# marcelm/cutadapt

Hardware: NVIDIA H100
Metric: reads/sec (150bp SE, 1 adapter, e=0.1) (higher is better)
Workload: dtype u8

## Files before the change

### cutadapt_b200/csrc/cg_api.cu

```cuda
#include <cuda_runtime.h>
#include <stdio.h>
#include <stdlib.h>
#include <string.h>

#include <algorithm>
#include <chrono>
#include <map>
#include <string>
#include <vector>

#include "../../include/cutadapt_b200.h"
#include "cg_hostpack.h"
#include <array>

#include "cg_gzip_core.cuh"
#include "cg_kernels.cuh"
#include "cg_jit.h"
#include "cg_setbuild.h"

static_assert(sizeof(cg_match) == 32 && sizeof(cg_match_rec) == 32, "cg_match must be 32 bytes");
static_assert(sizeof(CgAdapter) == 80 && sizeof(CgEntry) == 32 && sizeof(CgGroup) == 32 &&
                  sizeof(CgSetHeader) == 80, "table layout");

static thread_local std::string g_err;

static int fail(int code, const std::string &msg)
{
    g_err = msg;
    return code;
}
static int cuda_fail(cudaError_t e, const char *what)
{
    char buf[256];
    snprintf(buf, sizeof buf, "CUDA error in %s: %s", what, cudaGetErrorString(e));
    g_err = buf;
    return e == cudaErrorMemoryAllocation ? CG_ENOMEM : CG_ECUDA;
}
#define CU(x)                                                  \
    do {                                                       \
        cudaError_t _e = (x);                                  \
        if (_e != cudaSuccess) return cuda_fail(_e, #x);       \
    } while (0)

extern "C" int cg_version(void) { return CG_ABI_VERSION; }
extern "C" const char *cg_last_error(void) { return g_err.c_str(); }

template <class T> struct DevBuf {
    T *p = nullptr;
    size_t cap = 0;
    int ensure(size_t n)
    {
        if (n <= cap) return CG_OK;
        if (p) cudaFree(p);
        p = nullptr; cap = 0;
        size_t want = n + n / 4 + 64;
        cudaError_t e = cudaMalloc((void **)&p, want * sizeof(T));
        if (e != cudaSuccess) return cuda_fail(e, "cudaMalloc");
        cap = want;
        return CG_OK;
    }
    void release() { if (p) cudaFree(p); p = nullptr; cap = 0; }
};
template <class T> struct PinBuf {
    T *p = nullptr;
    size_t cap = 0;
    int ensure(size_t n)
    {
        if (n <= cap) return CG_OK;
        if (p) cudaFreeHost(p);
        p = nullptr; cap = 0;
        size_t want = n + n / 4 + 64;
        cudaError_t e = cudaMallocHost((void **)&p, want * sizeof(T));
        if (e != cudaSuccess) return cuda_fail(e, "cudaMallocHost");
        cap = want;
        return CG_OK;
    }
    void release() { if (p) cudaFreeHost(p); p = nullptr; cap = 0; }
};

#define CG_N_LANES 3
struct Lane {
    cudaStream_t stream = nullptr;
    DevBuf<uint8_t> d_seq, d_qual, d_pack;
    DevBuf<uint64_t> d_exc;
    PinBuf<uint8_t> h_pack;
    PinBuf<uint64_t> h_exc;
    DevBuf<int64_t> d_offs;
    DevBuf<cg_match_rec> d_out;
    DevBuf<int32_t> d_qtrim;
    PinBuf<uint8_t> h_seq, h_qual;
    PinBuf<int64_t> h_offs;
    PinBuf<cg_match_rec> h_out;
    PinBuf<int32_t> h_qtrim;
    bool busy = false;
    cg_match_rec *dst_out = nullptr; size_t n_out = 0; bool out_bounced = false;
    int32_t *dst_qtrim = nullptr; size_t n_qtrim = 0; bool qtrim_bounced = false;
};

#define CG_FQ_SLOTS 4
struct FastqSlot {
    cudaStream_t stream = nullptr;
    bool busy = false;
    int64_t n_bytes = 0;
    DevBuf<uint8_t> d_in, d_out, d_seq, d_qual;
    DevBuf<uint32_t> d_tiles, d_nl;
    DevBuf<CgFastqRecord> d_rec;
    DevBuf<int32_t> d_len, d_interval, d_keep, d_outlen, d_qtrim, d_mask, d_adest, d_dmbytes, d_dest, d_pairkey, d_origin;
    DevBuf<uint8_t> d_destkeep, d_names, d_infoout;
    DevBuf<int32_t> d_nameoff, d_inforow;
    DevBuf<int64_t> d_infooff;
    DevBuf<int64_t> d_dmbase;
    DevBuf<int64_t> d_offs, d_outoff;
    DevBuf<unsigned long long> d_scan;
    DevBuf<cg_match_rec> d_matches, d_matches_rc;
    DevBuf<uint8_t> d_isrc;
    DevBuf<uint8_t> d_norm;
    DevBuf<int32_t> d_faline;
    DevBuf<int64_t> d_faoff;
    DevBuf<unsigned long long> d_fqstats;
    DevBuf<int32_t> d_polya;
    PinBuf<unsigned long long> h_fqstats;
    DevBuf<int32_t> d_fold;
    DevBuf<unsigned long long> d_ilverr;
    DevBuf<CgGzPiece> d_gzpieces;
    DevBuf<uint8_t> d_gzslots, d_gzout;
    DevBuf<int32_t> d_gzsizes;
    DevBuf<int64_t> d_gzoff;
    int ilv = 0, ilv_peer = -1, ilv_format = 0;
    unsigned long long *d_counters = nullptr;
    int *d_err = nullptr;
    PinBuf<uint8_t> h_in, h_out;
    PinBuf<unsigned long long> h_counters;
};

struct GzinStream {
    DevBuf<uint8_t> d_gz, d_plain;
    PinBuf<uint8_t> h_gz;
    DevBuf<int32_t> d_counts, d_cand, d_members, d_flag;
    DevBuf<int64_t> d_offs;
    DevBuf<GuMember> d_res;
    DevBuf<long long> d_moff;
    DevBuf<unsigned long long> d_scan, d_small;
    DevBuf<uint32_t> d_tiles, d_nl;
    cudaEvent_t done = nullptr;
    long long carry = 0, consumed = 0, members = 0;
    long long pend_plain = 0, pend_consumed = 0, pend_members = 0;
    bool split = false;
    long long stride = CG_GZIN_STRIDE;
    struct Member { int in = 0, bitoff = 0, trailer = 0; uint32_t crc = 0; long long len = 0, start = 0; } mem, pmem;
    long long pend_respec = 0;
    DevBuf<uint8_t> d_win, d_pwin, d_wins;
    DevBuf<GuChunk> d_ch;
    DevBuf<long long> d_coff, d_room;
    DevBuf<uint16_t> d_sym;
    DevBuf<int32_t> d_redo;
    DevBuf<uint32_t> d_part;
    void release()
    {
        d_gz.release(); d_plain.release(); h_gz.release(); d_counts.release(); d_cand.release(); d_members.release();
        d_flag.release(); d_offs.release(); d_res.release(); d_moff.release(); d_scan.release(); d_small.release();
        d_tiles.release(); d_nl.release();
        d_win.release(); d_pwin.release(); d_wins.release(); d_ch.release(); d_coff.release(); d_room.release();
        d_sym.release(); d_redo.release(); d_part.release();
        if (done) cudaEventDestroy(done);
        done = nullptr;
    }
};

struct FqStatsAcc {
    int32_t n_adapters = 0, max_len = 0, kmax = 0;
    std::vector<int64_t> v;
};

struct cg_ctx {
    int device = 0;
    cudaStream_t stream = nullptr;
    bool own_stream = false;
    int sm_count = 148;
    size_t smem_optin = 0;
    Lane lanes[CG_N_LANES];
    int *d_err = nullptr;
    uint8_t *d_enc = nullptr;
    double *d_phred = nullptr;
    DevBuf<uint32_t> scratch_p;
    DevBuf<int> scratch_w;
    DevBuf<unsigned long long> d_stats;
    struct { unsigned long long *d_stats = nullptr; int max_len = 0, kmax = 0; bool armed = false, done = false; } fuse;
    DevBuf<uint4> tasks;
    DevBuf<uint4> tasks2, tasks3;
    unsigned long long *d_task_count = nullptr;
    DevBuf<cg_match_rec> pass_tmp;
    DevBuf<int32_t> view_base, view_back;
    long long launches = 0;
    std::vector<std::pair<cudaEvent_t, cudaEvent_t>> timing;
    std::vector<cudaEvent_t> event_pool;
    double timed_ms = 0.0;
    long long timed_n = 0;
    std::vector<std::array<cudaEvent_t, 4>> stage_events;
    double stage_ms[3] = {0, 0, 0};
    CgHostPool *pool = nullptr;
    std::vector<std::vector<uint64_t>> exc_scratch;
    long long h2d_bytes = 0, d2h_bytes = 0;
    double prof[8] = {0, 0, 0, 0, 0, 0, 0, 0};
    double pack_fraction = 0.6;
    double pack_ref_fraction = 0.6, pack_ref_rate = 0.0;
    int pack_dir = +1;
    bool pack_have_ref = false;
    int numa_node = -1;
    cudaEvent_t scratch_ev = nullptr;
    cudaStream_t scratch_stream = nullptr;
    bool scratch_busy = false;
    FastqSlot fq[CG_FQ_SLOTS];
    int fq_next = 0;
    std::map<int32_t, FqStatsAcc> fq_stats;
    int32_t fq_stats_next = 1;
    std::map<int32_t, GzinStream> gzin;
    int32_t gzin_next = 1;
};

struct cg_adapterset {
    cg_ctx *ctx = nullptr;
    CgBuiltSet host;
    uint8_t *d_blob = nullptr;
    uint64_t *d_masks = nullptr;
    CgEntry *d_entries = nullptr;
    uint8_t *d_index = nullptr;
    struct Pass {
        cg_adapterset *sub = nullptr;
        int group = 0, role = 0;
        int front_pass = -1;
        int map_off = 0;
    };
    std::vector<Pass> passes;
    std::vector<int32_t> pass_map;
    int32_t *d_pass_map = nullptr;
    CgSelectTables select_tables;
    mutable CgJitKernel *jit[2][2][2] = {};
    mutable int jit_state[2][2][2] = {};
    mutable long long plane_reads = 0;
    mutable std::string jit_error;
};

extern "C" int cg_ctx_create(int device, void *stream, cg_ctx **out)
{
    if (!out) return fail(CG_EINVAL, "cg_ctx_create: out is NULL");
    int count = 0;
    cudaError_t e = cudaGetDeviceCount(&count);
    if (e != cudaSuccess || count == 0)
        return fail(CG_ECUDA, std::string("no usable CUDA device (") + cudaGetErrorString(e) +
                                  "); cutadapt_b200 has no CPU fallback");
    if (device < 0 || device >= count) return fail(CG_EINVAL, "cg_ctx_create: device ordinal out of range");
    CU(cudaSetDevice(device));
    cg_ctx *c = new cg_ctx();
    c->device = device;
    cudaDeviceProp prop;
    CU(cudaGetDeviceProperties(&prop, device));
    c->sm_count = prop.multiProcessorCount;
    c->smem_optin = prop.sharedMemPerBlockOptin;
    if (stream) { c->stream = (cudaStream_t)stream; c->own_stream = false; }
    else { CU(cudaStreamCreateWithFlags(&c->stream, cudaStreamNonBlocking)); c->own_stream = true; }
    for (int i = 0; i < CG_N_LANES; ++i) CU(cudaStreamCreateWithFlags(&c->lanes[i].stream, cudaStreamNonBlocking));
    CU(cudaEventCreateWithFlags(&c->scratch_ev, cudaEventDisableTiming));
    CU(cudaMalloc((void **)&c->d_err, 16 * sizeof(int)));
    CU(cudaMemset(c->d_err, 0, 16 * sizeof(int)));
    CU(cudaMalloc((void **)&c->d_task_count, 64));
    CU(cudaMemset(c->d_task_count, 0, 64));
    CU(cudaMalloc((void **)&c->d_enc, 768));
    uint8_t enc[768];
    cg_build_enc_tables(enc);
    CU(cudaMemcpy(c->d_enc, enc, 768, cudaMemcpyHostToDevice));
    {
        double phred[256];
        cg_build_phred_table(phred);
        CU(cudaMalloc((void **)&c->d_phred, sizeof phred));
        CU(cudaMemcpy(c->d_phred, phred, sizeof phred, cudaMemcpyHostToDevice));
    }
    *out = c;
    return CG_OK;
}

static void resolve_timing(cg_ctx *c)
{
    for (auto &pr : c->timing) {
        float ms = 0.f;
        if (cudaEventSynchronize(pr.second) == cudaSuccess && cudaEventElapsedTime(&ms, pr.first, pr.second) == cudaSuccess) {
            c->timed_ms += ms; c->timed_n += 1;
        }
        c->event_pool.push_back(pr.first);
        c->event_pool.push_back(pr.second);
    }
    c->timing.clear();
}

extern "C" int cg_ctx_destroy(cg_ctx *c)
{
    if (!c) return CG_OK;
    cudaSetDevice(c->device);
    cudaDeviceSynchronize();
    resolve_timing(c);
    for (auto ev : c->event_pool) cudaEventDestroy(ev);
    delete c->pool;
    c->pool = nullptr;
    for (int i = 0; i < CG_N_LANES; ++i) {
        Lane &l = c->lanes[i];
        l.d_pack.release(); l.d_exc.release(); l.h_pack.release(); l.h_exc.release();
        l.d_seq.release(); l.d_qual.release(); l.d_offs.release(); l.d_out.release(); l.d_qtrim.release();
        l.h_seq.release(); l.h_qual.release(); l.h_offs.release(); l.h_out.release(); l.h_qtrim.release();
        if (l.stream) cudaStreamDestroy(l.stream);
    }
    c->scratch_p.release(); c->scratch_w.release(); c->tasks.release(); c->tasks2.release(); c->tasks3.release();
    c->pass_tmp.release(); c->view_base.release(); c->view_back.release();
    for (FastqSlot &f : c->fq) {
        f.d_in.release(); f.d_out.release(); f.d_seq.release(); f.d_qual.release(); f.d_tiles.release(); f.d_nl.release();
        f.d_rec.release(); f.d_len.release(); f.d_mask.release(); f.d_adest.release(); f.d_dmbytes.release();
        f.d_dmbase.release(); f.d_keep.release(); f.d_interval.release(); f.d_outlen.release(); f.d_qtrim.release();
        f.d_offs.release(); f.d_outoff.release(); f.d_scan.release(); f.d_matches.release(); f.d_matches_rc.release();
        f.d_isrc.release(); f.d_dest.release(); f.d_pairkey.release(); f.d_destkeep.release(); f.d_origin.release();
        f.d_names.release(); f.d_infoout.release(); f.d_nameoff.release(); f.d_inforow.release(); f.d_infooff.release();
        f.d_norm.release(); f.d_faline.release(); f.d_faoff.release();
        f.d_fqstats.release(); f.d_polya.release(); f.h_fqstats.release();
        f.d_gzpieces.release(); f.d_gzslots.release(); f.d_gzout.release(); f.d_gzsizes.release(); f.d_gzoff.release();
        f.h_in.release(); f.h_out.release(); f.h_counters.release();
        if (f.d_counters) cudaFree(f.d_counters);
        if (f.d_err) cudaFree(f.d_err);
        if (f.stream) cudaStreamDestroy(f.stream);
    }
    for (auto &kv : c->gzin) kv.second.release();
    if (c->scratch_ev) cudaEventDestroy(c->scratch_ev);
    if (c->d_task_count) cudaFree(c->d_task_count);
    if (c->d_err) cudaFree(c->d_err);
    if (c->d_enc) cudaFree(c->d_enc);
    if (c->d_phred) cudaFree(c->d_phred);
    if (c->own_stream && c->stream) cudaStreamDestroy(c->stream);
    delete c;
    return CG_OK;
}

extern "C" int cg_ctx_synchronize(cg_ctx *c)
{
    if (!c) return fail(CG_EINVAL, "ctx is NULL");
    CU(cudaSetDevice(c->device));
    CU(cudaStreamSynchronize(c->stream));
    for (int i = 0; i < CG_N_LANES; ++i) CU(cudaStreamSynchronize(c->lanes[i].stream));
    return CG_OK;
}

extern "C" int64_t cg_ctx_launch_count(cg_ctx *c) { return c ? c->launches : 0; }

extern "C" int cg_ctx_stage_times(cg_ctx *c, double *out3, int reset)
{
    if (!c || !out3) return fail(CG_EINVAL, "cg_ctx_stage_times: NULL argument");
    CU(cudaSetDevice(c->device));
    for (auto &e : c->stage_events) {
        CU(cudaEventSynchronize(e[3]));
        for (int i = 0; i < 3; ++i) {
            float ms = 0;
            CU(cudaEventElapsedTime(&ms, e[i], e[i + 1]));
            c->stage_ms[i] += ms;
        }
        for (auto ev : e) cudaEventDestroy(ev);
    }
    c->stage_events.clear();
    for (int i = 0; i < 3; ++i) out3[i] = c->stage_ms[i];
    if (reset) c->stage_ms[0] = c->stage_ms[1] = c->stage_ms[2] = 0;
    return CG_OK;
}

extern "C" int cg_ctx_kernel_time(cg_ctx *c, double *total_ms, int64_t *launches, int reset)
{
    if (!c) return fail(CG_EINVAL, "ctx is NULL");
    CU(cudaSetDevice(c->device));
    resolve_timing(c);
    if (total_ms) *total_ms = c->timed_ms;
    if (launches) *launches = c->timed_n;
    if (reset) { c->timed_ms = 0.0; c->timed_n = 0; }
    return CG_OK;
}

static void destroy_passes(cg_adapterset *s)
{
    for (auto &p : s->passes) cg_adapterset_destroy(p.sub);
    s->passes.clear();
    s->pass_map.clear();
    if (s->d_pass_map) { cudaFree(s->d_pass_map); s->d_pass_map = nullptr; }
}

static int upload_set(cg_ctx *c, cg_adapterset *s)
{
    s->ctx = c;
    cudaError_t e = cudaSetDevice(c->device);
    if (e == cudaSuccess) e = cudaMalloc((void **)&s->d_blob, s->host.blob.size());
    if (e == cudaSuccess) e = cudaMemcpy(s->d_blob, s->host.blob.data(), s->host.blob.size(), cudaMemcpyHostToDevice);
    if (e == cudaSuccess) e = cudaMalloc((void **)&s->d_masks, s->host.masks64.size() * 8);
    if (e == cudaSuccess) e = cudaMemcpy(s->d_masks, s->host.masks64.data(), s->host.masks64.size() * 8, cudaMemcpyHostToDevice);
    if (e == cudaSuccess && !s->host.index_blob.empty()) {
        e = cudaMalloc((void **)&s->d_index, s->host.index_blob.size());
        if (e == cudaSuccess) e = cudaMemcpy(s->d_index, s->host.index_blob.data(), s->host.index_blob.size(), cudaMemcpyHostToDevice);
    }
    if (e != cudaSuccess) {
        if (s->d_blob) cudaFree(s->d_blob);
        if (s->d_masks) cudaFree(s->d_masks);
        if (s->d_index) cudaFree(s->d_index);
        s->d_blob = nullptr; s->d_masks = nullptr; s->d_index = nullptr;
        return cuda_fail(e, "adapter set upload");
    }
    return CG_OK;
}

extern "C" int cg_adapterset_create_indexed(cg_ctx *c, const cg_adapter_desc *adapters, int32_t n_adapters,
                                            const cg_group_desc *groups, int32_t n_groups,
                                            const cg_index_desc *indexes, int32_t n_indexes, cg_adapterset **out)
{
    if (!c || !out) return fail(CG_EINVAL, "cg_adapterset_create: NULL argument");
    cg_adapterset *s = new cg_adapterset();
    std::string err;
    int rc = cg_build_set(adapters, n_adapters, groups, n_groups, s->host, err, indexes, n_indexes);
    if (rc != CG_OK) { delete s; return fail(rc, err); }
    rc = upload_set(c, s);
    if (rc != CG_OK) { delete s; return rc; }
    CgMultiPlan plan;
    if (cg_plan_passes(adapters, n_adapters, groups, n_groups, indexes, n_indexes, plan, err) == CG_OK &&
        !plan.passes.empty()) {
        bool ok = true;
        for (auto &pp : plan.passes) {
            cg_adapterset::Pass P;
            P.group = pp.group; P.role = pp.role; P.front_pass = pp.front_pass; P.map_off = pp.map_off;
            P.sub = new cg_adapterset();
            P.sub->host = std::move(pp.set);
            if (upload_set(c, P.sub) != CG_OK) { delete P.sub; ok = false; break; }
            s->passes.push_back(P);
        }
        if (ok) {
            const CgSetHeader *H = (const CgSetHeader *)s->host.blob.data();
            cg_fill_select_tables((const CgGroup *)(s->host.blob.data() + H->groups_off), s->host.n_groups,
                                  s->host.slots, plan.passes, s->select_tables);
            s->pass_map = plan.pass_map;
            cudaError_t e = cudaMalloc((void **)&s->d_pass_map, s->pass_map.size() * sizeof(int32_t));
            if (e == cudaSuccess)
                e = cudaMemcpy(s->d_pass_map, s->pass_map.data(), s->pass_map.size() * sizeof(int32_t), cudaMemcpyHostToDevice);
            if (e != cudaSuccess) { cudaGetLastError(); ok = false; }
        }
        if (!ok) destroy_passes(s);
    }
    *out = s;
    return CG_OK;
}

extern "C" int cg_adapterset_create(cg_ctx *c, const cg_adapter_desc *adapters, int32_t n_adapters,
                                    const cg_group_desc *groups, int32_t n_groups, cg_adapterset **out)
{
    return cg_adapterset_create_indexed(c, adapters, n_adapters, groups, n_groups, nullptr, 0, out);
}

extern "C" int cg_adapterset_destroy(cg_adapterset *s)
{
    if (!s) return CG_OK;
    if (s->ctx) cudaSetDevice(s->ctx->device);
    if (s->d_blob) cudaFree(s->d_blob);
    if (s->d_masks) cudaFree(s->d_masks);
    if (s->d_index) cudaFree(s->d_index);
    for (int w = 0; w < 2; ++w)
        for (int q = 0; q < 2; ++q)
            for (int v = 0; v < 2; ++v) cg_jit_destroy(s->jit[w][q][v]);
    destroy_passes(s);
    delete s;
    return CG_OK;
}

extern "C" int cg_adapterset_jit_status(const cg_adapterset *s)
{
    if (!s) return 0;
    const cg_adapterset *t = (!s->passes.empty() && s->passes[0].sub) ? s->passes[0].sub : s;
    int st = 0;
    for (int w = 0; w < 2; ++w)
        for (int q = 0; q < 2; ++q)
            for (int v = 0; v < 2; ++v) {
                if (t->jit_state[w][q][v] == 1) st = 1;
                else if (t->jit_state[w][q][v] == -1 && st == 0) st = -1;
            }
    if (st == -1) g_err = "first-stage specialisation failed: " + t->jit_error;
    return st;
}

extern "C" int64_t cg_adapterset_jit_source(const cg_adapterset *s, int32_t plane_words, int32_t has_qual, int32_t stats,
                                            char *buf, int64_t cap)
{
    if (!s) return 0;
    const std::string src = cg_jit_pscan_source(s->host, plane_words, has_qual != 0, stats != 0);
    if (buf && cap > 0) {
        const size_t n = std::min<size_t>(src.size(), (size_t)cap - 1);
        memcpy(buf, src.data(), n);
        buf[n] = 0;
    }
    return (int64_t)src.size();
}

extern "C" int cg_adapterset_slots(const cg_adapterset *s) { return s ? s->host.slots : 0; }

extern "C" int cg_adapterset_effective_length(const cg_adapterset *s, int32_t adapter, int32_t *out)
{
    if (!s || !out || adapter < 0 || adapter >= s->host.n_adapters) return fail(CG_EINVAL, "bad adapter index");
    *out = s->host.effective_length[adapter];
    return CG_OK;
}

static int launch_trim_single(cg_ctx *c, const cg_adapterset *s, const uint8_t *d_seq, const uint8_t *d_qual,
                              const int64_t *d_offsets, int64_t n_reads, int max_read_len, const cg_params *p,
                              cg_match_rec *d_out, int32_t *d_qtrim, const int32_t *d_view, cudaStream_t st,
                              bool timed)
{
    if (n_reads <= 0) return CG_OK;
    const int times = p->times < 1 ? 1 : p->times;
    const bool want_q = p->quality_trim != 0 || p->nextseq_trim != 0;
    if (want_q && !d_qual) return fail(CG_ENOQUAL, "Cannot do quality trimming when no qualities are available");
    CgKernelArgs a;
    memset(&a, 0, sizeof a);
    a.blob = s->d_blob; a.blob_bytes = (uint32_t)s->host.blob.size();
    a.masks64 = s->d_masks; a.enc = c->d_enc; a.index = s->d_index;
    a.seq = d_seq; a.qual = want_q ? d_qual : nullptr; a.offsets = d_offsets; a.n_reads = n_reads;
    a.quality_trim = (p->quality_trim ? 1 : 0) | (p->nextseq_trim ? 2 : 0);
    a.cutoff_front = p->cutoff_front; a.cutoff_back = p->cutoff_back;
    a.qbase = (p->quality_base & 255) | (int)((unsigned)p->nextseq_cutoff << 8); a.times = times; a.slots = s->host.slots;
    a.out = d_out; a.qtrim = d_qtrim; a.view = d_view; a.err_flag = c->d_err;
    a.col_rows = s->host.max_m + 1;
    a.no_band = getenv("CUTADAPT_B200_NO_BAND") != nullptr;

    const long long tile_cap_ll = ((long long)CG_NT * max_read_len + 32 + 15) / 16 * 16;
    bool fast = !s->host.any_wide && max_read_len <= CG_PACKED_MAX_N && tile_cap_ll < (1 << 24);
    size_t smem = 0;
    int occ = 0;
    if (fast) {
        a.tile_cap = (int)tile_cap_ll;
        smem = cg_fast_smem_bytes(a.blob_bytes, a.tile_cap, a.col_rows, want_q);
        if (smem > c->smem_optin) fast = false;
    }
    const char *kernel_env = getenv("CUTADAPT_B200_KERNEL");
    const bool force_general = kernel_env && strcmp(kernel_env, "general") == 0;
    const bool simple = fast && s->host.simple_ok && times == 1 && !force_general;
    if (fast) {
        CU(cg_fast_occupancy(want_q, simple, smem, &occ));
        if (occ < 1) fast = false;
    }
    const bool force_block = kernel_env && strcmp(kernel_env, "block") == 0;
    const bool force_warp = kernel_env && strcmp(kernel_env, "warp") == 0;
    bool split = false;
    int plane_w = 0;
    size_t scan_smem = 0, list_smem = 0;
    int scan_occ = 0, plan_occ = 0, run_occ = 0;
    if (simple && s->host.max_m <= 64 && !force_block && !force_warp) {
        const long long mini = ((long long)32 * max_read_len + 32 + 15) / 16 * 16;
        const long long cslot = ((long long)max_read_len + 4 + 15) / 16 * 16 + 32;
        const CgSetHeader *hdr = (const CgSetHeader *)s->host.blob.data();
        const char *scan_env = getenv("CUTADAPT_B200_SCAN");
        if (hdr->plane_count > 0 && max_read_len <= 256 && !(scan_env && strcmp(scan_env, "shiftand") == 0))
            plane_w = max_read_len <= 160 ? 5 : 8;
        long long cslot_need = cslot;
        if (plane_w) cslot_need = std::max<long long>(cslot, 16LL * (2 * plane_w + 1) + 16);
        if (mini < (1 << 20)) {
            a.mini_cap = (int)mini; a.carry_slot = (int)cslot_need;
            scan_smem = plane_w ? cg_pscan_smem_bytes(a.blob_bytes, a.mini_cap, want_q)
                                : cg_scan_smem_bytes(a.blob_bytes, a.mini_cap, want_q);
            list_smem = cg_dp_smem_bytes(a.blob_bytes, a.carry_slot);
            if (scan_smem <= c->smem_optin && list_smem <= c->smem_optin) {
                if (plane_w) CU(cg_pscan_occupancy(want_q, plane_w, false, scan_smem, &scan_occ));
                else CU(cg_scan_occupancy(want_q, scan_smem, &scan_occ));
                CU(cg_list_occupancy(true, s->host.max_m, list_smem, &plan_occ));
                CU(cg_list_occupancy(false, s->host.max_m, list_smem, &run_occ));
                split = scan_occ >= 1 && plan_occ >= 1 && run_occ >= 1;
            }
        }
    }
    bool warpk = false;
    size_t wsmem = 0;
    int wocc = 0;
    if (simple && s->host.max_m <= 32 && force_warp) {
        const long long mini = ((long long)32 * max_read_len + 32 + 15) / 16 * 16;
        const long long cslot = ((long long)max_read_len + 4 + 15) / 16 * 16 + 16;
        if (mini < (1 << 20)) {
            a.mini_cap = (int)mini; a.carry_slot = (int)cslot;
            wsmem = cg_warp_smem_bytes(a.blob_bytes, a.mini_cap, a.carry_slot, want_q);
            if (wsmem <= c->smem_optin) {
                CU(cg_warp_occupancy(want_q, wsmem, &wocc));
                warpk = wocc >= 1;
            }
        }
    }
    bool fuse_stats = split && plane_w && c->fuse.armed && !d_view && s->host.n_adapters == 1 && times == 1 &&
                      s->host.slots == 1 && !want_q && !getenv("CUTADAPT_B200_TWO_LISTS") && c->fuse.max_len <= 4096;
    if (fuse_stats) {
        const size_t fsmem = cg_pscan_smem_bytes(a.blob_bytes, a.mini_cap, want_q, c->fuse.max_len);
        int focc = 0;
        if (fsmem <= c->smem_optin) CU(cg_pscan_occupancy(want_q, plane_w, true, fsmem, &focc));
        fuse_stats = focc >= 1 && focc >= scan_occ;
        if (fuse_stats) {
            a.stats = c->fuse.d_stats; a.stats_max_len = c->fuse.max_len; a.stats_kmax = c->fuse.kmax;
            scan_smem = fsmem; scan_occ = focc;
        }
    }
    CgJitKernel *jit_kernel = nullptr;
    int jit_occ = 0;
    if (split && plane_w) {
        const int wi = plane_w <= 5 ? 0 : 1, qi = want_q ? 1 : 0, vi = fuse_stats ? 1 : 0;
        s->plane_reads += n_reads;
        const char *je = getenv("CUTADAPT_B200_JIT");
        const bool never = je && strcmp(je, "0") == 0, always = je && strcmp(je, "1") == 0;
        if (!never && s->jit_state[wi][qi][vi] == 0 && (always || s->plane_reads >= (4LL << 20))) {
            std::string err;
            s->jit[wi][qi][vi] = cg_jit_build_pscan(s->host, plane_w, want_q, fuse_stats, err);
            s->jit_state[wi][qi][vi] = s->jit[wi][qi][vi] ? 1 : -1;
            if (!s->jit[wi][qi][vi]) s->jit_error = err;
        }
        if (!never && s->jit_state[wi][qi][vi] == 1) {
            jit_occ = cg_jit_occupancy(s->jit[wi][qi][vi], CG_NT, scan_smem);
            if (jit_occ >= 1) jit_kernel = s->jit[wi][qi][vi];
        }
    }
    const bool stage_times = getenv("CUTADAPT_B200_STAGE_TIMES") != nullptr;
    cudaEvent_t ev0 = nullptr, ev1 = nullptr;
    if (timed && c->timing.size() < 8192) {
        for (cudaEvent_t *ev : {&ev0, &ev1}) {
            if (!c->event_pool.empty()) { *ev = c->event_pool.back(); c->event_pool.pop_back(); }
            else CU(cudaEventCreate(ev));
        }
        CU(cudaEventRecord(ev0, st));
    }
    const bool light = s->host.all_indexed && !want_q && !s->host.any_wide && s->host.max_m + 1 <= CG_LIGHT_ROWS &&
                       !(kernel_env && strcmp(kernel_env, "general") == 0) && !getenv("CUTADAPT_B200_NO_LIGHT");
    if (light && times == 1 && !d_view && a.slots == 1 && !getenv("CUTADAPT_B200_NO_INDEX_KERNEL")) {
        const long long SUBI = 64LL << 20;
        int rc = c->tasks.ensure((size_t)((std::min<long long>(n_reads, SUBI) + 3) / 4));
        if (rc != CG_OK) return rc;
        for (long long r0 = 0; r0 < n_reads; r0 += SUBI) {
            const long long n_sub = std::min<long long>(SUBI, n_reads - r0);
            CgKernelArgs b = a;
            b.offsets = a.offsets + r0; b.n_reads = n_sub; b.out = a.out + (size_t)r0 * a.slots;
            b.tasks = c->tasks.p; b.task_count = c->d_task_count;
            CU(cudaMemsetAsync(c->d_task_count, 0, sizeof(unsigned long long), st));
            const long long need = (n_sub + CG_NT - 1) / CG_NT;
            const int grid = (int)std::max<long long>(1, std::min<long long>((long long)c->sm_count * 16, need));
            CU(cg_launch_index(b, grid, st));
            c->launches += 1;
        }
    } else if (light) {
        const long long need = (n_reads + CG_NT - 1) / CG_NT;
        const int grid = (int)std::max<long long>(1, std::min<long long>((long long)c->sm_count * 16, need));
        CU(cg_launch_light(a, grid, st));
    } else if (split) {
        long long SUB = (plane_w && getenv("CUTADAPT_B200_TASK_BYTES")) ? (16LL << 20) : (32LL << 20);
        if (const char *e = getenv("CUTADAPT_B200_SUB_READS")) { const long long v = atoll(e); if (v >= 1024) SUB = v; }
        SUB = std::min<long long>(SUB, 1LL << 31);
        const long long cap = std::min<long long>(n_reads, SUB);
        const bool task_bytes = plane_w && getenv("CUTADAPT_B200_TASK_BYTES") != nullptr;
        const int plane_rec = plane_w ? (task_bytes ? 4 + 2 * plane_w + 1 : 4) : 2;
        int rc = c->tasks.ensure((size_t)cap * plane_rec);
        if (rc == CG_OK) rc = c->tasks2.ensure((size_t)cap * 4);
        if (rc == CG_OK) rc = c->tasks3.ensure((size_t)cap * 4);
        if (rc != CG_OK) return rc;
        unsigned long long *cnt = c->d_task_count;
        for (long long r0 = 0; r0 < n_reads; r0 += SUB) {
            const long long n_sub = std::min<long long>(SUB, n_reads - r0);
            CgKernelArgs b = a;
            b.offsets = a.offsets + r0;
            b.n_reads = n_sub;
            b.out = a.out + (size_t)r0 * a.times * a.slots;
            b.qtrim = a.qtrim ? a.qtrim + 2 * r0 : nullptr;
            b.view = a.view ? a.view + 2 * r0 : nullptr;
            b.task_cap = n_sub;
            CU(cudaMemsetAsync(cnt, 0, 8 * sizeof(unsigned long long), st));
            const long long n_mt = (n_sub + 31) / 32;
            const long long need = (n_mt + 3) / 4;
            auto grid_for = [&](int occ) { return (int)std::max<long long>(1, std::min<long long>((long long)occ * c->sm_count, need)); };
            std::array<cudaEvent_t, 4> sev = {nullptr, nullptr, nullptr, nullptr};
            if (stage_times && c->stage_events.size() < 4096) {
                for (auto &e : sev) CU(cudaEventCreate(&e));
                CU(cudaEventRecord(sev[0], st));
            }
            b.tasks = c->tasks.p; b.task_count = cnt;
            b.task_rec = plane_rec;
            b.task_count_b = (plane_w && getenv("CUTADAPT_B200_TWO_LISTS")) ? cnt + 4 : nullptr;
            if (plane_w && jit_kernel) {
                const int rcj = cg_jit_launch(jit_kernel, grid_for(jit_occ), CG_NT, scan_smem, (void *)st, &b);
                if (rcj != 0) return fail(CG_ECUDA, "launch of the specialised first stage failed (CUresult " + std::to_string(rcj) + ")");
            }
            else if (plane_w) CU(cg_launch_pscan(b, want_q, plane_w, grid_for(scan_occ), scan_smem, st));
            else CU(cg_launch_scan(b, want_q, grid_for(scan_occ), scan_smem, st));
            if (sev[0]) CU(cudaEventRecord(sev[1], st));
            b.tasks2 = c->tasks2.p; b.task2_count = cnt + 1;
            b.tasks3 = c->tasks3.p; b.task3_count = cnt + 2;
            b.task2_count_b = (CG_RUN_BAND && plane_w && !getenv("CUTADAPT_B200_NO_BAND_LISTS")) ? cnt + 5 : nullptr;
            CU(cg_launch_list(b, true, s->host.max_m, grid_for(plan_occ), list_smem, st));
            c->launches += 2;
            if (plane_w) {
                CgKernelArgs b2 = b;
                b2.tasks = c->tasks3.p; b2.task_count = cnt + 2; b2.task_rec = 2;
                b2.tasks3 = nullptr; b2.task3_count = cnt + 3; b2.task_count_b = nullptr;
                CU(cg_launch_list(b2, true, s->host.max_m, grid_for(plan_occ), list_smem, st));
                CU(cudaMemsetAsync(cnt + 2, 0, sizeof(unsigned long long), st));
                c->launches += 1;
            }
            if (sev[0]) CU(cudaEventRecord(sev[2], st));
            uint4 *lists[2] = {c->tasks2.p, c->tasks3.p};
            for (int round = 0; round < 4; ++round) {
                const int in = round & 1, outl = in ^ 1;
                if (round > 0) CU(cudaMemsetAsync(cnt + 1 + outl, 0, sizeof(unsigned long long), st));
                b.tasks = lists[in]; b.task_count = cnt + 1 + in;
                b.task_count_b = round == 0 ? b.task2_count_b : nullptr;
                b.tasks2 = lists[outl]; b.task2_count = cnt + 1 + outl;
                if (round == 0) b.task2_count_b = nullptr;
                else b.task_count_b = nullptr;
                CU(cg_launch_list(b, false, s->host.max_m, grid_for(run_occ), list_smem, st));
                c->launches += 1;
            }
            if (sev[0]) { CU(cudaEventRecord(sev[3], st)); c->stage_events.push_back(sev); }
            if (fuse_stats) {
                CU(cg_launch_stats(b.seq, b.offsets, n_sub, want_q && b.qtrim, 1, 1, b.out, b.qtrim, 1, a.stats_max_len,
                                   a.stats_kmax, a.stats, st, c->tasks.p, plane_rec, cnt));
                c->launches += 1;
            }
        }
        if (fuse_stats) c->fuse.done = true;
        c->launches -= 1;
    } else if (warpk) {
        const long long n_mt = (n_reads + 31) / 32;
        long long grid = (long long)wocc * c->sm_count;
        const long long need = (n_mt + 3) / 4;
        if (grid > need) grid = need;
        if (grid < 1) grid = 1;
        CU(cg_launch_warp(a, want_q, (int)grid, wsmem, st));
    } else if (fast) {
        const long long n_tiles = (n_reads + CG_NT - 1) / CG_NT;
        long long grid = (long long)occ * c->sm_count;
        if (grid > n_tiles) grid = n_tiles;
        CU(cg_launch_fast(a, want_q, simple, (int)grid, smem, st));
    } else {
        const int block = 128;
        long long threads = (long long)c->sm_count * 8 * block;
        const long long per_thread = (long long)a.col_rows * 16;
        while (threads > 32 * block && threads * per_thread > (1LL << 30)) threads /= 2;
        if (threads > ((n_reads + block - 1) / block) * block) threads = ((n_reads + block - 1) / block) * block;
        int rc = c->scratch_p.ensure((size_t)threads * a.col_rows);
        if (rc != CG_OK) return rc;
        rc = c->scratch_w.ensure((size_t)threads * a.col_rows * 3);
        if (rc != CG_OK) return rc;
        a.scratch_p = c->scratch_p.p; a.scratch_w = c->scratch_w.p; a.scratch_stride = threads;
        CU(cg_launch_generic(a, (int)(threads / block), block, st));
    }
    c->launches += 1;
    if (ev0) {
        CU(cudaEventRecord(ev1, st));
        c->timing.emplace_back(ev0, ev1);
    }
    return CG_OK;
}

static int launch_trim_inner(cg_ctx *c, const cg_adapterset *s, const uint8_t *d_seq, const uint8_t *d_qual,
                             const int64_t *d_offsets, int64_t n_reads, int max_read_len, const cg_params *p,
                             cg_match_rec *d_out, int32_t *d_qtrim, cudaStream_t st, bool timed)
{
    if (n_reads <= 0) return CG_OK;
    const int times = p->times < 1 ? 1 : p->times;
    const char *kernel_env = getenv("CUTADAPT_B200_KERNEL");
    const bool force_general = kernel_env && strcmp(kernel_env, "general") == 0;
    if (s->passes.empty() || times != 1 || force_general)
        return launch_trim_single(c, s, d_seq, d_qual, d_offsets, n_reads, max_read_len, p, d_out, d_qtrim, nullptr,
                                  st, timed);
    const bool want_q = p->quality_trim != 0 || p->nextseq_trim != 0;
    if (want_q && !d_qual) return fail(CG_ENOQUAL, "Cannot do quality trimming when no qualities are available");
    struct Disarm { cg_ctx *c; bool was; ~Disarm() { c->fuse.armed = was; } } disarm{c, c->fuse.armed};
    c->fuse.armed = false;
    const int np = (int)s->passes.size();
    long long SUB = 32LL << 20;
    if (const char *e = getenv("CUTADAPT_B200_SUB_READS")) { const long long v = atoll(e); if (v >= 1024) SUB = v; }
    const long long cap = std::min<long long>(n_reads, SUB);
    int rc = c->pass_tmp.ensure((size_t)cap * np);
    if (rc != CG_OK) return rc;
    bool any_linked = false;
    for (auto &P : s->passes) any_linked = any_linked || P.role == 1;
    if (any_linked) { rc = c->view_back.ensure((size_t)cap * 2); if (rc != CG_OK) return rc; }
    if (want_q && !d_qtrim) { rc = c->view_base.ensure((size_t)cap * 2); if (rc != CG_OK) return rc; }

    CgSelectArgs sel;
    memset(&sel, 0, sizeof sel);
    sel.tmp = c->pass_tmp.p; sel.stride = cap; sel.pass_map = s->d_pass_map;
    sel.t = s->select_tables;

    cudaEvent_t ev0 = nullptr, ev1 = nullptr;
    if (timed && c->timing.size() < 8192) {
        for (cudaEvent_t *ev : {&ev0, &ev1}) {
            if (!c->event_pool.empty()) { *ev = c->event_pool.back(); c->event_pool.pop_back(); }
            else CU(cudaEventCreate(ev));
        }
        CU(cudaEventRecord(ev0, st));
    }
    for (long long r0 = 0; r0 < n_reads; r0 += SUB) {
        const long long n_sub = std::min<long long>(SUB, n_reads - r0);
        const int64_t *offs = d_offsets + r0;
        int32_t *qt = want_q ? (d_qtrim ? d_qtrim + 2 * r0 : c->view_base.p) : nullptr;
        const int32_t *base_view = nullptr;
        for (int pi = 0; pi < np; ++pi) {
            const auto &P = s->passes[pi];
            cg_match_rec *tmp = c->pass_tmp.p + (size_t)pi * cap;
            cg_params pp = *p;
            pp.times = 1;
            const int32_t *view = base_view;
            if (P.role == 1) {
                CU(cg_launch_linked_view(c->pass_tmp.p + (size_t)P.front_pass * cap, base_view, offs, n_sub,
                                         c->view_back.p, st));
                c->launches += 1;
                view = c->view_back.p;
            }
            if (want_q && pi == 0) {
                rc = launch_trim_single(c, P.sub, d_seq, d_qual, offs, n_sub, max_read_len, &pp, tmp, qt, nullptr, st, false);
                base_view = qt;
            } else {
                pp.quality_trim = 0; pp.nextseq_trim = 0;
                rc = launch_trim_single(c, P.sub, d_seq, nullptr, offs, n_sub, max_read_len, &pp, tmp, nullptr, view, st, false);
            }
            if (rc != CG_OK) return rc;
        }
        sel.n_reads = n_sub;
        sel.out = d_out + (size_t)r0 * s->host.slots;
        CU(cg_launch_select(sel, st));
        c->launches += 1;
    }
    if (ev0) {
        CU(cudaEventRecord(ev1, st));
        c->timing.emplace_back(ev0, ev1);
    }
    return CG_OK;
}

extern "C" int cg_locate_debug(cg_ctx *c, const cg_adapter_desc *adapter, const uint8_t *query, int32_t n,
                               int32_t *cost, int32_t *score, int32_t *result8)
{
    if (!c || !adapter || !cost || !score || !result8 || n < 0 || (n && !query))
        return fail(CG_EINVAL, "cg_locate_debug: bad argument");
    if (adapter->kind != CG_KIND_ALIGNER) return fail(CG_EINVAL, "cg_locate_debug: only aligner adapters have a DP matrix");
    for (int32_t i = 0; i < n; ++i) if (query[i] & 0x80) return fail(CG_ENONASCII, "String must contain only ASCII characters");
    CU(cudaSetDevice(c->device));
    cg_adapter_desc d = *adapter;
    d.n_kmer_entries = 0; d.kmer_entries = nullptr; d.kmer_masks = nullptr; d.reverse_read = 0;
    cg_group_desc g;
    memset(&g, 0, sizeof g);
    g.type = CG_GROUP_SINGLE; g.a0 = 0; g.a1 = -1;
    CgBuiltSet set;
    std::string err;
    int rc = cg_build_set(&d, 1, &g, 1, set, err);
    if (rc != CG_OK) return fail(rc, err);
    const int m = set.max_m;
    const size_t cells = (size_t)(m + 1) * ((size_t)n + 1);
    DevBuf<uint8_t> d_blob, d_query;
    DevBuf<int> d_scratch;
    DevBuf<int32_t> d_mat, d_res;
    struct Free {
        DevBuf<uint8_t> &a, &b; DevBuf<int> &s; DevBuf<int32_t> &m, &r;
        ~Free() { a.release(); b.release(); s.release(); m.release(); r.release(); }
    } free_all{d_blob, d_query, d_scratch, d_mat, d_res};
    if ((rc = d_blob.ensure(set.blob.size())) != CG_OK || (rc = d_query.ensure((size_t)n + 16)) != CG_OK ||
        (rc = d_scratch.ensure(3 * ((size_t)m + 2))) != CG_OK || (rc = d_mat.ensure(2 * cells)) != CG_OK ||
        (rc = d_res.ensure(8)) != CG_OK)
        return rc;
    std::vector<int32_t> none(2 * cells, CG_DEBUG_NONE);
    CU(cudaMemcpy(d_blob.p, set.blob.data(), set.blob.size(), cudaMemcpyHostToDevice));
    if (n) CU(cudaMemcpy(d_query.p, query, (size_t)n, cudaMemcpyHostToDevice));
    CU(cudaMemcpy(d_mat.p, none.data(), 2 * cells * sizeof(int32_t), cudaMemcpyHostToDevice));
    CU(cg_launch_locate_debug(d_blob.p, c->d_enc, d_query.p, n, d_scratch.p, d_mat.p, d_mat.p + cells, d_res.p, c->stream));
    c->launches += 1;
    CU(cudaStreamSynchronize(c->stream));
    CU(cudaMemcpy(cost, d_mat.p, cells * sizeof(int32_t), cudaMemcpyDeviceToHost));
    CU(cudaMemcpy(score, d_mat.p + cells, cells * sizeof(int32_t), cudaMemcpyDeviceToHost));
    CU(cudaMemcpy(result8, d_res.p, 8 * sizeof(int32_t), cudaMemcpyDeviceToHost));
    return CG_OK;
}

static int launch_trim(cg_ctx *c, const cg_adapterset *s, const uint8_t *d_seq, const uint8_t *d_qual,
                       const int64_t *d_offsets, int64_t n_reads, int max_read_len, const cg_params *p,
                       cg_match_rec *d_out, int32_t *d_qtrim, cudaStream_t st, bool timed)
{
    if (n_reads <= 0) return CG_OK;
    if (c->scratch_busy && c->scratch_stream != st) CU(cudaStreamWaitEvent(st, c->scratch_ev, 0));
    const int rc = launch_trim_inner(c, s, d_seq, d_qual, d_offsets, n_reads, max_read_len, p, d_out, d_qtrim, st, timed);
    CU(cudaEventRecord(c->scratch_ev, st));
    c->scratch_busy = true;
    c->scratch_stream = st;
    return rc;
}

static int launch_trim_with_stats(cg_ctx *c, const cg_adapterset *s, const uint8_t *d_seq, const uint8_t *d_qual,
                                  const int64_t *d_offsets, int64_t n_reads, int max_read_len, const cg_params *p,
                                  cg_match_rec *d_out, int32_t *d_qtrim, cudaStream_t st, bool timed,
                                  unsigned long long *d_stats, int stats_max_len, int stats_kmax)
{
    if (n_reads <= 0) return CG_OK;
    c->fuse.d_stats = d_stats; c->fuse.max_len = stats_max_len; c->fuse.kmax = stats_kmax;
    c->fuse.armed = true; c->fuse.done = false;
    const int rc = launch_trim(c, s, d_seq, d_qual, d_offsets, n_reads, max_read_len, p, d_out, d_qtrim, st, timed);
    c->fuse.armed = false;
    if (rc != CG_OK) return rc;
    if (!c->fuse.done) {
        const int times = p->times < 1 ? 1 : p->times;
        CU(cg_launch_stats(d_seq, d_offsets, n_reads, (p->quality_trim || p->nextseq_trim) && d_qtrim, times, s->host.slots,
                           d_out, d_qtrim, s->host.n_adapters, stats_max_len, stats_kmax, d_stats, st));
        c->launches += 1;
    }
    return CG_OK;
}

static int check_err_flag(cg_ctx *c)
{
    int flags[2] = {0, 0};
    CU(cudaMemcpy(flags, c->d_err, sizeof flags, cudaMemcpyDeviceToHost));
    if (flags[0]) {
        cudaMemset(c->d_err, 0, sizeof(int));
        return fail(CG_ENONASCII, "String must contain only ASCII characters");
    }
    return CG_OK;
}

extern "C" int cg_process_batch_device(cg_ctx *c, const cg_adapterset *s, const uint8_t *d_seq,
                                       const uint8_t *d_qual, const int64_t *d_offsets, int64_t n_reads,
                                       int32_t max_read_len, const cg_params *p, cg_match *d_matches,
                                       int32_t *d_qtrim)
{
    if (!c || !s || !p || !d_seq || !d_offsets || !d_matches) return fail(CG_EINVAL, "cg_process_batch_device: NULL argument");
    if (s->ctx != c) return fail(CG_EINVAL, "adapter set belongs to another context");
    if (((uintptr_t)d_seq & 15) || (d_qual && ((uintptr_t)d_qual & 15)))
        return fail(CG_EINVAL, "device sequence/quality buffers must be 16-byte aligned");
    if (n_reads < 0) return fail(CG_EINVAL, "n_reads < 0");
    CU(cudaSetDevice(c->device));
    if (max_read_len <= 0) {
        CU(cudaMemsetAsync(c->d_err + 1, 0, sizeof(int), c->stream));
        CU(cg_launch_max_len(d_offsets, n_reads, c->d_err + 1, c->stream));
        c->launches += 1;
        CU(cudaMemcpyAsync(&max_read_len, c->d_err + 1, sizeof(int), cudaMemcpyDeviceToHost, c->stream));
        CU(cudaStreamSynchronize(c->stream));
    }
    return launch_trim(c, s, d_seq, d_qual, d_offsets, n_reads, max_read_len, p, (cg_match_rec *)d_matches,
                       d_qtrim, c->stream, true);
}

extern "C" int cg_process_batch_device_stats(cg_ctx *c, const cg_adapterset *s, const uint8_t *d_seq,
                                             const uint8_t *d_qual, const int64_t *d_offsets, int64_t n_reads,
                                             int32_t max_read_len, const cg_params *p, cg_match *d_matches,
                                             int32_t *d_qtrim, int32_t stats_max_len, int32_t stats_kmax, int64_t *d_stats)
{
    if (!c || !s || !p || !d_seq || !d_offsets || !d_matches || !d_stats || stats_max_len < 0 || stats_kmax < 0)
        return fail(CG_EINVAL, "cg_process_batch_device_stats: bad argument");
    if (s->ctx != c) return fail(CG_EINVAL, "adapter set belongs to another context");
    if (((uintptr_t)d_seq & 15) || (d_qual && ((uintptr_t)d_qual & 15)))
        return fail(CG_EINVAL, "device sequence/quality buffers must be 16-byte aligned");
    if (n_reads < 0) return fail(CG_EINVAL, "n_reads < 0");
    if ((p->quality_trim || p->nextseq_trim) && !d_qtrim)
        return fail(CG_EINVAL, "cg_process_batch_device_stats: quality trimming needs d_qtrim (the statistics read it)");
    CU(cudaSetDevice(c->device));
    if (max_read_len <= 0) {
        CU(cudaMemsetAsync(c->d_err + 1, 0, sizeof(int), c->stream));
        CU(cg_launch_max_len(d_offsets, n_reads, c->d_err + 1, c->stream));
        c->launches += 1;
        CU(cudaMemcpyAsync(&max_read_len, c->d_err + 1, sizeof(int), cudaMemcpyDeviceToHost, c->stream));
        CU(cudaStreamSynchronize(c->stream));
    }
    return launch_trim_with_stats(c, s, d_seq, d_qual, d_offsets, n_reads, max_read_len, p, (cg_match_rec *)d_matches,
                                  d_qtrim, c->stream, true, (unsigned long long *)d_stats, stats_max_len, stats_kmax);
}

static void parallel_copy(cg_ctx *c, void *dst, const void *src, size_t n);

static bool is_pinned(const void *p)
{
    if (!p) return false;
    cudaPointerAttributes at;
    if (cudaPointerGetAttributes(&at, p) != cudaSuccess) { cudaGetLastError(); return false; }
    return at.type == cudaMemoryTypeHost;
}

static int lane_finish(cg_ctx *c, Lane &l)
{
    if (!l.busy) return CG_OK;
    CU(cudaStreamSynchronize(l.stream));
    if (l.out_bounced && l.n_out) memcpy(l.dst_out, l.h_out.p, l.n_out * sizeof(cg_match_rec));
    if (l.qtrim_bounced && l.n_qtrim) memcpy(l.dst_qtrim, l.h_qtrim.p, l.n_qtrim * sizeof(int32_t));
    l.busy = false;
    return CG_OK;
}

struct OffsetScan { int64_t max_len = 0; bool uniform = true, valid = true; };
static OffsetScan scan_offsets_part(const int64_t *offsets, int64_t len0, int64_t a, int64_t b)
{
    OffsetScan o;
    for (int64_t r = a; r < b; ++r) {
        const int64_t len = offsets[r + 1] - offsets[r];
        if (len < 0 || len > 2000000000LL) o.valid = false;
        if (len > o.max_len) o.max_len = len;
        o.uniform = o.uniform && len == len0;
    }
    return o;
}
static void scan_merge(OffsetScan &t, const OffsetScan &o)
{
    t.max_len = std::max(t.max_len, o.max_len);
    t.uniform = t.uniform && o.uniform;
    t.valid = t.valid && o.valid;
}
static const int64_t SCAN_JOB = 1 << 15;
static OffsetScan scan_offsets(cg_ctx *c, const int64_t *offsets, int64_t r0, int64_t r1)
{
    const int64_t len0 = offsets[r0 + 1] - offsets[r0];
    const int64_t nr = r1 - r0;
    if (!c->pool || nr < (1 << 16)) return scan_offsets_part(offsets, len0, r0, r1);
    const int64_t n_jobs = (nr + SCAN_JOB - 1) / SCAN_JOB;
    std::vector<OffsetScan> parts((size_t)c->pool->size());
    c->pool->run(n_jobs, [&](int64_t j, int w) {
        const int64_t a = r0 + j * SCAN_JOB, b = std::min(r1, a + SCAN_JOB);
        scan_merge(parts[(size_t)w], scan_offsets_part(offsets, len0, a, b));
    });
    OffsetScan t;
    for (const OffsetScan &o : parts) scan_merge(t, o);
    return t;
}
// ... 1273 lines not shown
    CU(cg_launch_fastq_demux(0, d_len, d_dest, n, n_dest, f.d_dmbytes.p, nullptr, nullptr, st));
    CU(cg_launch_scan_i32(f.d_dmbytes.p, cells, f.d_scan.p, f.d_dmbase.p, st));
    CU(cg_launch_fastq_demux(1, d_len, d_dest, n, n_dest, nullptr, f.d_dmbase.p, f.d_outoff.p, st));
    c->launches += 5;
    CU(cudaMemcpy2DAsync(segments, sizeof(int64_t), f.d_dmbase.p, (size_t)tiles * sizeof(int64_t), sizeof(int64_t),
                         (size_t)n_dest, cudaMemcpyDeviceToHost, st));
    CU(cudaMemcpyAsync(segments + n_dest, f.d_dmbase.p + cells, sizeof(int64_t), cudaMemcpyDeviceToHost, st));
    CU(cudaMemcpyAsync(total, f.d_dmbase.p + cells, sizeof *total, cudaMemcpyDeviceToHost, st));
    return CG_OK;
}

static int fastq_split_interleaved(cg_ctx *c, FastqSlot &f1, FastqSlot &f2, cudaStream_t st)
{
    CU(cudaStreamSynchronize(f2.stream));
    CU(cudaStreamSynchronize(st));
    const bool fasta = f1.ilv_format == CG_FORMAT_FASTA;
    FqStage g;
    g.n_nl = (long long)f1.h_counters.p[0];
    long long n_lines = g.n_nl;
    if (f1.n_bytes > 0) {
        uint8_t last = 0;
        CU(cudaMemcpyAsync(&last, f1.d_in.p + f1.n_bytes - 1, 1, cudaMemcpyDeviceToHost, st));
        CU(cudaStreamSynchronize(st));
        if (last != '\n') n_lines += 1;
    }
    int rc;
    long long n = 0;
    if (!fasta) {
        if (n_lines % 4 != 0)
            return fail(CG_EINVAL, "FASTQ chunk does not consist of complete 4-line records (" + std::to_string(n_lines) +
                                       " lines)");
        n = n_lines / 4;
        if ((rc = f1.d_nl.ensure((size_t)g.n_nl + 1)) != CG_OK) return rc;
        CU(cg_launch_fastq_index(f1.d_in.p, f1.n_bytes, f1.d_tiles.p, nullptr, f1.d_nl.p, 1, st));
        c->launches += 1;
    } else if (n_lines > 0) {
        cg_fastq_params plain;
        memset(&plain, 0, sizeof plain);
        if ((rc = fasta_stage_normalise(c, f1, &plain, n_lines, st, g, &n)) != CG_OK) return rc;
    }
    if (n % 2 != 0)
        return fail(CG_EINVAL, "Interleaved input file incomplete: the chunk holds an odd number of records (" +
                                   std::to_string(n) + "), record " + std::to_string(n - 1) + " has no mate");
    int64_t seg[3] = {0, 0, 0};
    if (n > 0) {
        if ((rc = f1.d_rec.ensure((size_t)n + 1)) != CG_OK) return rc;
        if ((rc = f1.d_len.ensure((size_t)n)) != CG_OK) return rc;
        if ((rc = f1.d_outlen.ensure((size_t)n)) != CG_OK) return rc;
        if ((rc = f1.d_dest.ensure((size_t)n)) != CG_OK) return rc;
        if ((rc = f1.d_outoff.ensure((size_t)n + 1)) != CG_OK) return rc;
        if ((rc = f1.d_ilverr.ensure(1)) != CG_OK) return rc;
        const unsigned long long none = ~0ull;
        CU(cudaMemcpyAsync(f1.d_ilverr.p, &none, sizeof none, cudaMemcpyHostToDevice, st));
        CU(cg_launch_interleaved_split(0, f1.d_in.p, f1.n_bytes, fasta ? nullptr : f1.d_nl.p, g.n_nl, n, f1.d_rec.p,
                                       f1.d_len.p, f1.d_outlen.p, f1.d_dest.p, f1.d_ilverr.p, nullptr, 0, nullptr, nullptr,
                                       fasta ? 1 : 0, st));
        c->launches += 2;
        long long total = 0;
        if ((rc = fastq_partition(c, f1, n, 2, f1.d_outlen.p, f1.d_dest.p, seg, &total, st)) != CG_OK) return rc;
        unsigned long long bad = none;
        CU(cudaMemcpyAsync(&bad, f1.d_ilverr.p, sizeof bad, cudaMemcpyDeviceToHost, st));
        CU(cudaStreamSynchronize(st));
        if (bad != none) {
            const long long r = (long long)(bad >> 32);
            const int code = (int)(bad & 0xFFFFFFFFu);
            if (code != CG_FQ_ERR_PAIR) {
                const int e[2] = {code, (int)r};
                return fastq_format_error(e);
            }
            CgFastqRecord h[2];
            CU(cudaMemcpy(h, f1.d_rec.p + r - 1, sizeof h, cudaMemcpyDeviceToHost));
            std::string names[2];
            for (int k = 0; k < 2; ++k) {
                names[k].resize((size_t)std::max(h[k].hdr_len, 0));
                if (h[k].hdr_len > 0)
                    CU(cudaMemcpy(&names[k][0], f1.d_in.p + h[k].hdr_start, (size_t)h[k].hdr_len, cudaMemcpyDeviceToHost));
            }
            return fail(CG_EINVAL, "Reads are improperly paired: records " + std::to_string(r - 1) + " and " +
                                       std::to_string(r) + " of the interleaved chunk, read name '" + names[0] +
                                       "' does not match '" + names[1] + "'");
        }
        std::swap(f1.d_in, f1.d_norm);
        if ((rc = f1.d_in.ensure((size_t)seg[1] + 64)) != CG_OK) return rc;
        if ((rc = f2.d_in.ensure((size_t)(seg[2] - seg[1]) + 64)) != CG_OK) return rc;
        CU(cg_launch_interleaved_split(1, f1.d_norm.p, 0, nullptr, 0, n, nullptr, f1.d_len.p, f1.d_outlen.p, nullptr,
                                       nullptr, f1.d_outoff.p, seg[1], f1.d_in.p, f2.d_in.p, fasta ? 1 : 0, st));
        c->launches += 1;
    }
    f1.n_bytes = seg[1];
    f2.n_bytes = seg[2] - seg[1];
    const int err_init[2] = {0, 0x7FFFFFFF};
    for (FastqSlot *f : {&f1, &f2}) {
        if ((rc = f->d_tiles.ensure((size_t)cg_fastq_tiles(f->n_bytes) + 1)) != CG_OK) return rc;
        CU(cudaMemsetAsync(f->d_counters, 0, (1 + CG_FQ_COUNTERS) * sizeof(unsigned long long), st));
        CU(cudaMemcpyAsync(f->d_err, err_init, sizeof err_init, cudaMemcpyHostToDevice, st));
        if (f->n_bytes) {
            CU(cg_launch_fastq_index(f->d_in.p, f->n_bytes, f->d_tiles.p, f->d_counters, nullptr, 0, st));
            c->launches += 2;
        }
        CU(cudaMemcpyAsync(f->h_counters.p, f->d_counters, sizeof(unsigned long long), cudaMemcpyDeviceToHost, st));
    }
    CU(cudaStreamSynchronize(st));
    return CG_OK;
}

static int fastq_stage_records(cg_ctx *c, FastqSlot &f, const cg_fastq_params *fp, bool has_set, cudaStream_t st, FqStage &g)
{
    if (fp->format < CG_FORMAT_FASTQ || fp->format > CG_FORMAT_FASTQ_TO_FASTA)
        return fail(CG_EINVAL, "cg_fastq: format must be 0 (FASTQ), 1 (FASTA) or 2 (FASTQ in, FASTA out)");
    if (fp->format == CG_FORMAT_FASTA &&
        (fp->trim.quality_trim || fp->trim.nextseq_trim || fp->max_expected_errors >= 0.0))
        return fail(CG_EINVAL, "FASTA input has no qualities: quality trimming, --nextseq-trim and --max-ee need FASTQ");
    g.format = fp->format;
    CU(cudaStreamSynchronize(f.stream));
    const int64_t n_bytes = f.n_bytes;
    g.n_nl = (long long)f.h_counters.p[0];
    long long n_lines = g.n_nl;
    if (n_bytes > 0) {
        uint8_t last = 0;
        CU(cudaMemcpyAsync(&last, f.d_in.p + n_bytes - 1, 1, cudaMemcpyDeviceToHost, st));
        CU(cudaStreamSynchronize(st));
        if (last != '\n') n_lines += 1;
    }
    const bool fasta = fp->format == CG_FORMAT_FASTA;
    if (!fasta && n_lines % 4 != 0)
        return fail(CG_EINVAL, "FASTQ chunk does not consist of complete 4-line records (" + std::to_string(n_lines) +
                                   " lines)");
    long long n_fasta = 0;
    if (fasta && n_lines > 0) {
        int rc = fasta_stage_normalise(c, f, fp, n_lines, st, g, &n_fasta);
        if (rc != CG_OK) return rc;
    }
    const long long n = g.n = fasta ? n_fasta : n_lines / 4;
    if (n == 0) return CG_OK;
    const cg_params *p = &fp->trim;
    g.want_q = p->quality_trim != 0 || p->nextseq_trim != 0;
    g.times = p->times < 1 ? 1 : p->times;
    if (fp->cut_front < 0 || fp->cut_back < 0) return fail(CG_EINVAL, "cg_fastq: cut_front / cut_back must be >= 0");
    if (fp->action < CG_FQ_ACTION_TRIM || fp->action > CG_FQ_ACTION_CROP) return fail(CG_EINVAL, "cg_fastq: unknown action");
    if ((fp->action == CG_FQ_ACTION_RETAIN || fp->action == CG_FQ_ACTION_CROP) && g.times > 1)
        return fail(CG_EINVAL, "'retain' and 'crop' cannot be combined with times > 1");
    if (fp->revcomp < 0 || fp->revcomp > 2) return fail(CG_EINVAL, "cg_fastq: revcomp must be 0, 1 or 2");
    g.action = has_set ? fp->action : CG_FQ_ACTION_TRIM;
    int rc;
    if ((rc = f.d_nl.ensure((size_t)g.n_nl + 1)) != CG_OK) return rc;
    if ((rc = f.d_rec.ensure((size_t)n)) != CG_OK) return rc;
    if ((rc = f.d_len.ensure((size_t)n)) != CG_OK) return rc;
    if ((rc = f.d_origin.ensure((size_t)n * 2)) != CG_OK) return rc;
    if ((rc = f.d_interval.ensure((size_t)n * 2)) != CG_OK) return rc;
    if ((rc = f.d_mask.ensure((size_t)n)) != CG_OK) return rc;
    if ((rc = f.d_keep.ensure((size_t)n * 2)) != CG_OK) return rc;
    if ((rc = f.d_outlen.ensure((size_t)n)) != CG_OK) return rc;
    if ((rc = f.d_outoff.ensure((size_t)n + 1)) != CG_OK) return rc;
    if ((rc = f.d_scan.ensure((size_t)cg_scan_tiles(n) + 1)) != CG_OK) return rc;
    if (g.want_q && (rc = f.d_qtrim.ensure((size_t)n * 2)) != CG_OK) return rc;
    if (!fasta) {
        CU(cg_launch_fastq_index(f.d_in.p, n_bytes, f.d_tiles.p, nullptr, f.d_nl.p, 1, st));
        CU(cg_launch_fastq_records(f.d_in.p, n_bytes, f.d_nl.p, g.n_nl, n, fp->cut_front, fp->cut_back, f.d_rec.p, f.d_len.p,
                                   f.d_origin.p, f.d_counters + 1, f.d_err, st));
        c->launches += 2;
    }
    g.d_qtrim = g.want_q ? f.d_qtrim.p : nullptr;
    return CG_OK;
}

static int fastq_stage_pretrim(cg_ctx *c, FastqSlot &f, const cg_params *p, cudaStream_t st, FqStage &g)
{
    CU(cg_launch_fastq_pretrim(f.d_in.p, f.d_rec.p, f.d_len.p, g.n, (p->quality_trim ? 1 : 0) | (p->nextseq_trim ? 2 : 0),
                               p->cutoff_front, p->cutoff_back,
                               (p->quality_base & 255) | (int)((unsigned)p->nextseq_cutoff << 8), g.d_qtrim, st));
    c->launches += 1;
    return CG_OK;
}

static int fastq_stage_fold_qtrim(cg_ctx *c, FastqSlot &f, const cg_params *p, cudaStream_t st, FqStage &g)
{
    if (!g.want_q) return CG_OK;
    int rc = fastq_stage_pretrim(c, f, p, st, g);
    if (rc != CG_OK) return rc;
    CU(cg_launch_fastq_fold_qtrim(f.d_rec.p, f.d_len.p, g.d_qtrim, g.n, f.d_origin.p, f.d_counters + 1, st));
    c->launches += 1;
    g.d_qtrim = nullptr;
    g.want_q = false;
    return CG_OK;
}

static int fastq_stage_pack(cg_ctx *c, FastqSlot &f, cudaStream_t st, FqStage &g, bool reverse_complement)
{
    const long long n = g.n;
    int rc;
    if ((rc = f.d_offs.ensure((size_t)n + 1)) != CG_OK) return rc;
    if ((rc = f.d_seq.ensure((size_t)f.n_bytes + 64)) != CG_OK) return rc;
    if (g.want_q && (rc = f.d_qual.ensure((size_t)f.n_bytes + 64)) != CG_OK) return rc;
    if (!reverse_complement) {
        CU(cg_launch_scan_i32(f.d_len.p, n, f.d_scan.p, f.d_offs.p, st));
        c->launches += 3;
    }
    CU(cg_launch_fastq_gather(f.d_in.p, f.d_rec.p, f.d_offs.p, n, f.d_seq.p, g.want_q ? f.d_qual.p : nullptr,
                              reverse_complement ? 1 : 0, st));
    c->launches += 1;
    if (reverse_complement) return CG_OK;
    g.packed = true;
    CU(cudaMemsetAsync(c->d_err + 1, 0, sizeof(int), st));
    CU(cg_launch_max_len(f.d_offs.p, n, c->d_err + 1, st));
    c->launches += 1;
    int fq_err[2];
    CU(cudaMemcpyAsync(&g.max_len, c->d_err + 1, sizeof(int), cudaMemcpyDeviceToHost, st));
    CU(cudaMemcpyAsync(fq_err, f.d_err, sizeof fq_err, cudaMemcpyDeviceToHost, st));
    CU(cudaStreamSynchronize(st));
    if (fq_err[0]) return fastq_format_error(fq_err, f.ilv);
    return CG_OK;
}

static int fastq_stage_verdict(cg_ctx *c, FastqSlot &f, const cg_fastq_params *fp, int poly_a_mode, cudaStream_t st,
                               FqStage &g)
{
    int32_t *d_poly_a = nullptr;
    if (g.acc && fp->poly_a) {
        int rc = f.d_polya.ensure((size_t)g.n);
        if (rc != CG_OK) return rc;
        d_poly_a = f.d_polya.p;
        g.st_poly_a = true;
    }
    CgFastqFilter flt;
    flt.minimum_length = fp->minimum_length;
    flt.maximum_length = fp->maximum_length;
    flt.discard_trimmed = fp->discard_trimmed;
    flt.discard_untrimmed = fp->discard_untrimmed;
    flt.max_n = fp->max_n;
    flt.max_ee = fp->max_expected_errors;
    flt.poly_a = fp->poly_a ? poly_a_mode : 0;
    flt.shorten = !fp->shorten ? 0 : (fp->shorten_length >= 0 ? fp->shorten_length + 1 : fp->shorten_length);
    flt.trim_n = fp->trim_n;
    flt.discard_casava = fp->discard_casava;
    flt.action = g.action;
    CU(cg_launch_fastq_evaluate(f.d_in.p, f.d_rec.p, f.d_len.p, g.n, g.d_matches, g.times, g.slots, g.d_qtrim, flt,
                                c->d_phred, g.d_is_rc, f.d_interval.p, f.d_keep.p, f.d_mask.p, f.d_counters + 1, f.d_err,
                                st, d_poly_a));
    c->launches += 1;
    return CG_OK;
}

static long long fqstats_total(int n_adapters, int max_len, int kmax)
{
    return cg_stats_total(n_adapters, max_len, kmax) + n_adapters + (max_len + 1);
}

static void fqstats_grow(FqStatsAcc &a, int max_len, int kmax)
{
    max_len = std::max(max_len, a.max_len);
    kmax = std::max(kmax, a.kmax);
    if (max_len == a.max_len && kmax == a.kmax) return;
    const int n = a.n_adapters, L0 = a.max_len, K0 = a.kmax;
    std::vector<int64_t> v((size_t)fqstats_total(n, max_len, kmax), 0);
    for (int i = 0; i < CG_STATS_SCALARS; ++i) v[i] = a.v[i];
    for (int l = 0; l <= L0; ++l) v[CG_STATS_SCALARS + l] = a.v[CG_STATS_SCALARS + l];
    const long long e0 = cg_stats_end_size(L0, K0), e1 = cg_stats_end_size(max_len, kmax);
    const long long b0 = cg_stats_adapters_off(L0), b1 = cg_stats_adapters_off(max_len);
    for (long long e = 0; e < 2LL * n; ++e) {
        const int64_t *src = a.v.data() + b0 + e * e0;
        int64_t *dst = v.data() + b1 + e * e1;
        for (int j = 0; j < CG_STATS_ADJ; ++j) dst[j] = src[j];
        for (int l = 0; l <= L0; ++l)
            for (int k = 0; k <= K0; ++k)
                dst[CG_STATS_ADJ + (long long)l * (kmax + 1) + k] = src[CG_STATS_ADJ + (long long)l * (K0 + 1) + k];
    }
    const long long t0 = cg_stats_total(n, L0, K0), t1 = cg_stats_total(n, max_len, kmax);
    for (int i = 0; i < n; ++i) v[t1 + i] = a.v[t0 + i];
    for (int l = 0; l <= L0; ++l) v[t1 + n + l] = a.v[t0 + n + l];
    a.v.swap(v);
    a.max_len = max_len;
    a.kmax = kmax;
}

static int fqstats_lookup(cg_ctx *c, int32_t handle, int n_adapters, FqStatsAcc **out)
{
    *out = nullptr;
    if (handle == 0) return CG_OK;
    auto it = c->fq_stats.find(handle);
    if (it == c->fq_stats.end()) return fail(CG_EINVAL, "cg_fastq: unknown statistics handle " + std::to_string(handle));
    if (it->second.n_adapters != n_adapters)
        return fail(CG_EINVAL, "cg_fastq: the statistics accumulator was created for " +
                                   std::to_string(it->second.n_adapters) + " adapters, the adapter set has " +
                                   std::to_string(n_adapters));
    *out = &it->second;
    return CG_OK;
}

static int fastq_stage_stats(cg_ctx *c, FastqSlot &f, FqStage &g, int kmax, cudaStream_t st)
{
    if (!g.acc || g.n == 0) return CG_OK;
    int rc;
    if (!g.packed && (rc = fastq_stage_pack(c, f, st, g, false)) != CG_OK) return rc;
    FqStatsAcc &a = *g.acc;
    fqstats_grow(a, g.max_len, kmax);
    g.st_len = a.max_len;
    g.st_kmax = a.kmax;
    const size_t total = (size_t)fqstats_total(a.n_adapters, a.max_len, a.kmax);
    if ((rc = f.d_fqstats.ensure(total)) != CG_OK) return rc;
    if ((rc = f.h_fqstats.ensure(total)) != CG_OK) return rc;
    CU(cudaMemsetAsync(f.d_fqstats.p, 0, total * sizeof(unsigned long long), st));
    if (g.d_matches && a.n_adapters > 0) {
        CU(cg_launch_stats(f.d_seq.p, f.d_offs.p, g.n, g.d_qtrim != nullptr, g.times, g.slots, g.d_matches, g.d_qtrim,
                           a.n_adapters, a.max_len, a.kmax, f.d_fqstats.p, st, nullptr, 0, nullptr, 0,
                           g.action == CG_FQ_ACTION_LOWERCASE ? 1 : 0));
        c->launches += 1;
    }
    return CG_OK;
}

static int fastq_stage_stats_tail(cg_ctx *c, FastqSlot &f, const FqStage &g, cudaStream_t st,
                                  const int32_t *d_route = nullptr)
{
    if (!g.acc || g.n == 0) return CG_OK;
    const int n_ad = g.acc->n_adapters;
    unsigned long long *v = f.d_fqstats.p;
    const long long tail = cg_stats_total(n_ad, g.st_len, g.st_kmax);
    CU(cg_launch_fastq_stats_tail(g.n, f.d_interval.p, f.d_outlen.p, g.st_poly_a ? f.d_polya.p : nullptr, g.d_matches,
                                  g.times, g.slots, g.d_is_rc, n_ad, g.st_len, v + CG_STATS_SCALARS, v + tail + n_ad,
                                  v + tail, st, d_route));
    c->launches += 1;
    const size_t total = (size_t)fqstats_total(n_ad, g.st_len, g.st_kmax);
    CU(cudaMemcpyAsync(f.h_fqstats.p, v, total * sizeof(unsigned long long), cudaMemcpyDeviceToHost, st));
    return CG_OK;
}

static void fastq_stats_commit(const FastqSlot &f, const FqStage &g, const cg_fastq_params *fp, const cg_fastq_result &res)
{
    if (!g.acc || g.n == 0) return;
    FqStatsAcc &a = *g.acc;
    const unsigned long long *h = f.h_fqstats.p;
    for (size_t i = CG_STATS_SCALARS; i < a.v.size(); ++i) a.v[i] += (int64_t)h[i];
    int64_t *v = a.v.data();
    v[0] += res.n_records; v[1] += res.bp_in; v[2] += res.with_adapters; v[3] += res.quality_trimmed_bp;
    v[4] += (int64_t)h[4]; v[5] += res.reverse_complemented; v[6] += res.n_written; v[7] += res.bp_out;
    v[8] += res.too_short; v[9] += res.too_long; v[10] += res.too_many_n; v[11] += res.too_many_expected_errors;
    v[12] += res.casava_filtered;
    v[fp->discard_trimmed ? 13 : 14] += res.discarded;
}

static int fastq_stage_evaluate(cg_ctx *c, FastqSlot &f, const cg_adapterset *s, const cg_fastq_params *fp, int poly_a_mode,
                                cudaStream_t st, FqStage &g)
{
    int rc = fastq_stage_records(c, f, fp, s != nullptr, st, g);
    if (rc != CG_OK || g.n == 0) return rc;
    const long long n = g.n;
    const cg_params *p = &fp->trim;
    g.slots = s ? s->host.slots : 1;
    if (s && fp->revcomp) {
        if ((rc = fastq_stage_fold_qtrim(c, f, p, st, g)) != CG_OK) return rc;
        cg_params pt = *p;
        pt.quality_trim = 0;
        pt.nextseq_trim = 0;
        const size_t per_read = (size_t)g.times * g.slots;
        if ((rc = f.d_matches.ensure((size_t)n * per_read)) != CG_OK) return rc;
        if ((rc = f.d_matches_rc.ensure((size_t)n * per_read)) != CG_OK) return rc;
        if ((rc = f.d_isrc.ensure((size_t)n)) != CG_OK) return rc;
        if ((rc = fastq_stage_pack(c, f, st, g, false)) != CG_OK) return rc;
        rc = launch_trim(c, s, f.d_seq.p, nullptr, f.d_offs.p, n, g.max_len, &pt, f.d_matches.p, nullptr, st, true);
        if (rc != CG_OK) return rc;
        if ((rc = fastq_stage_pack(c, f, st, g, true)) != CG_OK) return rc;
        rc = launch_trim(c, s, f.d_seq.p, nullptr, f.d_offs.p, n, g.max_len, &pt, f.d_matches_rc.p, nullptr, st, true);
        if (rc != CG_OK) return rc;
        CU(cg_launch_fastq_revcomp_commit(f.d_in.p, f.d_rec.p, f.d_len.p, f.d_origin.p, n, f.d_matches.p, f.d_matches_rc.p, (int)per_read,
                                          f.d_isrc.p, f.d_counters + 1, st, g.has_qual() ? 1 : 0));
        c->launches += 1;
        g.d_matches = f.d_matches.p;
        g.d_is_rc = f.d_isrc.p;
        g.rc_suffix = fp->revcomp == 1;
        if (g.acc) {
            CU(cg_launch_fastq_gather(f.d_in.p, f.d_rec.p, f.d_offs.p, n, f.d_seq.p, nullptr, 0, st));
            c->launches += 1;
        }
    } else if (s) {
        if ((rc = f.d_matches.ensure((size_t)n * g.times * g.slots)) != CG_OK) return rc;
        if ((rc = fastq_stage_pack(c, f, st, g, false)) != CG_OK) return rc;
        rc = launch_trim(c, s, f.d_seq.p, g.want_q ? f.d_qual.p : nullptr, f.d_offs.p, n, g.max_len, p, f.d_matches.p,
                         g.d_qtrim, st, true);
        if (rc != CG_OK) return rc;
        g.d_matches = f.d_matches.p;
    } else if (g.want_q) {
        if ((rc = fastq_stage_pretrim(c, f, p, st, g)) != CG_OK) return rc;
    }
    if ((rc = fastq_stage_stats(c, f, g, s ? s->host.max_k : 0, st)) != CG_OK) return rc;
    return fastq_stage_verdict(c, f, fp, poly_a_mode, st, g);
}

struct FqDemux {
    const int32_t *adapter_dest1 = nullptr;
    int n_adapters1 = 0, n_named1 = 0;
    const int32_t *adapter_dest2 = nullptr;
    int n_adapters2 = 0, n_named2 = 0;
    const uint8_t *dest_keep = nullptr;
    int n_dest() const { return (n_named1 + 1) * (adapter_dest2 ? n_named2 + 1 : 1); }
    const int32_t *d_dest = nullptr;
    const uint8_t *d_dest_keep = nullptr;
};

static int fastq_stage_route(cg_ctx *c, FastqSlot &f1, FastqSlot *f2, long long n, FqDemux &dm, cudaStream_t st)
{
    int rc;
    if ((rc = f1.d_adest.ensure((size_t)dm.n_adapters1 + dm.n_adapters2 + 1)) != CG_OK) return rc;
    if ((rc = f1.d_dest.ensure((size_t)n)) != CG_OK) return rc;
    CU(cudaMemcpyAsync(f1.d_adest.p, dm.adapter_dest1, (size_t)dm.n_adapters1 * sizeof(int32_t), cudaMemcpyHostToDevice, st));
    if (dm.adapter_dest2)
        CU(cudaMemcpyAsync(f1.d_adest.p + dm.n_adapters1, dm.adapter_dest2, (size_t)dm.n_adapters2 * sizeof(int32_t),
                           cudaMemcpyHostToDevice, st));
    CU(cg_launch_fastq_dest(f1.d_mask.p, dm.adapter_dest2 ? f2->d_mask.p : nullptr, n, f1.d_adest.p, dm.n_named1,
                            f1.d_adest.p + dm.n_adapters1, dm.n_named2, f1.d_dest.p, st));
    c->launches += 1;
    dm.d_dest = f1.d_dest.p;
    if (dm.dest_keep) {
        if ((rc = f1.d_destkeep.ensure((size_t)dm.n_dest())) != CG_OK) return rc;
        CU(cudaMemcpyAsync(f1.d_destkeep.p, dm.dest_keep, (size_t)dm.n_dest(), cudaMemcpyHostToDevice, st));
        dm.d_dest_keep = f1.d_destkeep.p;
    }
    return CG_OK;
}

struct FqSplit {
    int redirect = 0;
    int fasta_dests = 0;
    int32_t *d_route = nullptr;
    bool interleaved = false;
    int ilv_dests = 0;
    static constexpr int n_dest = 4;
};

static int split_check(const FqSplit &sp, const cg_fastq_params *fp, const char *who)
{
    if (sp.redirect & ~7) return fail(CG_EINVAL, std::string(who) + ": redirect takes CG_REDIRECT_* bits only");
    if ((sp.fasta_dests >> 1) & ~7) return fail(CG_EINVAL, std::string(who) + ": fasta_outputs takes CG_REDIRECT_* bits only");
    if ((sp.redirect & CG_REDIRECT_UNTRIMMED) && fp->discard_trimmed)
        return fail(CG_EINVAL, std::string(who) + ": the untrimmed output cannot be combined with discard_trimmed");
    if (fp->format == CG_FORMAT_FASTA && (sp.redirect & ~(sp.fasta_dests >> 1)))
        return fail(CG_EINVAL, std::string(who) + ": FASTA input can only be written as FASTA (set every redirect bit in "
                                                   "fasta_outputs)");
    return CG_OK;
}

static int fastq_stage_result(FastqSlot &f, const FqStage &g, cudaStream_t st, cg_fastq_result *res)
{
    int fq_err[2];
    CU(cudaMemcpyAsync(fq_err, f.d_err, sizeof fq_err, cudaMemcpyDeviceToHost, st));
    CU(cudaMemcpyAsync(f.h_counters.p, f.d_counters, (1 + CG_FQ_COUNTERS) * sizeof(unsigned long long),
                       cudaMemcpyDeviceToHost, st));
    CU(cudaStreamSynchronize(st));
    if (fq_err[0]) return fastq_format_error(fq_err, f.ilv);
    const unsigned long long *k = f.h_counters.p + 1;
    res->n_records = g.n;
    res->n_written = (int64_t)k[0]; res->bp_in = (int64_t)k[1]; res->bp_out = (int64_t)k[2];
    res->with_adapters = (int64_t)k[3]; res->too_short = (int64_t)k[4]; res->too_long = (int64_t)k[5];
    res->quality_trimmed_bp = (int64_t)k[6]; res->discarded = (int64_t)k[7]; res->too_many_n = (int64_t)k[8];
    res->too_many_expected_errors = (int64_t)k[9];
    res->casava_filtered = (int64_t)k[10];
    res->reverse_complemented = (int64_t)k[11];
    return CG_OK;
}

static int fastq_write_records(cg_ctx *c, FastqSlot &f, const FqStage &g, uint8_t *d_out, const FqSplit *sp,
                               const int64_t *segments, cudaStream_t st)
{
    if (!sp) {
        CU(cg_launch_fastq_write(f.d_in.p, f.d_rec.p, f.d_interval.p, f.d_outoff.p, f.d_outlen.p, g.n, d_out, g.action,
                                 f.d_keep.p, f.d_mask.p, g.rc_suffix, st, g.fasta_out() ? 1 : 0));
        c->launches += 1;
        return CG_OK;
    }
    for (int fa = 0; fa < 2; ++fa) {
        bool present = false;
        for (int d = 0; d < FqSplit::n_dest; ++d)
            present |= ((sp->fasta_dests >> d) & 1) == fa && segments[d + 1] > segments[d];
        if (!present) continue;
        CU(cg_launch_fastq_write(f.d_in.p, f.d_rec.p, f.d_interval.p, f.d_outoff.p, f.d_outlen.p, g.n, d_out, g.action,
                                 f.d_keep.p, f.d_mask.p, g.rc_suffix, st, fa, sp->d_route, sp->fasta_dests));
        c->launches += 1;
    }
    return CG_OK;
}

static int fastq_copy_out(cg_ctx *c, FastqSlot &f, uint8_t *out, const uint8_t *d_src, long long bytes, cudaStream_t st)
{
    if (bytes <= 0) return CG_OK;
    if (is_pinned(out)) {
        CU(cudaMemcpyAsync(out, d_src, (size_t)bytes, cudaMemcpyDeviceToHost, st));
        CU(cudaStreamSynchronize(st));
    } else {
        const int rc = f.h_out.ensure((size_t)bytes);
        if (rc != CG_OK) return rc;
        CU(cudaMemcpyAsync(f.h_out.p, d_src, (size_t)bytes, cudaMemcpyDeviceToHost, st));
        CU(cudaStreamSynchronize(st));
        parallel_copy(c, out, f.h_out.p, (size_t)bytes);
    }
    c->d2h_bytes += bytes;
    return CG_OK;
}

static int fastq_gzip(cg_ctx *c, FastqSlot &f, const uint8_t *d_src, std::vector<int64_t> &bounds, const std::vector<char> &gz,
                      long long *total, cudaStream_t st)
{
    const size_t n_dest = gz.size();
    std::vector<CgGzPiece> pieces;
    for (size_t d = 0; d < n_dest; ++d)
        for (int64_t o = bounds[d]; o < bounds[d + 1]; o += GZ_MEMBER)
            pieces.push_back(CgGzPiece{(long long)o, (int32_t)std::min<int64_t>(GZ_MEMBER, bounds[d + 1] - o), gz[d] ? 1 : 0});
    const size_t np = pieces.size();
    *total = 0;
    if (np == 0) return CG_OK;
    int rc;
    if ((rc = f.d_gzpieces.ensure(np)) != CG_OK || (rc = f.d_gzsizes.ensure(np)) != CG_OK ||
        (rc = f.d_gzoff.ensure(np)) != CG_OK || (rc = f.d_gzslots.ensure(np * GZ_SLOT)) != CG_OK)
        return rc;
    CU(cudaMemcpyAsync(f.d_gzpieces.p, pieces.data(), np * sizeof(CgGzPiece), cudaMemcpyHostToDevice, st));
    CU(cg_launch_gzip_compress(d_src, f.d_gzpieces.p, (int)np, f.d_gzslots.p, f.d_gzsizes.p, st));
    std::vector<int32_t> sizes(np);
    CU(cudaMemcpyAsync(sizes.data(), f.d_gzsizes.p, np * sizeof(int32_t), cudaMemcpyDeviceToHost, st));
    CU(cudaStreamSynchronize(st));
    std::vector<int64_t> off(np);
    int64_t at = 0;
    size_t k = 0;
    for (size_t d = 0; d < n_dest; ++d) {
        const int64_t n_pieces = (bounds[d + 1] - bounds[d] + GZ_MEMBER - 1) / GZ_MEMBER;
        bounds[d] = at;
        for (int64_t i = 0; i < n_pieces; ++i, ++k) { off[k] = at; at += sizes[k]; }
    }
    bounds[n_dest] = at;
    if ((rc = f.d_gzout.ensure((size_t)at + 64)) != CG_OK) return rc;
    CU(cudaMemcpyAsync(f.d_gzoff.p, off.data(), np * sizeof(int64_t), cudaMemcpyHostToDevice, st));
    CU(cg_launch_gzip_gather(f.d_gzslots.p, f.d_gzsizes.p, f.d_gzoff.p, (int)np, f.d_gzout.p, st));
    c->launches += 2;
    *total = at;
    return CG_OK;
}

static bool gzip_dest(int gzip_outputs, bool demux, int d)
{
    return (demux || d == 0) ? (gzip_outputs & CG_GZIP_MAIN) != 0 : ((gzip_outputs >> (d - 1)) & 1) != 0;
}

static int gzip_check(const cg_fastq_params *fp, const char *who)
{
    if (fp->gzip_outputs & ~(CG_GZIP_MAIN | 7))
        return fail(CG_EINVAL, std::string(who) + ": gzip_outputs takes CG_GZIP_MAIN and CG_REDIRECT_* bits only");
    return CG_OK;
}

static int fastq_stage_output(cg_ctx *c, FastqSlot &f, const FqStage &g, cudaStream_t st, uint8_t *out,
                              int64_t out_capacity, cg_fastq_result *res, const FqDemux *dm = nullptr,
                              int64_t *segments = nullptr, const FqSplit *sp = nullptr, int gzip_outputs = 0)
{
    const long long n = g.n;
    int rc;
    long long total = 0;
    if (dm || sp) {
        rc = fastq_partition(c, f, n, dm ? dm->n_dest() : FqSplit::n_dest, f.d_outlen.p, dm ? dm->d_dest : sp->d_route,
                             segments, &total, st);
        if (rc != CG_OK) return rc;
    } else {
        CU(cg_launch_scan_i32(f.d_outlen.p, n, f.d_scan.p, f.d_outoff.p, st));
        c->launches += 3;
        CU(cudaMemcpyAsync(&total, f.d_outoff.p + n, sizeof total, cudaMemcpyDeviceToHost, st));
    }
    if ((rc = fastq_stage_result(f, g, st, res)) != CG_OK) return rc;
    res->out_bytes = res->out_bytes_plain = total;
    if (gzip_outputs && total > 0) {
        const int n_dest = dm ? dm->n_dest() : sp ? FqSplit::n_dest : 1;
        std::vector<int64_t> bounds{0, (int64_t)total};
        if (segments) bounds.assign(segments, segments + n_dest + 1);
        std::vector<char> gz((size_t)n_dest);
        for (int d = 0; d < n_dest; ++d) gz[(size_t)d] = gzip_dest(gzip_outputs, dm != nullptr, d);
        if ((rc = f.d_out.ensure((size_t)total + 64)) != CG_OK) return rc;
        if ((rc = fastq_write_records(c, f, g, f.d_out.p, sp, segments, st)) != CG_OK) return rc;
        long long packed = 0;
        if ((rc = fastq_gzip(c, f, f.d_out.p, bounds, gz, &packed, st)) != CG_OK) return rc;
        res->out_bytes = packed;
        if (packed > out_capacity)
            return fail(CG_EINVAL, "cg_fastq_collect: output buffer too small (" + std::to_string(packed) + " bytes needed)");
        if (!out) return fail(CG_EINVAL, "cg_fastq_collect: out is NULL");
        if (segments) std::copy(bounds.begin(), bounds.end(), segments);
        return fastq_copy_out(c, f, out, f.d_gzout.p, packed, st);
    }
    if (total > out_capacity)
        return fail(CG_EINVAL, "cg_fastq_collect: output buffer too small (" + std::to_string(total) + " bytes needed)");
    if (total > 0) {
        if (!out) return fail(CG_EINVAL, "cg_fastq_collect: out is NULL");
        if ((rc = f.d_out.ensure((size_t)total + 64)) != CG_OK) return rc;
        if ((rc = fastq_write_records(c, f, g, f.d_out.p, sp, segments, st)) != CG_OK) return rc;
        if ((rc = fastq_copy_out(c, f, out, f.d_out.p, total, st)) != CG_OK) return rc;
    }
    return CG_OK;
}

static int fastq_stage_output_interleaved(cg_ctx *c, FastqSlot &f1, const FqStage &g1, FastqSlot &f2, const FqStage &g2,
                                          cudaStream_t st, uint8_t *out1, int64_t out_capacity1, uint8_t *out2,
                                          int64_t out_capacity2, cg_fastq_result *res1, cg_fastq_result *res2,
                                          int64_t *segments1, int64_t *segments2, const FqSplit &sp, int gzip1, int gzip2)
{
    const long long n = g1.n;
    int rc;
    if ((rc = f1.d_fold.ensure((size_t)n)) != CG_OK) return rc;
    if ((rc = f2.d_fold.ensure((size_t)n)) != CG_OK) return rc;
    CU(cg_launch_fastq_interleave(0, n, sp.d_route, sp.ilv_dests, f1.d_outlen.p, f2.d_outlen.p, f1.d_fold.p, f2.d_fold.p,
                                  nullptr, nullptr, nullptr, st));
    c->launches += 1;
    long long total1 = 0, total2 = 0;
    if ((rc = fastq_partition(c, f1, n, FqSplit::n_dest, f1.d_fold.p, sp.d_route, segments1, &total1, st)) != CG_OK) return rc;
    if ((rc = fastq_partition(c, f2, n, FqSplit::n_dest, f2.d_fold.p, sp.d_route, segments2, &total2, st)) != CG_OK) return rc;
// ... 519 lines not shown
```

### cutadapt_b200/csrc/cg_args.h

```cpp
#pragma once
#include "cg_core.cuh"

#ifndef CG_NT
#define CG_NT 128
#endif

struct CgKernelArgs {
    const uint8_t *blob;
    uint32_t blob_bytes;
    const uint64_t *masks64;
    const uint8_t *enc;
    const uint8_t *index;
    const uint8_t *seq;
    const uint8_t *qual;
    const int64_t *offsets;
    long long n_reads;
    int quality_trim, cutoff_front, cutoff_back, qbase, times, slots;
    cg_match_rec *out;
    int32_t *qtrim;
    const int32_t *view;
    int *err_flag;
    int tile_cap;
    int col_rows;
    int mini_cap;
    int carry_slot;
    int task_rec;
    uint4 *tasks;
    unsigned long long *task_count;
    unsigned long long *task_count_b;
    long long task_cap;
    uint4 *tasks2;
    unsigned long long *task2_count;
    unsigned long long *task2_count_b;
    uint4 *tasks3;
    unsigned long long *task3_count;
    int no_band;
    unsigned long long *stats;
    int stats_max_len, stats_kmax;
    uint32_t *scratch_p;
    int *scratch_w;
    long long scratch_stride;
};
```

### cutadapt_b200/csrc/cg_kernels.cu

```cuda
#include <atomic>

#include "cg_kernels.cuh"
#include "cg_device.cuh"
#include "cg_pscan.cuh"

struct FastSmem {
    size_t bar_off, cnt_off, task_off, blob_off, enc_off, seq_off, qual_off, col_off, total;
};
__host__ __device__ inline FastSmem fast_smem_layout(uint32_t blob_bytes, int tile_cap, int col_rows, bool has_qual)
{
    FastSmem L;
    size_t o = 0;
    L.bar_off = o; o += 16;
    L.cnt_off = o; o += 16;
    o = cg_align_up(o, 128);
    L.task_off = o; o += CG_NT * 32;
    L.blob_off = o; o += cg_align_up(blob_bytes, 16);
    L.enc_off = o; o += 768;
    o = cg_align_up(o, 128);
    L.seq_off = o; o += 2 * (size_t)tile_cap;
    L.qual_off = o; if (has_qual) o += 2 * (size_t)tile_cap;
    o = cg_align_up(o, 128);
    L.col_off = o; o += (size_t)col_rows * CG_NT * sizeof(uint32_t);
    L.total = cg_align_up(o, 128);
// ... 360 lines not shown
                }
                if (a.qtrim) { a.qtrim[2 * r] = ts; a.qtrim[2 * r + 1] = te; }
                if (a.view) { ts = a.view[2 * r]; te = a.view[2 * r + 1]; }
                t_off = off + (uint32_t)ts; t_len = (uint32_t)(te - ts);
                const ScanOut sc = simple_scan(S, tile_seq + t_off, (int)t_len, &gs);
                pass = sc.pass; hits = sc.hits; rs0 = sc.rs0; rs1 = sc.rs1;
                if (!pass) {
                    CgHit none; none.adapter = -1; none.remove = 0;
                    none.astart = none.astop = none.rstart = none.rstop = none.score = none.errors = 0;
                    store_hit(a.out + (size_t)r * a.slots, none, 0, 0);
                }
            }
            const uint32_t ballot = __ballot_sync(0xffffffffu, pass);
            c_new = __popc(ballot);
            if (pass) {
                const uint32_t idx = __popc(ballot & ((1u << lane) - 1u));
                meta_new[2 * idx] = make_uint4((uint32_t)(tile_seq - smem) + t_off, t_len, hits, (uint32_t)gs);
                meta_new[2 * idx + 1] = make_uint4(rs0, rs1, (uint32_t)((unsigned long long)r & 0xffffffffu),
                                                   (uint32_t)((unsigned long long)r >> 32));
            }
            __syncwarp();
        }
        const int total = c_old + c_new;
        const bool flush = !have_tile;
        int first_left = 0, n_left = c_new;
        int carry_at = c_old;
        if (total >= 32 || flush) {
            const bool has_task = lane < total;
            uint4 ma = make_uint4(0, 0, 0, 4), mb = make_uint4(0, 0, 0, 0);
            if (has_task) {
                if (lane < c_old) { ma = meta_carry[2 * lane]; mb = meta_carry[2 * lane + 1]; }
                else { ma = meta_new[2 * (lane - c_old)]; mb = meta_new[2 * (lane - c_old) + 1]; }
            }
            warp_dp_pass(S, smem, ma, mb, has_task, a.out, a.slots);
            __syncwarp();
            first_left = 32 - c_old;
            n_left = total >= 32 ? total - 32 : 0;
            carry_at = 0;
            c_old = 0;
        }
        for (int j = 0; j < n_left; ++j) {
            const uint4 ma = meta_new[2 * (first_left + j)];
            const uint4 mb = meta_new[2 * (first_left + j) + 1];
            const uint32_t src = ma.x & ~15u;
            const uint32_t nch = ((ma.x & 15u) + ma.y + 15u) >> 4;
            uint8_t *dst = s_carry + (size_t)(carry_at + j) * a.carry_slot;
            if ((uint32_t)lane < nch) ((uint4 *)dst)[lane] = ((const uint4 *)(smem + src))[lane];
            if (lane == 0) {
                meta_carry[2 * (carry_at + j)] = make_uint4((uint32_t)(dst - smem) + (ma.x & 15u), ma.y, ma.z, ma.w);
                meta_carry[2 * (carry_at + j) + 1] = mb;
            }
        }
        c_old = carry_at + n_left;
        __syncwarp();
        if (have_tile) {
            if (lane == 0) {
                const long long next = mt + 2 * warps_total;
                if (next < n_mt) issue(next, st);
            }
            mt += warps_total;
            ++it;
        }
    }
}

cudaError_t cg_warp_occupancy(bool has_qual, size_t smem, int *blocks_per_sm)
{
    void (*k)(const CgKernelArgs) = has_qual ? cg_trim_warp_kernel<true> : cg_trim_warp_kernel<false>;
    cudaError_t e = cudaFuncSetAttribute(k, cudaFuncAttributeMaxDynamicSharedMemorySize, (int)smem);
    if (e != cudaSuccess) return e;
    return cudaOccupancyMaxActiveBlocksPerMultiprocessor(blocks_per_sm, k, CG_NT, smem);
}

cudaError_t cg_launch_warp(const CgKernelArgs &a, bool has_qual, int grid, size_t smem, cudaStream_t st)
{
    if (has_qual) cg_trim_warp_kernel<true><<<grid, CG_NT, smem, st>>>(a);
    else cg_trim_warp_kernel<false><<<grid, CG_NT, smem, st>>>(a);
    return cudaGetLastError();
}

#ifndef CG_SCAN_STAGES
#define CG_SCAN_STAGES 1
#endif
__host__ __device__ inline ScanSmem scan_smem_layout(uint32_t blob_bytes, int mini_cap, bool has_qual)
{
    ScanSmem L;
    size_t o = 0;
    L.blob_off = o; o += cg_align_up(blob_bytes, 16);
    L.enc_off = o; o += 768;
    o = cg_align_up(o, 128);
    L.warp_off = o;
    size_t w = 0;
    L.bar_rel = w; w += 16;
    w = cg_align_up(w, 128);
    L.seq_rel = w; w += CG_SCAN_STAGES * (size_t)mini_cap;
    L.qual_rel = w; if (has_qual) w += CG_SCAN_STAGES * (size_t)mini_cap;
    L.warp_stride = cg_align_up(w, 128);
    L.total = L.warp_off + (CG_NT / 32) * L.warp_stride;
    return L;
}
size_t cg_scan_smem_bytes(uint32_t blob_bytes, int mini_cap, bool has_qual)
{
    return scan_smem_layout(blob_bytes, mini_cap, has_qual).total;
}

template <bool HAS_QUAL>
__global__ void __launch_bounds__(CG_NT) cg_scan_kernel(const CgKernelArgs a)
{
    extern __shared__ __align__(128) uint8_t smem[];
    const ScanSmem L = scan_smem_layout(a.blob_bytes, a.mini_cap, HAS_QUAL);
    uint8_t *s_blob = smem + L.blob_off;
    uint8_t *s_enc = smem + L.enc_off;
    const int tid = threadIdx.x, lane = tid & 31, wib = tid >> 5;
    uint8_t *wbase = smem + L.warp_off + (size_t)wib * L.warp_stride;
    uint64_t *bars = (uint64_t *)(wbase + L.bar_rel);
    uint8_t *s_seq = wbase + L.seq_rel;
    uint8_t *s_qual = wbase + L.qual_rel;

    for (uint32_t i = tid; i < a.blob_bytes / 16; i += CG_NT) ((uint4 *)s_blob)[i] = ((const uint4 *)a.blob)[i];
    for (uint32_t i = tid; i < 768 / 16; i += CG_NT) ((uint4 *)s_enc)[i] = ((const uint4 *)a.enc)[i];
    if (lane == 0) {
        mbar_init(&bars[0], 1);
        mbar_init(&bars[1], 1);
        fence_barrier_init();
    }
    __syncthreads();
    const SetView S = make_set_view(s_blob, a.masks64, s_enc, a.index);

    const bool fold_ascii = scan_checks_ascii(S.scan, S.h->scan_count);
    const long long n_reads = a.n_reads;
    const long long n_mt = (n_reads + 31) / 32;
    const long long warps_total = (long long)gridDim.x * (CG_NT / 32);
    const long long wg = (long long)blockIdx.x * (CG_NT / 32) + wib;
    const uintptr_t seq_base = (uintptr_t)a.seq, qual_base = (uintptr_t)a.qual;

    auto issue = [&](long long mt, int st) {
        const long long r0 = mt * 32;
        const long long r1 = (r0 + 32 < n_reads) ? r0 + 32 : n_reads;
        const long long b0 = a.offsets[r0], b1 = a.offsets[r1];
        if (b1 <= b0) return;
        const uintptr_t sa0 = (seq_base + b0) & ~(uintptr_t)15;
        const uint32_t bytes = (uint32_t)(((seq_base + b1 + 15) & ~(uintptr_t)15) - sa0);
        uint32_t qbytes = 0;
        uintptr_t qa0 = 0;
        if (HAS_QUAL) {
            qa0 = (qual_base + b0) & ~(uintptr_t)15;
            qbytes = (uint32_t)(((qual_base + b1 + 15) & ~(uintptr_t)15) - qa0);
        }
        mbar_expect_tx(&bars[st], bytes + qbytes);
        tma_load_1d(s_seq + (size_t)st * a.mini_cap, (const void *)sa0, bytes, &bars[st]);
        if (HAS_QUAL) tma_load_1d(s_qual + (size_t)st * a.mini_cap, (const void *)qa0, qbytes, &bars[st]);
    };
    if (lane == 0) {
        if (wg < n_mt) issue(wg, 0);
        if (CG_SCAN_STAGES > 1 && wg + warps_total < n_mt) issue(wg + warps_total, 1);
    }
    uint32_t phase0 = 0, phase1 = 0;
    int it = 0;
    for (long long mt = wg; mt < n_mt; mt += warps_total, ++it) {
        const int st = CG_SCAN_STAGES > 1 ? (it & 1) : 0;
        const long long r0 = mt * 32;
        const long long r1 = (r0 + 32 < n_reads) ? r0 + 32 : n_reads;
        const long long r = r0 + lane;
        const long long b0 = a.offsets[r0], b1 = a.offsets[r1];
        long long o0 = 0, o1 = 0;
        if (r < n_reads) { o0 = a.offsets[r]; o1 = a.offsets[r + 1]; }
        const uintptr_t sa0 = (seq_base + b0) & ~(uintptr_t)15;
        const uint8_t *tile_seq = s_seq + (size_t)st * a.mini_cap;
        const uint8_t *tile_qual = s_qual + (size_t)st * a.mini_cap;
        if (b1 > b0) {
            if (st == 0) { mbar_wait(&bars[0], phase0); phase0 ^= 1; }
            else { mbar_wait(&bars[1], phase1); phase1 ^= 1; }
        }
        if (b1 > b0 && !fold_ascii) {
            const uint32_t head = (uint32_t)((seq_base + b0) - sa0);
            const uint32_t body = (uint32_t)(b1 - b0);
            const uint32_t nchunks = (head + body + 15) / 16;
            uint32_t bad = 0;
            const bool edge_first = mt == 0, edge_last = mt == n_mt - 1;
            for (uint32_t c = lane; c < nchunks; c += 32) {
                const uint4 v = ((const uint4 *)tile_seq)[c];
                if ((c == 0 && edge_first) || (c == nchunks - 1 && edge_last)) {
                    const uint8_t *pb = tile_seq + 16 * c;
                    for (uint32_t b = 0; b < 16; ++b) {
                        const uint32_t idx = 16 * c + b;
                        if (idx >= head && idx < head + body) bad |= pb[b];
                    }
                } else bad |= v.x | v.y | v.z | v.w;
            }
            if (bad & 0x80808080u) atomicOr(a.err_flag, 1);
        }
        bool pass = false;
        uint32_t hits = 0, rs0 = 0, rs1 = 0;
        int gs = 4, ts = 0, te = 0;
        if (r < n_reads) {
            const int n = (int)(o1 - o0);
            const uint32_t off = (uint32_t)((seq_base + o0) - sa0);
            ts = 0; te = n;
            if (HAS_QUAL) {
                const uintptr_t qa0 = (qual_base + b0) & ~(uintptr_t)15;
                const uint8_t *q = tile_qual + (size_t)((qual_base + o0) - qa0);
                if (a.quality_trim) pre_trim_core(tile_seq + off, q, n, a.quality_trim, a.cutoff_front, a.cutoff_back, a.qbase, &ts, &te);
            }
            if (a.qtrim) { a.qtrim[2 * r] = ts; a.qtrim[2 * r + 1] = te; }
            if (a.view) { ts = a.view[2 * r]; te = a.view[2 * r + 1]; }
            const ScanOut sc = simple_scan(S, tile_seq + off + ts, te - ts, &gs);
            pass = sc.pass; hits = sc.hits; rs0 = sc.rs0; rs1 = sc.rs1;
            if (fold_ascii && (sc.bad & 0x80808080u)) atomicOr(a.err_flag, 1);
            if (!pass) {
                CgHit none; none.adapter = -1; none.remove = 0;
                none.astart = none.astop = none.rstart = none.rstop = none.score = none.errors = 0;
                store_hit(a.out + (size_t)r * a.slots, none, 0, 0);
            }
        }
        const uint32_t ballot = __ballot_sync(0xffffffffu, pass);
        if (ballot) {
            unsigned long long base = 0;
            if (lane == 0) base = atomicAdd(a.task_count, (unsigned long long)__popc(ballot));
            base = __shfl_sync(0xffffffffu, base, 0);
            if (pass) {
                const unsigned long long slot = base + __popc(ballot & ((1u << lane) - 1u));
                const unsigned long long woff = (unsigned long long)(o0 + ts);
                a.tasks[2 * slot] = make_uint4((uint32_t)r, (uint32_t)(woff >> 32), (uint32_t)woff, (uint32_t)(te - ts));
                a.tasks[2 * slot + 1] = make_uint4(hits, (uint32_t)gs, rs0, rs1);
            }
        }
        __syncwarp();
        if (lane == 0) {
            const long long next = mt + (long long)CG_SCAN_STAGES * warps_total;
            if (next < n_mt) issue(next, st);
        }
    }
}

cudaError_t cg_scan_occupancy(bool has_qual, size_t smem, int *blocks_per_sm)
{
    void (*k)(const CgKernelArgs) = has_qual ? cg_scan_kernel<true> : cg_scan_kernel<false>;
    cudaError_t e = cudaFuncSetAttribute(k, cudaFuncAttributeMaxDynamicSharedMemorySize, (int)smem);
    if (e != cudaSuccess) return e;
    return cudaOccupancyMaxActiveBlocksPerMultiprocessor(blocks_per_sm, k, CG_NT, smem);
}
cudaError_t cg_launch_scan(const CgKernelArgs &a, bool has_qual, int grid, size_t smem, cudaStream_t st)
{
    if (has_qual) cg_scan_kernel<true><<<grid, CG_NT, smem, st>>>(a);
    else cg_scan_kernel<false><<<grid, CG_NT, smem, st>>>(a);
    return cudaGetLastError();
}

#include "cg_pscan.cuh"

size_t cg_pscan_smem_bytes(uint32_t blob_bytes, int mini_cap, bool has_qual, int stats_max_len)
{
    return pscan_smem_layout(blob_bytes, mini_cap, has_qual, stats_max_len).total;
}

template <bool HAS_QUAL, int W, bool STATS>
__global__ void __launch_bounds__(CG_NT, W <= 5 ? CG_PSCAN_BLOCKS : 5) cg_pscan_kernel(const CgKernelArgs a)
{
    cg_pscan_body<HAS_QUAL, W, RuntimePlaneProg, STATS>(a);
}

typedef void (*pscan_kernel_t)(const CgKernelArgs);
static pscan_kernel_t pick_pscan(bool has_qual, int w, bool stats)
{
    if (stats) return w <= 5 ? cg_pscan_kernel<false, 5, true> : cg_pscan_kernel<false, 8, true>;
    if (w <= 5) return has_qual ? cg_pscan_kernel<true, 5, false> : cg_pscan_kernel<false, 5, false>;
    return has_qual ? cg_pscan_kernel<true, 8, false> : cg_pscan_kernel<false, 8, false>;
}
cudaError_t cg_pscan_occupancy(bool has_qual, int w, bool stats, size_t smem, int *blocks_per_sm)
{
    pscan_kernel_t k = pick_pscan(has_qual, w, stats);
    cudaError_t e = cudaFuncSetAttribute(k, cudaFuncAttributeMaxDynamicSharedMemorySize, (int)smem);
    if (e != cudaSuccess) return e;
    return cudaOccupancyMaxActiveBlocksPerMultiprocessor(blocks_per_sm, k, CG_NT, smem);
}
cudaError_t cg_launch_pscan(const CgKernelArgs &a, bool has_qual, int w, int grid, size_t smem, cudaStream_t st)
{
    pick_pscan(has_qual, w, a.stats != nullptr)<<<grid, CG_NT, smem, st>>>(a);
    return cudaGetLastError();
}

#ifndef CG_LIST_STAGES
#define CG_LIST_STAGES 1
#endif
struct DpSmem { size_t blob_off, enc_off, warp_off, warp_stride, bar_rel, slot_rel, total; };
__host__ __device__ inline DpSmem dp_smem_layout(uint32_t blob_bytes, int slot_bytes)
{
    DpSmem L;
    size_t o = 0;
    L.blob_off = o; o += cg_align_up(blob_bytes, 16);
    L.enc_off = o; o += 768;
    o = cg_align_up(o, 128);
    L.warp_off = o;
    size_t w = 0;
    L.bar_rel = w; w += 16;
    w = cg_align_up(w, 128);
    L.slot_rel = w; w += CG_LIST_STAGES * 32 * (size_t)slot_bytes;
    L.warp_stride = cg_align_up(w, 128);
    L.total = L.warp_off + (CG_NT / 32) * L.warp_stride;
    return L;
}
size_t cg_dp_smem_bytes(uint32_t blob_bytes, int slot_bytes) { return dp_smem_layout(blob_bytes, slot_bytes).total; }

#ifndef CG_PLAN_BLOCKS
#define CG_PLAN_BLOCKS 6
#endif
#ifndef CG_RUN16_BLOCKS
#define CG_RUN16_BLOCKS 4
#endif
#ifndef CG_RUN48_BLOCKS
#define CG_RUN48_BLOCKS 3
#endif
template <bool PLAN, int MR>
__global__ void __launch_bounds__(CG_NT, PLAN ? CG_PLAN_BLOCKS : (MR <= 16 ? CG_RUN16_BLOCKS : (MR <= 32 ? 3 : (MR <= 48 ? CG_RUN48_BLOCKS : 2)))) cg_list_kernel(const CgKernelArgs a)
{
    extern __shared__ __align__(128) uint8_t smem[];
    const int slot_bytes = a.carry_slot;
    const DpSmem L = dp_smem_layout(a.blob_bytes, slot_bytes);
    uint8_t *s_blob = smem + L.blob_off;
    uint8_t *s_enc = smem + L.enc_off;
    const int tid = threadIdx.x, lane = tid & 31, wib = tid >> 5;
    uint8_t *wbase = smem + L.warp_off + (size_t)wib * L.warp_stride;
    uint8_t *s_slot = wbase + L.slot_rel;

    for (uint32_t i = tid; i < a.blob_bytes / 16; i += CG_NT) ((uint4 *)s_blob)[i] = ((const uint4 *)a.blob)[i];
    for (uint32_t i = tid; i < 768 / 16; i += CG_NT) ((uint4 *)s_enc)[i] = ((const uint4 *)a.enc)[i];
    __syncthreads();
    const SetView S = make_set_view(s_blob, a.masks64, s_enc, a.index);
    const CgAdapter &A = S.ad[0];

    unsigned long long n_tasks = *a.task_count;
    if (n_tasks > (unsigned long long)a.task_cap) n_tasks = (unsigned long long)a.task_cap;
    unsigned long long n_tasks_b = a.task_count_b ? *a.task_count_b : 0ull;
    if (n_tasks + n_tasks_b > (unsigned long long)a.task_cap) n_tasks_b = (unsigned long long)a.task_cap - n_tasks;
    const long long n_groups_a = (long long)((n_tasks + 31) / 32);
    const uint4 *list = a.tasks;
    const int rec = PLAN ? a.task_rec : 4;
    const long long n_groups = n_groups_a + (long long)((n_tasks_b + 31) / 32);
    const long long warps_total = (long long)gridDim.x * (CG_NT / 32);
    const long long wg = (long long)blockIdx.x * (CG_NT / 32) + wib;
    const uintptr_t seq_base = (uintptr_t)a.seq;

    struct Task { uint4 ta, tb, tc, td; uintptr_t src; uint32_t bytes, soff; };
    auto task_index = [&](long long g) -> long long {
        if (g < n_groups_a) {
            const unsigned long long t = (unsigned long long)g * 32 + lane;
            return t < n_tasks ? (long long)t : -1;
        }
        const unsigned long long t = (unsigned long long)(g - n_groups_a) * 32 + lane;
        return t < n_tasks_b ? (long long)a.task_cap - 1 - (long long)t : -1;
    };
    auto load_task = [&](long long g, Task &T) {
        const long long t = task_index(g);
        T.ta = make_uint4(0, 0, 0, 0); T.tb = make_uint4(0, 4, 0, 0); T.tc = make_uint4(0, 0, 0, 0); T.td = make_uint4(0, 0, 0, 0);
        T.src = 0; T.bytes = 0; T.soff = 0;
        if (t < 0) return;
        T.ta = list[rec * t]; T.tb = list[rec * t + 1];
        if (!PLAN || rec >= 4) { T.tc = list[rec * t + 2]; T.td = list[rec * t + 3]; }
        if (PLAN && (T.tb.y & CG_TASK_BYTES)) {
            T.src = (uintptr_t)(list + rec * t + 4);
            T.bytes = 16u * (uint32_t)(rec - 4);
            T.soff = T.td.y;
            return;
        }
        uintptr_t addr = seq_base + (uintptr_t)(((unsigned long long)T.ta.y << 32) | T.ta.z);
        uint32_t len = T.ta.w;
        if (!PLAN) {
            const int n = (int)T.ta.w, ri = (int)T.tc.z;
            const uint32_t pk = ri == 0 ? T.td.x : (ri == 1 ? T.td.y : (ri == 2 ? T.td.z : T.td.w));
            const int lo = (int)(pk & 0xffffu), hi = (int)(pk >> 16);
            len = hi > lo ? (uint32_t)(hi - lo) : 0u;
            if (len) addr += (uintptr_t)(A.reverse ? n - hi : lo);
        }
        T.src = addr & ~(uintptr_t)15;
        T.bytes = len ? (uint32_t)(((addr + len + 15) & ~(uintptr_t)15) - T.src) : 0u;
        T.soff = (uint32_t)(addr - T.src);
    };
    auto stage = [&](const Task &T) {
        uint8_t *dst = s_slot + (size_t)lane * slot_bytes;
        for (uint32_t o = 0; o < T.bytes; o += 16) cp_async16(dst + o, (const void *)(T.src + o));
        cp_async_commit();
    };

    Task next;
    if (wg < n_groups) load_task(wg, next);
    for (long long g = wg; g < n_groups; g += warps_total) {
        const Task cur = next;
        stage(cur);
        if (g + warps_total < n_groups) load_task(g + warps_total, next);
        cp_async_wait<0>();
        const uint4 ta = cur.ta, tb = cur.tb, tc = cur.tc, td = cur.td;
        const uint32_t soff = cur.soff;
        const int st = 0;
        const bool has_task = task_index(g) >= 0;
        const uint8_t *p = s_slot + ((size_t)st * 32 + lane) * slot_bytes + soff;
        const int n = (int)ta.w;
        const long long r = (long long)ta.x;
        CgHit hit;
        hit.adapter = -1; hit.remove = 0;
        hit.astart = hit.astop = hit.rstart = hit.rstop = hit.score = hit.errors = 0;
        bool cont = false, cont_b = false, defer = false;
        uint4 ob = make_uint4(0, 0, 0, 0), oc = make_uint4(0, 0, 0, 0), od = make_uint4(0, 0, 0, 0);
        if (PLAN) {
            if (has_task) {
                RunPlan P;
                P.n_runs = 0; P.exact = 0; P.s0 = 0; P.end_idx = -1; P.banded = 0;
                uint32_t hits = tb.x, rs0 = tb.z, rs1 = tb.w;
                int gs = (int)(tb.y & 0xffu);
                bool pass = true;
                bool planned = false;
                if (tb.y & CG_TASK_PLANES) {
                    if (window_is_plain(p, n)) {
                        const uint32_t M[8] = {tb.x, tb.z, tb.w, tc.x, tc.y, tc.z, tc.w, td.x};
                        const int W = (int)((tb.y >> 12) & 15u);
                        plan_runs_planes(S, p, n, M, W, (int)((tb.y >> 20) & 1u), (int)((tb.y >> 21) & 1u), 32 * W - n, P);
                        planned = true;
                    } else {
                        defer = true;
                        pass = false;
                    }
                } else if (tb.y & CG_TASK_RESCAN) {
                    const ScanOut sc = simple_scan(S, p, n, &gs);
                    pass = sc.pass; hits = sc.hits; rs0 = sc.rs0; rs1 = sc.rs1;
                }
                if (planned) {}
                else if (pass) plan_runs(S, p, n, hits, gs, rs0, rs1, P);
                if (P.exact == 2) hit_end_overlap(A, n, P.s0, hit);
                else if (P.exact) hit_exact(A, n, P.s0, hit);
                else if (P.n_runs > 0) {
                    cont = true;
                    oc = make_uint4((uint32_t)A.m, (uint32_t)n, 0u, (uint32_t)P.n_runs | ((uint32_t)(P.end_idx & 15) << 8) |
                                                                   ((P.banded && !a.no_band) ? 1u << 16 : 0u));
                    cont_b = a.task2_count_b != nullptr &&
                             run_band_d(A, n, P.lo0, P.hi0, P.banded != 0 && !a.no_band, P.end_idx == 0) < 0;
                    od = make_uint4((uint32_t)P.lo0 | ((uint32_t)P.hi0 << 16), (uint32_t)P.lo1 | ((uint32_t)P.hi1 << 16),
                                    (uint32_t)P.lo2 | ((uint32_t)P.hi2 << 16), (uint32_t)P.lo3 | ((uint32_t)P.hi3 << 16));
                }
            }
        } else {
            const int ri = (int)tc.z, n_runs = (int)(tc.w & 255u);
            int end_idx = (int)((tc.w >> 8) & 15u);
            if (end_idx == 15) end_idx = -1;
            const uint32_t pk = ri == 0 ? td.x : (ri == 1 ? td.y : (ri == 2 ? td.z : td.w));
            const int lo = (int)(pk & 0xffffu), hi = (int)(pk >> 16);
            LocState ls;
            ls.have = (int)tb.x; ls.b_origin = (int)tb.y; ls.b_cost = (int)tb.z; ls.b_score = (int)tb.w;
            ls.b_ref_stop = (int)tc.x; ls.b_q_stop = (int)tc.y; ls.stopped = 0;
            const bool last = ri == n_runs - 1;
            const int band = has_task ? run_band_d(A, n, lo, hi, (tc.w >> 16) & 1u, ri == end_idx) : -1;
            run_pass<MR>(S, p, n, lo, hi, ri != end_idx, last, has_task, ls, band);
            if (has_task) {
                if (ls.stopped || last) hit_from_state(A, n, ls, hit);
                else {
                    cont = true;
                    ob = make_uint4((uint32_t)ls.have, (uint32_t)ls.b_origin, (uint32_t)ls.b_cost, (uint32_t)ls.b_score);
                    oc = make_uint4((uint32_t)ls.b_ref_stop, (uint32_t)ls.b_q_stop, (uint32_t)(ri + 1), tc.w);
                    od = td;
                }
            }
        }
        if (has_task && !cont && !defer) store_hit(a.out + (size_t)r * a.slots, hit, 0, n);
        if (PLAN) {
            const uint32_t dballot = __ballot_sync(0xffffffffu, defer);
            if (dballot) {
                unsigned long long base = 0;
                if (lane == 0) base = atomicAdd(a.task3_count, (unsigned long long)__popc(dballot));
                base = __shfl_sync(0xffffffffu, base, 0);
                if (defer) {
                    const unsigned long long slot = base + __popc(dballot & ((1u << lane) - 1u));
                    a.tasks3[2 * slot] = ta;
                    a.tasks3[2 * slot + 1] = make_uint4(0u, 4u | CG_TASK_RESCAN, 0u, 0u);
                }
            }
        }
        const uint32_t ballot = __ballot_sync(0xffffffffu, cont && !cont_b);
        const uint32_t ballot_b = __ballot_sync(0xffffffffu, cont && cont_b);
        if (ballot | ballot_b) {
            unsigned long long base = 0, base_b = 0;
            if (lane == 0) {
                if (ballot) base = atomicAdd(a.task2_count, (unsigned long long)__popc(ballot));
                if (ballot_b) base_b = atomicAdd(a.task2_count_b, (unsigned long long)__popc(ballot_b));
            }
            base = __shfl_sync(0xffffffffu, base, 0);
            base_b = __shfl_sync(0xffffffffu, base_b, 0);
            if (cont) {
                const uint32_t below = (1u << lane) - 1u;
                const unsigned long long slot = cont_b ? (unsigned long long)a.task_cap - 1ull - (base_b + __popc(ballot_b & below))
                                                       : base + __popc(ballot & below);
                a.tasks2[4 * slot] = ta;
                a.tasks2[4 * slot + 1] = ob;
                a.tasks2[4 * slot + 2] = oc;
                a.tasks2[4 * slot + 3] = od;
            }
        }
        __syncwarp();
    }
}

typedef void (*list_kernel_t)(const CgKernelArgs);
static list_kernel_t pick_list(bool plan, int mr)
{
    if (plan) return cg_list_kernel<true, 16>;
    if (mr <= 16) return cg_list_kernel<false, 16>;
    if (mr <= 32) return cg_list_kernel<false, 32>;
    if (mr <= 40) return cg_list_kernel<false, 40>;
    return mr <= 48 ? cg_list_kernel<false, 48> : cg_list_kernel<false, 64>;
}
cudaError_t cg_list_occupancy(bool plan, int mr, size_t smem, int *blocks_per_sm)
{
    list_kernel_t k = pick_list(plan, mr);
    cudaError_t e = cudaFuncSetAttribute(k, cudaFuncAttributeMaxDynamicSharedMemorySize, (int)smem);
    if (e != cudaSuccess) return e;
    return cudaOccupancyMaxActiveBlocksPerMultiprocessor(blocks_per_sm, k, CG_NT, smem);
}
cudaError_t cg_launch_list(const CgKernelArgs &a, bool plan, int mr, int grid, size_t smem, cudaStream_t st)
{
    pick_list(plan, mr)<<<grid, CG_NT, smem, st>>>(a);
    return cudaGetLastError();
}

__device__ __forceinline__ cg_match_rec load_rec(const cg_match_rec *p)
{
    const int4 a = __ldg((const int4 *)p), b = __ldg((const int4 *)p + 1);
    cg_match_rec r;
    r.adapter = a.x; r.astart = a.y; r.astop = a.z; r.rstart = a.w;
    r.rstop = b.x; r.score = b.y; r.errors = b.z; r.info = b.w;
    return r;
}
__device__ __forceinline__ void store_rec(cg_match_rec *p, const cg_match_rec &r)
{
    ((int4 *)p)[0] = make_int4(r.adapter, r.astart, r.astop, r.rstart);
    ((int4 *)p)[1] = make_int4(r.rstop, r.score, r.errors, r.info);
}

__global__ void cg_linked_view_kernel(const cg_match_rec *front, const int32_t *base_view, const int64_t *offsets,
                                      long long n_reads, int32_t *out_view)
{
    const long long r = (long long)blockIdx.x * blockDim.x + threadIdx.x;
    if (r >= n_reads) return;
    int s = 0, e;
    if (base_view) { s = base_view[2 * r]; e = base_view[2 * r + 1]; }
    else e = (int)(offsets[r + 1] - offsets[r]);
    linked_view(load_rec(front + r), s, e);
    *(int2 *)(out_view + 2 * r) = make_int2(s, e);
}
cudaError_t cg_launch_linked_view(const cg_match_rec *front, const int32_t *base_view, const int64_t *offsets,
                                  long long n_reads, int32_t *out_view, cudaStream_t st)
{
    const int block = 256;
    cg_linked_view_kernel<<<(unsigned)((n_reads + block - 1) / block), block, 0, st>>>(front, base_view, offsets,
                                                                                     n_reads, out_view);
    return cudaGetLastError();
}

__global__ void cg_select_kernel(const CgSelectArgs a)
{
    const long long r = (long long)blockIdx.x * blockDim.x + threadIdx.x;
    if (r >= a.n_reads) return;
    cg_match_rec b0, b1;
    select_best(a.t, a.pass_map, [&](int pass) { return load_rec(a.tmp + (size_t)pass * a.stride + r); }, b0, b1);
    cg_match_rec *dst = a.out + (size_t)r * a.t.slots;
    store_rec(dst, b0);
    if (a.t.slots > 1) store_rec(dst + 1, b1);
}
cudaError_t cg_launch_select(const CgSelectArgs &a, cudaStream_t st)
{
    const int block = 256;
    cg_select_kernel<<<(unsigned)((a.n_reads + block - 1) / block), block, 0, st>>>(a);
    return cudaGetLastError();
}

__global__ void cg_trim_generic_kernel(const CgKernelArgs a)
{
    const long long gtid = (long long)blockIdx.x * blockDim.x + threadIdx.x;
    const long long nthreads = (long long)gridDim.x * blockDim.x;
    const SetView S = make_set_view(a.blob, a.masks64, a.enc, a.index);
    PackedCol colp; colp.base = a.scratch_p + gtid; colp.stride = (int)a.scratch_stride;
    WideCol colw; colw.base = a.scratch_w + gtid; colw.stride = a.scratch_stride;
    for (long long r = gtid; r < a.n_reads; r += nthreads) {
        const long long o0 = a.offsets[r], o1 = a.offsets[r + 1];
        const int n = (int)(o1 - o0);
        const uint8_t *p = a.seq + o0;
        uint32_t bad = 0;
        for (int i = 0; i < n; ++i) bad |= p[i];
        if (bad & 0x80) atomicOr(a.err_flag, 1);
        process_read<true>(S, p, a.qual ? a.qual + o0 : nullptr, n, a.qual ? a.quality_trim : 0,
                           a.cutoff_front, a.cutoff_back, a.qbase, a.times, colp, colw,
                           a.out + (size_t)r * a.times * a.slots, a.qtrim ? a.qtrim + 2 * r : nullptr,
                                    a.view ? a.view + 2 * r : nullptr);
    }
}

__global__ void __launch_bounds__(CG_NT) cg_trim_light_kernel(const CgKernelArgs a)
{
    const SetView S = make_set_view(a.blob, a.masks64, a.enc, a.index);
    uint32_t lcol[CG_LIGHT_ROWS];
    PackedCol colp; colp.base = lcol; colp.stride = 1;
    WideCol colw; colw.base = nullptr; colw.stride = 0;
    const int lane = threadIdx.x & 31;
    const long long n_reads = a.n_reads;
    const long long n_mt = (n_reads + 31) / 32;
    const long long warps_total = (long long)gridDim.x * (CG_NT / 32);
    const uintptr_t seq_base = (uintptr_t)a.seq;
    for (long long mt = (long long)blockIdx.x * (CG_NT / 32) + (threadIdx.x >> 5); mt < n_mt; mt += warps_total) {
        const long long r0 = mt * 32;
        const long long r1 = (r0 + 32 < n_reads) ? r0 + 32 : n_reads;
        const long long r = r0 + lane;
        const uintptr_t s = seq_base + (uintptr_t)a.offsets[r0], e = seq_base + (uintptr_t)a.offsets[r1];
        const uintptr_t as = (s + 15) & ~(uintptr_t)15, ae = e & ~(uintptr_t)15;
        uint32_t bad = 0;
        if (as >= ae) {
            for (uintptr_t q = s + lane; q < e; q += 32) bad |= *(const uint8_t *)q;
        } else {
            for (uintptr_t q = s + lane; q < as; q += 32) bad |= *(const uint8_t *)q;
            for (uintptr_t q = ae + lane; q < e; q += 32) bad |= *(const uint8_t *)q;
            for (uintptr_t q = as + 16u * lane; q < ae; q += 512) {
                const uint4 v = *(const uint4 *)q;
                bad |= v.x | v.y | v.z | v.w;
            }
        }
        if (bad & 0x80808080u) atomicOr(a.err_flag, 1);
        if (r < n_reads) {
            const long long o0 = a.offsets[r], o1 = a.offsets[r + 1];
            process_read<false>(S, a.seq + o0, nullptr, (int)(o1 - o0), 0, 0, 0, a.qbase, a.times, colp, colw,
                                a.out + (size_t)r * a.times * a.slots, nullptr, a.view ? a.view + 2 * r : nullptr);
        }
    }
}

cudaError_t cg_launch_light(const CgKernelArgs &a, int grid, cudaStream_t st)
{
    cg_trim_light_kernel<<<grid, CG_NT, 0, st>>>(a);
    return cudaGetLastError();
}

__global__ void __launch_bounds__(CG_NT) cg_index_kernel(const CgKernelArgs a)
{
    const SetView S = make_set_view(a.blob, a.masks64, a.enc, a.index);
    PackedCol colp; colp.base = nullptr; colp.stride = 0;
    WideCol colw; colw.base = nullptr; colw.stride = 0;
    const int lane = threadIdx.x & 31;
    const long long n_reads = a.n_reads;
    const long long n_mt = (n_reads + 31) / 32;
    const long long warps_total = (long long)gridDim.x * (CG_NT / 32);
    const uintptr_t seq_base = (uintptr_t)a.seq;
    uint32_t *slow_list = (uint32_t *)a.tasks;
    for (long long mt = (long long)blockIdx.x * (CG_NT / 32) + (threadIdx.x >> 5); mt < n_mt; mt += warps_total) {
        const long long r0 = mt * 32;
        const long long r1 = (r0 + 32 < n_reads) ? r0 + 32 : n_reads;
        const long long r = r0 + lane;
        const uintptr_t s = seq_base + (uintptr_t)a.offsets[r0], e = seq_base + (uintptr_t)a.offsets[r1];
        const uintptr_t as = (s + 15) & ~(uintptr_t)15, ae = e & ~(uintptr_t)15;
        uint32_t bad = 0;
        if (as >= ae) {
            for (uintptr_t q = s + lane; q < e; q += 32) bad |= *(const uint8_t *)q;
        } else {
            for (uintptr_t q = s + lane; q < as; q += 32) bad |= *(const uint8_t *)q;
            for (uintptr_t q = ae + lane; q < e; q += 32) bad |= *(const uint8_t *)q;
            for (uintptr_t q = as + 16u * lane; q < ae; q += 512) {
                const uint4 v = *(const uint4 *)q;
                bad |= v.x | v.y | v.z | v.w;
            }
        }
        if (bad & 0x80808080u) atomicOr(a.err_flag, 1);
        bool slow = false;
        if (r < n_reads) {
            const long long o0 = a.offsets[r], o1 = a.offsets[r + 1];
            const int n = (int)(o1 - o0);
            CgHit best; best.adapter = -1; best.remove = 0;
            best.astart = best.astop = best.rstart = best.rstop = best.score = best.errors = 0;
            int best_group = 0;
            bool have = false;
            for (int g = 0; g < S.h->n_groups && !slow; ++g) {
                CgHit h;
                if (!match_indexed<false>(S, S.gr[g].a0, a.seq + o0, n, colp, colw, h, &slow)) continue;
                if (!have || h.score > best.score || (h.score == best.score && h.errors < best.errors)) {
                    have = true; best = h; best_group = g;
                }
            }
            if (!slow) store_hit(a.out + (size_t)r * a.slots, best, have ? best_group : 0, have ? n : 0);
        }
        const uint32_t ballot = __ballot_sync(0xffffffffu, slow);
        if (ballot) {
            unsigned long long base = 0;
            if (lane == 0) base = atomicAdd(a.task_count, (unsigned long long)__popc(ballot));
            base = __shfl_sync(0xffffffffu, base, 0);
            if (slow) slow_list[base + __popc(ballot & ((1u << lane) - 1u))] = (uint32_t)r;
        }
    }
}

__global__ void __launch_bounds__(CG_NT) cg_trim_listed_kernel(const CgKernelArgs a)
{
    const SetView S = make_set_view(a.blob, a.masks64, a.enc, a.index);
    uint32_t lcol[CG_LIGHT_ROWS];
    PackedCol colp; colp.base = lcol; colp.stride = 1;
    WideCol colw; colw.base = nullptr; colw.stride = 0;
    const uint32_t *list = (const uint32_t *)a.tasks;
    const unsigned long long n_listed = *a.task_count;
    const long long nthreads = (long long)gridDim.x * blockDim.x;
    for (long long i = (long long)blockIdx.x * blockDim.x + threadIdx.x; i < (long long)n_listed; i += nthreads) {
        const long long r = (long long)list[i];
        const long long o0 = a.offsets[r], o1 = a.offsets[r + 1];
        process_read<false>(S, a.seq + o0, nullptr, (int)(o1 - o0), 0, 0, 0, a.qbase, 1, colp, colw,
                            a.out + (size_t)r * a.slots, nullptr, nullptr);
    }
}

int cg_device_sm_count()
{
    static std::atomic<int> cached[64];
    int dev = 0, sms = 0;
    if (cudaGetDevice(&dev) != cudaSuccess) return 1;
    if (dev >= 0 && dev < 64 && (sms = cached[dev].load(std::memory_order_relaxed)) > 0) return sms;
    if (cudaDeviceGetAttribute(&sms, cudaDevAttrMultiProcessorCount, dev) != cudaSuccess || sms < 1) return 1;
    if (dev >= 0 && dev < 64) cached[dev].store(sms, std::memory_order_relaxed);
    return sms;
}

cudaError_t cg_launch_index(const CgKernelArgs &a, int grid, cudaStream_t st)
{
    cg_index_kernel<<<grid, CG_NT, 0, st>>>(a);
    cudaError_t e = cudaGetLastError();
    if (e != cudaSuccess) return e;
    cg_trim_listed_kernel<<<cg_device_sm_count(), CG_NT, 0, st>>>(a);
    return cudaGetLastError();
}

__global__ void cg_locate_debug_kernel(const uint8_t *blob, const uint8_t *enc768, const uint8_t *query, int n,
                                       int *scratch , int32_t *cost, int32_t *score, int32_t *result8)
{
    if (threadIdx.x || blockIdx.x) return;
    const SetView S = make_set_view(blob, nullptr, enc768, nullptr);
    const CgAdapter &A = S.ad[0];
    ReadView rv; rv.p = query; rv.n = n; rv.rev = 0;
    WideCol col; col.base = scratch; col.stride = 1;
    int o[6] = {0, 0, 0, 0, 0, 0};
    const bool found = locate_core<WideCell, WideCol>(A, S.pool + A.ref_off, (const int32_t *)(S.pool + A.ncount_off),
                                                      (const int32_t *)(S.pool + A.maxcost_off), enc768 + 256 * A.query_enc,
                                                      rv, col, o, 0xFFFFFFFFu, 0, cost, score);
    result8[0] = found ? 1 : 0;
    for (int i = 0; i < 6; ++i) result8[1 + i] = o[i];
    result8[7] = 0;
}

cudaError_t cg_launch_locate_debug(const uint8_t *d_blob, const uint8_t *d_enc, const uint8_t *d_query, int n,
                                   int *d_scratch, int32_t *d_cost, int32_t *d_score, int32_t *d_result, cudaStream_t st)
{
    cg_locate_debug_kernel<<<1, 32, 0, st>>>(d_blob, d_enc, d_query, n, d_scratch, d_cost, d_score, d_result);
    return cudaGetLastError();
}

cudaError_t cg_launch_generic(const CgKernelArgs &a, int grid, int block, cudaStream_t st)
{
    cg_trim_generic_kernel<<<grid, block, 0, st>>>(a);
    return cudaGetLastError();
}

__global__ void cg_kmers_present_kernel(const CgEntry *ents, int n_entries, const uint64_t *masks,
                                        const uint8_t *seq, const int64_t *offsets, long long n_reads,
                                        uint8_t *out, int *err)
{
    const long long nthreads = (long long)gridDim.x * blockDim.x;
    for (long long r = (long long)blockIdx.x * blockDim.x + threadIdx.x; r < n_reads; r += nthreads) {
        ReadView rv; rv.p = seq + offsets[r]; rv.n = (int)(offsets[r + 1] - offsets[r]); rv.rev = 0;
        uint32_t bad = 0;
        for (int i = 0; i < rv.n; ++i) bad |= rv.p[i];
        if (bad & 0x80) atomicOr(err, 1);
        out[r] = kmers_present_core(ents, n_entries, masks, rv) ? 1 : 0;
    }
}

cudaError_t cg_launch_kmers_present(const CgEntry *d_entries, int n_entries, const uint64_t *d_masks,
                                    const uint8_t *d_seq, const int64_t *d_offsets, long long n_reads,
                                    uint8_t *d_out, int *d_err, cudaStream_t st)
{
    const int block = 128;
    long long grid = (n_reads + block - 1) / block;
    grid = cg_grid_cap(grid, 16);
    if (grid < 1) grid = 1;
    cg_kmers_present_kernel<<<(int)grid, block, 0, st>>>(d_entries, n_entries, d_masks, d_seq, d_offsets,
                                                         n_reads, d_out, d_err);
    return cudaGetLastError();
}

__global__ void cg_quality_trim_kernel(const uint8_t *qual, const int64_t *offsets, long long n_reads,
                                       int cutoff_front, int cutoff_back, int base, int32_t *out)
{
    const long long nthreads = (long long)gridDim.x * blockDim.x;
    for (long long r = (long long)blockIdx.x * blockDim.x + threadIdx.x; r < n_reads; r += nthreads) {
        int s, e;
        quality_trim_core(qual + offsets[r], (int)(offsets[r + 1] - offsets[r]), cutoff_front, cutoff_back,
                          base, &s, &e);
        out[2 * r] = s; out[2 * r + 1] = e;
    }
}

cudaError_t cg_launch_quality_trim(const uint8_t *d_qual, const int64_t *d_offsets, long long n_reads,
                                   int cutoff_front, int cutoff_back, int base, int32_t *d_out,
                                   cudaStream_t st)
{
    const int block = 128;
    long long grid = (n_reads + block - 1) / block;
    grid = cg_grid_cap(grid, 16);
    if (grid < 1) grid = 1;
    cg_quality_trim_kernel<<<(int)grid, block, 0, st>>>(d_qual, d_offsets, n_reads, cutoff_front,
                                                        cutoff_back, base, d_out);
    return cudaGetLastError();
}

__global__ void cg_nextseq_trim_kernel(const uint8_t *seq, const uint8_t *qual, const int64_t *offsets,
                                       long long n_reads, int cutoff, int base, int32_t *out)
{
    const long long nthreads = (long long)gridDim.x * blockDim.x;
    for (long long r = (long long)blockIdx.x * blockDim.x + threadIdx.x; r < n_reads; r += nthreads) {
        const long long o = offsets[r];
        out[r] = nextseq_trim_core(seq + o, qual + o, (int)(offsets[r + 1] - o), cutoff, base);
    }
}
__global__ void cg_poly_a_trim_kernel(const uint8_t *seq, const int64_t *offsets, long long n_reads, int revcomp,
                                      int32_t *out, int *err_flag)
{
    const long long nthreads = (long long)gridDim.x * blockDim.x;
    for (long long r = (long long)blockIdx.x * blockDim.x + threadIdx.x; r < n_reads; r += nthreads) {
        const long long o = offsets[r];
        const int n = (int)(offsets[r + 1] - o);
        out[r] = poly_a_trim_core(seq + o, n, revcomp);
    }
    (void)err_flag;
}
__global__ void cg_expected_errors_kernel(const uint8_t *qual, const int64_t *offsets, long long n_reads, int base,
                                          const double *table, double *out)
{
    __shared__ double s_table[256];
    for (int i = threadIdx.x; i < 256; i += blockDim.x) s_table[i] = table[i];
    __syncthreads();
    const long long nthreads = (long long)gridDim.x * blockDim.x;
    for (long long r = (long long)blockIdx.x * blockDim.x + threadIdx.x; r < n_reads; r += nthreads) {
        const long long o = offsets[r];
        out[r] = expected_errors_core(qual + o, (int)(offsets[r + 1] - o), base, s_table);
    }
}
cudaError_t cg_launch_expected_errors(const uint8_t *d_qual, const int64_t *d_offsets, long long n_reads, int base,
                                      const double *d_table, double *d_out, cudaStream_t st)
{
    const int block = 128;
    long long grid = (n_reads + block - 1) / block;
    grid = cg_grid_cap(grid, 16);
    if (grid < 1) grid = 1;
    cg_expected_errors_kernel<<<(int)grid, block, 0, st>>>(d_qual, d_offsets, n_reads, base, d_table, d_out);
    return cudaGetLastError();
}
cudaError_t cg_launch_nextseq_trim(const uint8_t *d_seq, const uint8_t *d_qual, const int64_t *d_offsets,
                                   long long n_reads, int cutoff, int base, int32_t *d_out, cudaStream_t st)
{
    const int block = 128;
    long long grid = (n_reads + block - 1) / block;
    grid = cg_grid_cap(grid, 16);
    if (grid < 1) grid = 1;
    cg_nextseq_trim_kernel<<<(int)grid, block, 0, st>>>(d_seq, d_qual, d_offsets, n_reads, cutoff, base, d_out);
    return cudaGetLastError();
}
cudaError_t cg_launch_poly_a_trim(const uint8_t *d_seq, const int64_t *d_offsets, long long n_reads, int revcomp,
                                  int32_t *d_out, cudaStream_t st)
{
    const int block = 128;
    long long grid = (n_reads + block - 1) / block;
    grid = cg_grid_cap(grid, 16);
    if (grid < 1) grid = 1;
    cg_poly_a_trim_kernel<<<(int)grid, block, 0, st>>>(d_seq, d_offsets, n_reads, revcomp, d_out, nullptr);
    return cudaGetLastError();
}

__global__ void cg_fill_offsets_kernel(int64_t *out, long long base, long long len, long long count)
{
    const long long i = (long long)blockIdx.x * blockDim.x + threadIdx.x;
    if (i < count) out[i] = base + i * len;
}
cudaError_t cg_launch_fill_offsets(int64_t *d_out, long long base, long long len, long long count, cudaStream_t st)
{
    const int block = 256;
    cg_fill_offsets_kernel<<<(unsigned)((count + block - 1) / block), block, 0, st>>>(d_out, base, len, count);
    return cudaGetLastError();
}

__global__ void __launch_bounds__(256) cg_unpack3_kernel(const uint4 *__restrict__ packed, uint4 *__restrict__ out,
                                                          long long n_vec)
{
    __shared__ uint32_t lut[256];
    {
        const uint32_t ch = 0x41u | (0x43u << 8) | (0x47u << 16) | (0x54u << 24);
        const int i = threadIdx.x;
        const int v0 = i / 36, v1 = (i / 6) % 6, v2 = i % 6;
        auto chr = [&](int v) -> uint32_t { return v < 4 ? (ch >> (8 * v)) & 0xFFu : (v == 4 ? 0x4Eu : 0x41u); };
        lut[i] = chr(v0) | (chr(v1) << 8) | (chr(v2) << 16);
    }
    __syncthreads();
    const long long stride = (long long)gridDim.x * blockDim.x;
    for (long long i = (long long)blockIdx.x * blockDim.x + threadIdx.x; i < n_vec; i += stride) {
        const uint4 p = __ldg(packed + i);
        const uint32_t w[4] = {p.x, p.y, p.z, p.w};
        uint32_t o[12];
#pragma unroll
        for (int k = 0; k < 4; ++k) {
            const uint32_t t0 = lut[w[k] & 0xFFu], t1 = lut[(w[k] >> 8) & 0xFFu];
            const uint32_t t2 = lut[(w[k] >> 16) & 0xFFu], t3 = lut[w[k] >> 24];
            o[3 * k + 0] = t0 | (t1 << 24);
            o[3 * k + 1] = (t1 >> 8) | (t2 << 16);
            o[3 * k + 2] = (t2 >> 16) | (t3 << 8);
        }
        out[3 * i + 0] = make_uint4(o[0], o[1], o[2], o[3]);
        out[3 * i + 1] = make_uint4(o[4], o[5], o[6], o[7]);
        out[3 * i + 2] = make_uint4(o[8], o[9], o[10], o[11]);
    }
}
__global__ void cg_unpack_fix_kernel(const unsigned long long *__restrict__ exc, long long n_exc, uint8_t *out)
{
    const long long i = (long long)blockIdx.x * blockDim.x + threadIdx.x;
    if (i < n_exc) {
        const unsigned long long e = exc[i];
        out[e >> 8] = (uint8_t)(e & 0xFFu);
    }
}
cudaError_t cg_launch_unpack3(const uint8_t *d_packed, long long packed_bytes, uint8_t *d_out,
                              const unsigned long long *d_exc, long long n_exc, cudaStream_t st)
{
    const long long n_vec = packed_bytes / 16;
    if (n_vec > 0) {
        const int block = 256;
        long long grid = (n_vec + block - 1) / block;
        grid = cg_grid_cap(grid, 8);
        cg_unpack3_kernel<<<(int)grid, block, 0, st>>>((const uint4 *)d_packed, (uint4 *)d_out, n_vec);
        cudaError_t e = cudaGetLastError();
        if (e != cudaSuccess) return e;
    }
    if (n_exc > 0) {
        const int block = 256;
        cg_unpack_fix_kernel<<<(unsigned)((n_exc + block - 1) / block), block, 0, st>>>(d_exc, n_exc, d_out);
    }
    return cudaGetLastError();
}

__global__ void cg_max_len_kernel(const int64_t *offsets, long long n_reads, int *out)
{
    const long long nthreads = (long long)gridDim.x * blockDim.x;
    int best = 0;
    for (long long r = (long long)blockIdx.x * blockDim.x + threadIdx.x; r < n_reads; r += nthreads) {
        const long long d = offsets[r + 1] - offsets[r];
        const int v = d > 2147483647LL ? 2147483647 : (int)d;
        best = v > best ? v : best;
    }
    for (int o = 16; o > 0; o >>= 1) {
        const int other = __shfl_xor_sync(0xffffffffu, best, o);
        best = other > best ? other : best;
    }
    if ((threadIdx.x & 31) == 0) atomicMax(out, best);
}

cudaError_t cg_launch_max_len(const int64_t *d_offsets, long long n_reads, int *d_out, cudaStream_t st)
{
    const int block = 256;
    long long grid = (n_reads + block - 1) / block;
    grid = cg_grid_cap(grid, 8);
    if (grid < 1) grid = 1;
    cg_max_len_kernel<<<(int)grid, block, 0, st>>>(d_offsets, n_reads, d_out);
    return cudaGetLastError();
}

template <bool SMEM_HIST>
__global__ void cg_stats_kernel(const uint8_t *seq, const int64_t *offsets, long long n_reads, int quality_trim, int times,
                                int slots, const cg_match_rec *matches, const int32_t *qtrim,
                                int n_adapters, int max_len, int kmax, unsigned long long *stats,
                                const uint4 *task_list, int task_rec, const unsigned long long *task_count,
                                int count_lengths, int upper)
{
    extern __shared__ unsigned int s_hist[];
    const long long nbins = cg_stats_total(n_adapters, max_len, kmax) - CG_STATS_SCALARS;
    const long long n_local = SMEM_HIST ? nbins : (count_lengths ? (long long)(max_len + 1) : 0);
    for (long long i = threadIdx.x; i < n_local; i += blockDim.x) s_hist[i] = 0;
    __syncthreads();
    const long long nthreads = (long long)gridDim.x * blockDim.x;
    unsigned long long n = 0;
    StatsScalars sc; sc.bp = sc.with_adapters = sc.qtrim_bp = sc.adapter_bp = 0;
    unsigned long long *hist = stats + CG_STATS_SCALARS;
    long long n_items = n_reads;
    if (task_list) {
        const unsigned long long t = *task_count;
        n_items = t < (unsigned long long)n_reads ? (long long)t : n_reads;
    }
    for (long long i = (long long)blockIdx.x * blockDim.x + threadIdx.x; i < n_items; i += nthreads) {
        long long r = i;
        if (task_list) {
            const uint4 t = task_list[(size_t)task_rec * i];
            r = (long long)t.x;
        }
        const long long o0 = offsets[r];
        const int len = (int)(offsets[r + 1] - o0);
        n += 1;
        const bool hq = quality_trim && qtrim;
        stats_read_core(seq ? seq + o0 : nullptr, len, hq, hq ? qtrim[2 * r] : 0, hq ? qtrim[2 * r + 1] : len,
                        matches + (size_t)r * times * slots, times, slots, n_adapters, max_len, kmax, sc,
                        [&](long long idx, unsigned int v) {
                            if (!count_lengths && idx <= max_len) return;
                            if (idx < n_local) atomicAdd(&s_hist[idx], v);
                            else atomicAdd(&hist[idx], (unsigned long long)v);
                        },
                        upper != 0);
    }
    for (int o = 16; o > 0; o >>= 1) {
        n += __shfl_xor_sync(0xffffffffu, n, o);
        sc.bp += __shfl_xor_sync(0xffffffffu, sc.bp, o);
        sc.with_adapters += __shfl_xor_sync(0xffffffffu, sc.with_adapters, o);
        sc.qtrim_bp += __shfl_xor_sync(0xffffffffu, sc.qtrim_bp, o);
        sc.adapter_bp += __shfl_xor_sync(0xffffffffu, sc.adapter_bp, o);
    }
    if ((threadIdx.x & 31) == 0) {
        atomicAdd(&stats[0], n); atomicAdd(&stats[1], sc.bp); atomicAdd(&stats[2], sc.with_adapters);
        atomicAdd(&stats[3], sc.qtrim_bp); atomicAdd(&stats[4], sc.adapter_bp);
    }
    __syncthreads();
    for (long long i = threadIdx.x; i < n_local; i += blockDim.x) {
        const unsigned int v = s_hist[i];
        if (v) atomicAdd(&hist[i], (unsigned long long)v);
    }
}

cudaError_t cg_launch_stats(const uint8_t *d_seq, const int64_t *d_offsets, long long n_reads, int quality_trim, int times,
                            int slots, const cg_match_rec *d_matches, const int32_t *d_qtrim,
                            int n_adapters, int max_len, int kmax, unsigned long long *d_stats,
                            cudaStream_t st, const uint4 *d_task_list, int task_rec, const unsigned long long *d_task_count,
                            int count_lengths, int upper)
{
    const int block = 256;
    long long grid = (n_reads + block - 1) / block;
    grid = cg_grid_cap(grid, 8);
    if (grid < 1) grid = 1;
    const size_t hist_bytes = (size_t)(cg_stats_total(n_adapters, max_len, kmax) - CG_STATS_SCALARS) * sizeof(unsigned int);
    const size_t len_bytes = count_lengths ? (size_t)(max_len + 1) * sizeof(unsigned int) : 0;
    if (len_bytes > 48 * 1024) return cudaErrorInvalidValue;
    if (hist_bytes <= 48 * 1024 && n_reads / grid < (1LL << 31))
        cg_stats_kernel<true><<<(int)grid, block, hist_bytes, st>>>(d_seq, d_offsets, n_reads, quality_trim, times, slots,
                                                                     d_matches, d_qtrim, n_adapters, max_len, kmax, d_stats,
                                                                     d_task_list, task_rec, d_task_count, count_lengths,
                                                                     upper);
    else
        cg_stats_kernel<false><<<(int)grid, block, len_bytes, st>>>(d_seq, d_offsets, n_reads, quality_trim, times, slots,
                                                                     d_matches, d_qtrim, n_adapters, max_len, kmax, d_stats,
                                                                     d_task_list, task_rec, d_task_count, count_lengths,
                                                                     upper);
    return cudaGetLastError();
}
```

### cutadapt_b200/csrc/cg_kernels.cuh

```cuda
#pragma once
#include <cuda_runtime.h>
#include <stdint.h>

#include "cg_core.cuh"

#include "cg_args.h"

int cg_device_sm_count();
static inline long long cg_grid_cap(long long grid, int blocks_per_sm)
{
    const long long cap = (long long)blocks_per_sm * cg_device_sm_count();
    return grid > cap ? cap : grid;
}

struct CgSelectArgs {
    const cg_match_rec *tmp;
    long long stride;
    long long n_reads;
    cg_match_rec *out;
    const int32_t *pass_map;
    CgSelectTables t;
};
cudaError_t cg_launch_select(const CgSelectArgs &a, cudaStream_t st);
cudaError_t cg_launch_linked_view(const cg_match_rec *front, const int32_t *base_view, const int64_t *offsets,
                                  long long n_reads, int32_t *out_view, cudaStream_t st);

size_t cg_fast_smem_bytes(uint32_t blob_bytes, int tile_cap, int col_rows, bool has_qual);
cudaError_t cg_launch_fast(const CgKernelArgs &a, bool has_qual, bool simple, int grid, size_t smem, cudaStream_t st);
cudaError_t cg_fast_occupancy(bool has_qual, bool simple, size_t smem, int *blocks_per_sm);
size_t cg_warp_smem_bytes(uint32_t blob_bytes, int mini_cap, int carry_slot, bool has_qual);
cudaError_t cg_warp_occupancy(bool has_qual, size_t smem, int *blocks_per_sm);
cudaError_t cg_launch_warp(const CgKernelArgs &a, bool has_qual, int grid, size_t smem, cudaStream_t st);
size_t cg_scan_smem_bytes(uint32_t blob_bytes, int mini_cap, bool has_qual);
cudaError_t cg_scan_occupancy(bool has_qual, size_t smem, int *blocks_per_sm);
cudaError_t cg_launch_scan(const CgKernelArgs &a, bool has_qual, int grid, size_t smem, cudaStream_t st);
#define CG_LIGHT_ROWS 68
cudaError_t cg_launch_light(const CgKernelArgs &a, int grid, cudaStream_t st);
cudaError_t cg_launch_index(const CgKernelArgs &a, int grid, cudaStream_t st);
size_t cg_pscan_smem_bytes(uint32_t blob_bytes, int mini_cap, bool has_qual, int stats_max_len = -1);
cudaError_t cg_pscan_occupancy(bool has_qual, int w, bool stats, size_t smem, int *blocks_per_sm);
cudaError_t cg_launch_pscan(const CgKernelArgs &a, bool has_qual, int w, int grid, size_t smem, cudaStream_t st);
size_t cg_dp_smem_bytes(uint32_t blob_bytes, int slot_bytes);
cudaError_t cg_list_occupancy(bool plan, int mr, size_t smem, int *blocks_per_sm);
cudaError_t cg_launch_list(const CgKernelArgs &a, bool plan, int mr, int grid, size_t smem, cudaStream_t st);
cudaError_t cg_launch_generic(const CgKernelArgs &a, int grid, int block, cudaStream_t st);
cudaError_t cg_launch_locate_debug(const uint8_t *d_blob, const uint8_t *d_enc, const uint8_t *d_query, int n,
                                   int *d_scratch, int32_t *d_cost, int32_t *d_score, int32_t *d_result, cudaStream_t st);
cudaError_t cg_launch_kmers_present(const CgEntry *d_entries, int n_entries, const uint64_t *d_masks,
                                    const uint8_t *d_seq, const int64_t *d_offsets, long long n_reads,
                                    uint8_t *d_out, int *d_err, cudaStream_t st);
cudaError_t cg_launch_quality_trim(const uint8_t *d_qual, const int64_t *d_offsets, long long n_reads,
                                   int cutoff_front, int cutoff_back, int base, int32_t *d_out,
                                   cudaStream_t st);
cudaError_t cg_launch_max_len(const int64_t *d_offsets, long long n_reads, int *d_out, cudaStream_t st);
cudaError_t cg_launch_stats(const uint8_t *d_seq, const int64_t *d_offsets, long long n_reads, int quality_trim, int times,
                            int slots, const cg_match_rec *d_matches, const int32_t *d_qtrim,
                            int n_adapters, int max_len, int kmax, unsigned long long *d_stats,
                            cudaStream_t st, const uint4 *d_task_list = nullptr, int task_rec = 0,
                            const unsigned long long *d_task_count = nullptr,
                            int count_lengths = 1,
                            int upper = 0);
cudaError_t cg_launch_nextseq_trim(const uint8_t *d_seq, const uint8_t *d_qual, const int64_t *d_offsets,
                                   long long n_reads, int cutoff, int base, int32_t *d_out, cudaStream_t st);
cudaError_t cg_launch_poly_a_trim(const uint8_t *d_seq, const int64_t *d_offsets, long long n_reads, int revcomp,
                                  int32_t *d_out, cudaStream_t st);
cudaError_t cg_launch_expected_errors(const uint8_t *d_qual, const int64_t *d_offsets, long long n_reads, int base,
                                      const double *d_table, double *d_out, cudaStream_t st);
cudaError_t cg_launch_fill_offsets(int64_t *d_out, long long base, long long len, long long count, cudaStream_t st);
cudaError_t cg_launch_unpack3(const uint8_t *d_packed, long long packed_bytes, uint8_t *d_out,
                              const unsigned long long *d_exc, long long n_exc, cudaStream_t st);

#include "cg_fastq_core.cuh"
#define CG_FQ_COUNTERS 16
long long cg_fastq_tiles(long long n_bytes);
long long cg_scan_tiles(long long n);
cudaError_t cg_launch_fastq_index(const uint8_t *d_buf, long long n_bytes, uint32_t *d_tile_counts,
                                  unsigned long long *d_total, uint32_t *d_nl_pos, int phase, cudaStream_t st);
cudaError_t cg_launch_fastq_records(const uint8_t *d_buf, long long n_bytes, const uint32_t *d_nl_pos, long long n_newlines,
                                    long long n_records, int cut_front, int cut_back, CgFastqRecord *d_rec,
                                    int32_t *d_seq_len, int32_t *d_origin, unsigned long long *d_counters, int *d_err,
                                    cudaStream_t st);
cudaError_t cg_launch_fasta_classify(const uint8_t *d_buf, long long n_bytes, const uint32_t *d_nl_pos, long long n_newlines,
                                     long long n_lines, int32_t *d_keep, int32_t *d_is_hdr, int *d_first_hdr, cudaStream_t st);
cudaError_t cg_launch_fasta_scatter(const uint8_t *d_buf, long long n_bytes, const uint32_t *d_nl_pos, long long n_newlines,
                                    long long n_lines, const int64_t *d_line_off, const int64_t *d_hdr_idx,
                                    const int *d_first_hdr, uint8_t *d_norm, CgFastqRecord *d_rec, int *d_err,
                                    cudaStream_t st);
cudaError_t cg_launch_fasta_records(CgFastqRecord *d_rec, long long n_records, long long n_norm, int cut_front, int cut_back,
                                    int32_t *d_seq_len, int32_t *d_origin, unsigned long long *d_counters, cudaStream_t st);
cudaError_t cg_launch_scan_i32(const int32_t *d_in, long long n, unsigned long long *d_tile_scratch, int64_t *d_out,
                               cudaStream_t st);
cudaError_t cg_launch_fastq_gather(const uint8_t *d_buf, const CgFastqRecord *d_rec, const int64_t *d_offsets,
                                   long long n_records, uint8_t *d_seq, uint8_t *d_qual, int rc, cudaStream_t st);
cudaError_t cg_launch_fastq_fold_qtrim(CgFastqRecord *d_rec, int32_t *d_seq_len, const int32_t *d_qtrim, long long n_records,
                                       int32_t *d_origin, unsigned long long *d_counters, cudaStream_t st);
cudaError_t cg_launch_fastq_revcomp_commit(uint8_t *d_buf, CgFastqRecord *d_rec, const int32_t *d_seq_len, int32_t *d_origin,
                                           long long n_records, cg_match_rec *d_matches, const cg_match_rec *d_matches_rc,
                                           int per_read, uint8_t *d_is_rc, unsigned long long *d_counters, cudaStream_t st,
                                           int has_qual = 1);
cudaError_t cg_launch_fastq_pretrim(const uint8_t *d_buf, const CgFastqRecord *d_rec, const int32_t *d_seq_len,
                                    long long n_records, int flags, int cutoff_front, int cutoff_back, int qbase,
                                    int32_t *d_qtrim, cudaStream_t st);
cudaError_t cg_launch_fastq_evaluate(const uint8_t *d_buf, const CgFastqRecord *d_rec, const int32_t *d_seq_len,
                                     long long n_records, const cg_match_rec *d_matches, int times, int slots,
                                     const int32_t *d_qtrim, CgFastqFilter f, const double *d_phred, const uint8_t *d_is_rc,
                                     int32_t *d_interval, int32_t *d_keep_interval, int32_t *d_fail_mask,
                                     unsigned long long *d_counters, int *d_err, cudaStream_t st,
                                     int32_t *d_poly_a_len = nullptr);
cudaError_t cg_launch_fastq_stats_tail(long long n_records, const int32_t *d_interval, const int32_t *d_out_len,
                                       const int32_t *d_poly_a_len, const cg_match_rec *d_matches, int times, int slots,
                                       const uint8_t *d_is_rc, int n_adapters, int max_len, unsigned long long *d_lengths,
                                       unsigned long long *d_poly_a, unsigned long long *d_rc, cudaStream_t st,
                                       const int32_t *d_route = nullptr);
cudaError_t cg_launch_fastq_finish(long long n_records, const CgFastqRecord *d_rec1, const int32_t *d_interval1,
                                   const int32_t *d_mask1, int enabled1, int32_t *d_out_len1,
                                   unsigned long long *d_counters1, const CgFastqRecord *d_rec2,
                                   const int32_t *d_interval2, const int32_t *d_mask2, int enabled2, int32_t *d_out_len2,
                                   unsigned long long *d_counters2, int mode, int mode_untrimmed, int rc_suffix,
                                   const int32_t *d_dest, const uint8_t *d_dest_keep, cudaStream_t st, int fasta_out = 0,
                                   int redirect = 0, int fasta_dests = 0, int32_t *d_route = nullptr);
cudaError_t cg_launch_fastq_write(const uint8_t *d_buf, const CgFastqRecord *d_rec, const int32_t *d_interval,
                                  const int64_t *d_out_off, const int32_t *d_out_len, long long n_records,
                                  uint8_t *d_out, int action, const int32_t *d_keep_interval, const int32_t *d_mask,
                                  int rc_suffix, cudaStream_t st, int fasta_out = 0, const int32_t *d_route = nullptr,
                                  int fasta_dests = 0);
long long cg_demux_tiles(long long n_records);
cudaError_t cg_launch_fastq_dest(const int32_t *d_mask1, const int32_t *d_mask2, long long n_records,
                                 const int32_t *d_adapter_dest1, int n_named1, const int32_t *d_adapter_dest2, int n_named2,
                                 int32_t *d_dest, cudaStream_t st);
cudaError_t cg_launch_fastq_demux(int phase, const int32_t *d_out_len, const int32_t *d_dest, long long n_records,
                                  int n_dest, int32_t *d_bytes, const int64_t *d_base, int64_t *d_out_off, cudaStream_t st);
cudaError_t cg_launch_fastq_info(int phase, const uint8_t *d_buf, const CgFastqRecord *d_rec, const int32_t *d_origin,
                                 const int32_t *d_interval, const int32_t *d_mask, const cg_match_rec *d_matches, int times,
                                 int slots, const uint8_t *d_names, const int32_t *d_name_off, int revcomp, int rc_suffix,
                                 int upper_unmatched, long long n_records, int32_t *d_row_bytes, const int64_t *d_row_off,
                                 uint8_t *d_out, cudaStream_t st, int kind = 0, const int32_t *d_qtrim = nullptr,
                                 const int32_t *d_seq_len = nullptr,
                                 int has_qual = 1);
cudaError_t cg_launch_interleaved_split(int phase, const uint8_t *d_buf, long long n_bytes, const uint32_t *d_nl_pos,
                                        long long n_newlines, long long n_records, CgFastqRecord *d_rec, int32_t *d_start,
                                        int32_t *d_size, int32_t *d_dest, unsigned long long *d_err, const int64_t *d_off,
                                        long long seg1, uint8_t *d_out1, uint8_t *d_out2, int fasta, cudaStream_t st);
cudaError_t cg_launch_fastq_interleave(int phase, long long n_records, const int32_t *d_route, int ilv,
                                       const int32_t *d_len1, const int32_t *d_len2, int32_t *d_fold1, int32_t *d_fold2,
                                       const int64_t *d_off1, int64_t *d_off2, const int64_t *d_total1, cudaStream_t st);
struct CgGzPiece {
    long long src;
    int32_t len;
    int32_t gz;
};
cudaError_t cg_launch_gzip_compress(const uint8_t *d_src, const CgGzPiece *d_pieces, int n_pieces, uint8_t *d_slots,
                                    int32_t *d_sizes, cudaStream_t st);
cudaError_t cg_launch_gzip_gather(const uint8_t *d_slots, const int32_t *d_sizes, const int64_t *d_dst_off, int n_pieces,
                                  uint8_t *d_out, cudaStream_t st);
#include "cg_gunzip_core.cuh"
long long cg_gunzip_tiles(long long n_bytes);
cudaError_t cg_launch_gunzip_candidates(int phase, const uint8_t *d_gz, long long n, int32_t *d_counts,
                                        const int64_t *d_offs, int32_t *d_cand, cudaStream_t st);
cudaError_t cg_launch_gunzip_parse(const uint8_t *d_gz, long long n, const int32_t *d_cand, int n_cand, long long budget,
                                   GuMember *d_res, cudaStream_t st);
cudaError_t cg_launch_gunzip_chain(const uint8_t *d_gz, long long n, const int32_t *d_cand, const GuMember *d_res,
                                   int n_cand, int after_member, int final, long long base, long long limit,
                                   int32_t *d_members, long long *d_moff, GuChain *d_chain, long long from, int split,
                                   cudaStream_t st);
cudaError_t cg_launch_gunzip_search(const uint8_t *d_gz, long long n, long long s0, long long stride, int K, GuChunk *d_ch,
                                    cudaStream_t st);
cudaError_t cg_launch_gunzip_spec(const uint8_t *d_gz, long long n, long long s0, long long stride, int K,
                                  const int32_t *d_list, int n_list, const long long *d_off, const long long *d_room,
                                  uint16_t *d_sym, GuChunk *d_ch, cudaStream_t st);
cudaError_t cg_launch_gunzip_walk(GuChunk *d_ch, int K, long long limit, int32_t *d_redo, GuWalk *d_walk, cudaStream_t st);
cudaError_t cg_launch_gunzip_resolve(const GuChunk *d_ch, int n_ok, long long max_n, const long long *d_off,
                                     const uint16_t *d_sym, uint8_t *d_win, long long mpos, uint8_t *d_out, int *d_bad,
                                     cudaStream_t st);
int cg_gunzip_crc_piece();
cudaError_t cg_launch_gunzip_crc(const uint8_t *d_plain, long long len, uint32_t *d_part, uint32_t *d_state,
                                 cudaStream_t st);
cudaError_t cg_launch_gunzip_place(const uint8_t *d_gz, long long n, const int32_t *d_cand, const int32_t *d_members,
                                   const long long *d_moff, const GuChain *d_chain, int n_members, const GuMember *d_res,
                                   uint8_t *d_out, int *d_bad, cudaStream_t st);
cudaError_t cg_launch_gunzip_flags(const uint8_t *d_buf, long long n, const uint32_t *d_nl, long long n_nl, int fasta,
                                   int32_t *d_flag, cudaStream_t st);
cudaError_t cg_launch_gunzip_select(const uint32_t *d_nl, long long n_nl, const int32_t *d_flag, const int64_t *d_offs,
                                    long long s, long long *d_cut, cudaStream_t st);
cudaError_t cg_launch_fastq_pair_select(long long n_records, int pair, const cg_match_rec *d_cur1, int slots1,
                                        const cg_match_rec *d_cur2, int slots2, cg_match_rec *d_best1, cg_match_rec *d_best2,
                                        int slots, int32_t *d_best_key, cudaStream_t st);
```

### cutadapt_b200/csrc/cg_pscan.cuh

```cuda
#pragma once
#include "cg_core.cuh"
#include "cg_args.h"
#include "cg_device.cuh"

struct ScanSmem { size_t blob_off, enc_off, stats_off, warp_off, warp_stride, bar_rel, seq_rel, qual_rel, total; };

#define CG_PSCAN_MARGIN 272
#ifndef CG_PSCAN_BLOCKS
#define CG_PSCAN_BLOCKS 8
#endif
#define CG_TASK_RESCAN 0x100u
#define CG_TASK_BYTES 0x400u
#define CG_TASK_PLANES 0x200u
__host__ __device__ inline ScanSmem pscan_smem_layout(uint32_t blob_bytes, int mini_cap, bool has_qual, int stats_max_len = -1)
{
    ScanSmem L;
    size_t o = 0;
    L.blob_off = o; o += cg_align_up(blob_bytes, 16);
    L.enc_off = o; o += 768;
    L.stats_off = o;
    if (stats_max_len >= 0) o += cg_align_up((size_t)(3 * (stats_max_len + 1) + 8) * sizeof(uint32_t), 8) + 8 * sizeof(unsigned long long);
    o = cg_align_up(o, 128);
    L.warp_off = o;
    size_t w = 0;
    L.bar_rel = w; w += 16;
    w = cg_align_up(w, 128);
    w += CG_PSCAN_MARGIN;
    L.seq_rel = w; w += (size_t)mini_cap;
    L.qual_rel = w; if (has_qual) w += (size_t)mini_cap;
    L.warp_stride = cg_align_up(w, 128);
    L.total = L.warp_off + (CG_NT / 32) * L.warp_stride;
    return L;
}

template <int DIR>
__device__ __forceinline__ int trim_scan_warp(uint32_t q_smem, int n, int cutoff, int base, int lane)
{
#if defined(__CUDA_ARCH__)
    int res = DIR > 0 ? 0 : n;
    bool more = false;
    if (n > 0) {
        const int d0 = cutoff - ((int)(signed char)cg_lds_u8(q_smem + (uint32_t)(DIR > 0 ? 0 : n - 1)) - base);
        more = d0 >= 0;
    }
    uint32_t todo = __ballot_sync(0xffffffffu, more);
    while (todo) {
        const int T = __ffs(todo) - 1;
        todo &= todo - 1;
        const uint32_t qT = __shfl_sync(0xffffffffu, q_smem, T);
        const int nT = __shfl_sync(0xffffffffu, n, T);
        int carry = 0, best = 0, resT = DIR > 0 ? 0 : nT;
        for (int j0 = 0; j0 < nT; j0 += 32) {
            const int j = j0 + lane;
            const bool valid = j < nT;
            int P = 0;
            if (valid) P = cutoff - ((int)(signed char)cg_lds_u8(qT + (uint32_t)(DIR > 0 ? j : nT - 1 - j)) - base);
#pragma unroll
            for (int o = 1; o < 32; o <<= 1) {
                const int t = __shfl_up_sync(0xffffffffu, P, o);
                if (lane >= o) P += t;
            }
            P += carry;
            const uint32_t neg = __ballot_sync(0xffffffffu, valid && P < 0);
            const int first_neg = neg ? __ffs(neg) - 1 : 32;
            const bool ok = valid && lane < first_neg;
            const int M = __reduce_max_sync(0xffffffffu, ok ? P : (int)0x80000000);
            if (M > best) {
                best = M;
                const int w = __ffs(__ballot_sync(0xffffffffu, ok && P == M)) - 1;
                resT = DIR > 0 ? j0 + w + 1 : nT - 1 - (j0 + w);
            }
            if (first_neg < 32) break;
            carry = __shfl_sync(0xffffffffu, P, 31);
        }
        if (lane == T) res = resT;
    }
    return res;
#else
    return 0;
#endif
}

__device__ __forceinline__ void pre_trim_warp(const uint8_t *seq, const uint8_t *qual, int n, int flags, int cutoff_front,
                                              int cutoff_back, int qbase, int lane, int *s_out, int *e_out)
{
    const int base = qbase & 255;
    int start = 0, stop = n;
    if (flags & 2) stop = nextseq_trim_core(seq, qual, n, qbase >> 8, base);
    if (flags & 1) {
        const uint32_t q_smem = (uint32_t)__cvta_generic_to_shared(qual);
        const int nq = stop;
        start = trim_scan_warp<+1>(q_smem, nq, cutoff_front, base, lane);
        stop = trim_scan_warp<-1>(q_smem, nq, cutoff_back, base, lane);
        if (start >= stop) { start = 0; stop = 0; }
    }
    *s_out = start; *e_out = stop;
}

template <bool HAS_QUAL, int W, class Prog, bool STATS = false>
__device__ __forceinline__ void cg_pscan_body(const CgKernelArgs &a)
{
    extern __shared__ __align__(128) uint8_t smem[];
    const ScanSmem L = pscan_smem_layout(a.blob_bytes, a.mini_cap, HAS_QUAL, (STATS && a.stats) ? a.stats_max_len : -1);
    uint8_t *s_blob = smem + L.blob_off;
    uint8_t *s_enc = smem + L.enc_off;
    const int tid = threadIdx.x, lane = tid & 31, wib = tid >> 5;
    uint8_t *wbase = smem + L.warp_off + (size_t)wib * L.warp_stride;
    uint64_t *bars = (uint64_t *)(wbase + L.bar_rel);
    uint8_t *s_seq = wbase + L.seq_rel;
    uint8_t *s_qual = wbase + L.qual_rel;
#define CG_PSCAN_STATS_VIEW                                                                                              \
    const int st_len = a.stats_max_len;                                                                                  \
    uint32_t *s_hlen = (uint32_t *)(smem + pscan_smem_layout(a.blob_bytes, a.mini_cap, HAS_QUAL, st_len).stats_off);     \
    uint32_t *s_hrem = s_hlen + (st_len + 1);              \
    uint32_t *s_hadj = s_hrem + 2 * (st_len + 1);                                                                        \
    unsigned long long *s_scal = (unsigned long long *)((uint8_t *)s_hlen + cg_align_up((size_t)(3 * (st_len + 1) + 8) * sizeof(uint32_t), 8));
    if (STATS && a.stats) {
        CG_PSCAN_STATS_VIEW
        (void)s_hrem; (void)s_hadj;
        for (int i = threadIdx.x; i < 3 * (st_len + 1) + 8; i += CG_NT) s_hlen[i] = 0;
        if (threadIdx.x < 8) s_scal[threadIdx.x] = 0;
    }
    for (uint32_t i = tid; i < a.blob_bytes / 16; i += CG_NT) ((uint4 *)s_blob)[i] = ((const uint4 *)a.blob)[i];
    for (uint32_t i = tid; i < 768 / 16; i += CG_NT) ((uint4 *)s_enc)[i] = ((const uint4 *)a.enc)[i];
    if (lane == 0) {
        mbar_init(&bars[0], 1);
        fence_barrier_init();
    }
    __syncthreads();
    const SetView S = make_set_view(s_blob, a.masks64, s_enc, a.index);
    const CgAdapter &A = S.ad[0];
    const uint32_t *prog = plane_program(S);
    const int n_prog = S.h->plane_count, pflags = S.h->plane_flags;
    const uint8_t *ref = S.pool + A.ref_off;
    const bool always_pass = A.pf_count == 0;

    const long long n_reads = a.n_reads;
    const long long n_mt = (n_reads + 31) / 32;
    const long long warps_total = (long long)gridDim.x * (CG_NT / 32);
    const long long wg = (long long)blockIdx.x * (CG_NT / 32) + wib;
    const uintptr_t seq_base = (uintptr_t)a.seq, qual_base = (uintptr_t)a.qual;

    auto issue = [&](long long mt) {
        const long long r0 = mt * 32;
        const long long r1 = (r0 + 32 < n_reads) ? r0 + 32 : n_reads;
        const long long b0 = a.offsets[r0], b1 = a.offsets[r1];
        if (b1 <= b0) return;
        const uintptr_t sa0 = (seq_base + b0) & ~(uintptr_t)15;
        const uint32_t bytes = (uint32_t)(((seq_base + b1 + 15) & ~(uintptr_t)15) - sa0);
        uint32_t qbytes = 0;
        uintptr_t qa0 = 0;
        if (HAS_QUAL) {
            qa0 = (qual_base + b0) & ~(uintptr_t)15;
            qbytes = (uint32_t)(((qual_base + b1 + 15) & ~(uintptr_t)15) - qa0);
        }
        mbar_expect_tx(&bars[0], bytes + qbytes);
        tma_load_1d(s_seq, (const void *)sa0, bytes, &bars[0]);
        if (HAS_QUAL) tma_load_1d(s_qual, (const void *)qa0, qbytes, &bars[0]);
    };
    if (lane == 0 && wg < n_mt) issue(wg);
    uint32_t phase0 = 0;
    for (long long mt = wg; mt < n_mt; mt += warps_total) {
        const long long r0 = mt * 32;
        const long long r1 = (r0 + 32 < n_reads) ? r0 + 32 : n_reads;
        const long long r = r0 + lane;
        const long long b0 = a.offsets[r0], b1 = a.offsets[r1];
        long long o0 = 0, o1 = 0;
        if (r < n_reads) { o0 = a.offsets[r]; o1 = a.offsets[r + 1]; }
        const uintptr_t sa0 = (seq_base + b0) & ~(uintptr_t)15;
        if (b1 > b0) { mbar_wait(&bars[0], phase0); phase0 ^= 1; }
        int q_ts = 0, q_te = 0;
        if (HAS_QUAL && a.quality_trim) {
            const uintptr_t qa0 = (qual_base + b0) & ~(uintptr_t)15;
            const bool has = r < n_reads;
            pre_trim_warp(s_seq + (size_t)(has ? (seq_base + o0) - sa0 : 0), s_qual + (size_t)(has ? (qual_base + o0) - qa0 : 0),
                          has ? (int)(o1 - o0) : 0, a.quality_trim, a.cutoff_front, a.cutoff_back, a.qbase, lane, &q_ts, &q_te);
        }
        int cls = CG_PLANE_NONE, s0 = 0, ts = 0, te = 0;
        int st_fin = -1;
        uint32_t st_p1 = 0, st_p2 = 0, st_p3 = 0;
        uint32_t t_flags = 4u | CG_TASK_RESCAN;
        uint32_t tm[8] = {0, 0, 0, 0, 0, 0, 0, 0};
        uint32_t win_region = 0, win_off = 0;
        bool mine = false;
        if (r < n_reads) {
            mine = true;
            const int n = (int)(o1 - o0);
            const uint32_t off = (uint32_t)((seq_base + o0) - sa0);
            ts = 0; te = n;
            if (HAS_QUAL && a.quality_trim) { ts = q_ts; te = q_te; }
            if (a.qtrim) { a.qtrim[2 * r] = ts; a.qtrim[2 * r + 1] = te; }
            if (a.view) { ts = a.view[2 * r]; te = a.view[2 * r + 1]; }
            const int nn = te - ts;
            if (nn >= 1 && nn <= 32 * W) {
                const PlaneOut po = plane_scan_core<W, Prog>(prog, n_prog, pflags, A.m, ref, s_seq + off + te, nn, always_pass);
                cls = po.cls; s0 = po.s0;
                if (po.bad & 0x80808080u) atomicOr(a.err_flag, 1);
                if (cls == CG_PLANE_SLOW) {
                    t_flags = 4u | CG_TASK_PLANES | (a.task_rec > 4 ? CG_TASK_BYTES : 0u) | ((uint32_t)W << 12) |
                              ((uint32_t)po.end_hit << 20) | ((uint32_t)po.no_end << 21);
                    const uint32_t wend = smem_u32(s_seq + off + te);
                    win_region = (wend - 32u * W) & ~15u;
                    win_off = (wend - (uint32_t)nn) - win_region;
#pragma unroll
                    for (int b = 0; b < 8; ++b) tm[b] = po.M[b];
                }
            } else {
                cls = CG_PLANE_SLOW;
                uint32_t bad = 0;
                for (int i = ts; i < te; ++i) bad |= s_seq[off + i];
                if (bad & 0x80u) atomicOr(a.err_flag, 1);
            }
            if (cls != CG_PLANE_SLOW) {
                CgHit hit; hit.adapter = -1; hit.remove = 0;
                hit.astart = hit.astop = hit.rstart = hit.rstop = hit.score = hit.errors = 0;
                if (cls == CG_PLANE_EXACT) hit_exact(A, nn, s0, hit);
                else if (cls == CG_PLANE_OVERLAP) hit_end_overlap(A, nn, s0, hit);
                store_hit(a.out + (size_t)r * a.slots, hit, 0, nn);
                if (STATS && a.stats) {
                    CG_PSCAN_STATS_VIEW
                    (void)s_hlen; (void)s_scal; (void)s_hadj;
                    st_p1 = (uint32_t)n | ((a.quality_trim && a.qtrim) ? (uint32_t)(n - nn) << 16 : 0u);
                    st_p2 = 1u << 16;
                    int fin = nn;
                    if (hit.adapter >= 0) {
                        const int kind = Prog::remove_kind(A.remove);
                        const bool after = kind == CGK_REMOVE_AUTO ? hit.remove == CGK_REMOVE_AFTER : kind == CGK_REMOVE_AFTER;
                        int removed = after ? nn - hit.rstart : hit.rstop;
                        removed = removed < 0 ? 0 : removed;
                        st_p2 |= (uint32_t)removed | (1u << 22);
                        atomicAdd(&s_hrem[(after ? st_len + 1 : 0) + (removed > st_len ? st_len : removed)], 1u);
                        if (after) {
                            int k = 4;
                            if (hit.rstart > 0) {
                                const uint8_t c = s_seq[off + ts + hit.rstart - 1];
                                k = c == 'A' ? 0 : (c == 'C' ? 1 : (c == 'G' ? 2 : (c == 'T' ? 3 : 4)));
                            }
                            st_p3 = 1u << (6 * k);
                            fin = hit.rstart;
                        } else {
                            fin = nn - hit.rstop;
                        }
                    }
                    st_fin = fin < 0 ? 0 : (fin > st_len ? st_len : fin);
                }
            }
        }
        if (STATS && a.stats) {
            CG_PSCAN_STATS_VIEW
            (void)s_hrem;
            const uint32_t counted = __ballot_sync(0xffffffffu, st_fin >= 0);
            if (counted) {
                const int leader = __ffs(counted) - 1;
                const int common = __shfl_sync(0xffffffffu, st_fin, leader);
                const uint32_t same = __ballot_sync(0xffffffffu, st_fin == common);
                if (lane == leader) atomicAdd(&s_hlen[common], (uint32_t)__popc(same));
                else if (st_fin >= 0 && st_fin != common) atomicAdd(&s_hlen[st_fin], 1u);
                const uint32_t s1 = __reduce_add_sync(0xffffffffu, st_p1);
                const uint32_t s2 = __reduce_add_sync(0xffffffffu, st_p2);
                const uint32_t s3 = __reduce_add_sync(0xffffffffu, st_p3);
                uint32_t mine_add = 0;
                switch (lane) {
                case 0: mine_add = (s2 >> 16) & 63u; break;
                case 1: mine_add = s2 >> 22; break;
                case 2: mine_add = s1 & 0xffffu; break;
                case 3: mine_add = s1 >> 16; break;
                case 4: mine_add = s2 & 0xffffu; break;
                default: if (lane < 10) mine_add = (s3 >> (6 * (lane - 5))) & 63u; break;
                }
                if (mine_add) {
                    if (lane < 5) atomicAdd(&s_scal[lane], (unsigned long long)mine_add);
                    else atomicAdd(&s_hadj[lane - 5], mine_add);
                }
            }
        }
        const bool slow = mine && cls == CG_PLANE_SLOW;
        const bool kind_b = slow && a.task_count_b != nullptr && (t_flags & CG_TASK_PLANES) && !(t_flags & (1u << 20)) &&
                            (tm[0] | tm[1] | tm[2] | tm[3] | tm[4] | tm[5] | tm[6] | tm[7]) == 0u;
        const uint32_t ballot_a = __ballot_sync(0xffffffffu, slow && !kind_b);
        const uint32_t ballot_b = __ballot_sync(0xffffffffu, kind_b);
        if (ballot_a | ballot_b) {
            unsigned long long base_a = 0, base_b = 0;
            if (lane == 0) {
                if (ballot_a) base_a = atomicAdd(a.task_count, (unsigned long long)__popc(ballot_a));
                if (ballot_b) base_b = atomicAdd(a.task_count_b, (unsigned long long)__popc(ballot_b));
            }
            base_a = __shfl_sync(0xffffffffu, base_a, 0);
            base_b = __shfl_sync(0xffffffffu, base_b, 0);
            if (slow) {
                const uint32_t below = (1u << lane) - 1u;
                const unsigned long long slot = kind_b
                    ? (unsigned long long)a.task_cap - 1ull - (base_b + __popc(ballot_b & below))
                    : base_a + __popc(ballot_a & below);
                uint4 *rec = a.tasks + (size_t)a.task_rec * slot;
                const unsigned long long woff = (unsigned long long)(o0 + ts);
                rec[0] = make_uint4((uint32_t)r, (uint32_t)(woff >> 32), (uint32_t)woff, (uint32_t)(te - ts));
                rec[1] = make_uint4(tm[0], t_flags, tm[1], tm[2]);
                rec[2] = make_uint4(tm[3], tm[4], tm[5], tm[6]);
                rec[3] = make_uint4(tm[7], win_off, 0u, 0u);
                if (t_flags & CG_TASK_BYTES) {
#pragma unroll
                    for (int c = 0; c < 2 * W + 1; ++c) {
                        uint4 v;
                        asm volatile("ld.shared.v4.u32 {%0, %1, %2, %3}, [%4];"
                                     : "=r"(v.x), "=r"(v.y), "=r"(v.z), "=r"(v.w) : "r"(win_region + 16u * (uint32_t)c));
                        rec[4 + c] = v;
                    }
                }
            }
        }
        __syncwarp();
        if (lane == 0) {
            const long long next = mt + warps_total;
            if (next < n_mt) issue(next);
        }
    }
    if (STATS && a.stats) {
        CG_PSCAN_STATS_VIEW
        __syncthreads();
        if (threadIdx.x < 5 && s_scal[threadIdx.x])
            atomicAdd(&a.stats[threadIdx.x == 1 ? 2 : (threadIdx.x == 2 ? 1 : threadIdx.x)], s_scal[threadIdx.x]);
        unsigned long long *hist = a.stats + CG_STATS_SCALARS;
        const long long end_size = cg_stats_end_size(st_len, a.stats_kmax);
        for (int i = threadIdx.x; i <= st_len; i += CG_NT) {
            const uint32_t v = s_hlen[i];
            if (v) atomicAdd(&hist[i], (unsigned long long)v);
            for (int kind = 0; kind < 2; ++kind) {
                const uint32_t w = s_hrem[kind * (st_len + 1) + i];
                if (w) atomicAdd(&hist[(st_len + 1) + kind * end_size + CG_STATS_ADJ + (long long)i * (a.stats_kmax + 1)],
                                 (unsigned long long)w);
            }
        }
        if (threadIdx.x < 8 && s_hadj[threadIdx.x])
            atomicAdd(&hist[(st_len + 1) + end_size + threadIdx.x], (unsigned long long)s_hadj[threadIdx.x]);
    }
}
```

Before: 7.462 billion.

## Emit compact stats entries from list kernels instead of rescanning task list

When stats are fused into the plane scan, the list kernels now gain a STATS template variant. Each finished slow read appends a packed 8-byte entry (lengths, removal, errors, preceding base) to a global buffer through a warp-aggregated atomic. A new small kernel builds histograms from these entries, replacing the old stats kernel that re-read the task list and sequences. The shared-memory stats helpers are factored out and reused by the pscan kernel. This adds extra atomics and stores in the list kernels and a second template instantiation, which may change occupancy; that is why occupancy is checked before fusing.

```diff
diff --git a/cutadapt_b200/csrc/cg_api.cu b/cutadapt_b200/csrc/cg_api.cu
--- a/cutadapt_b200/csrc/cg_api.cu
+++ b/cutadapt_b200/csrc/cg_api.cu
@@ -188,6 +188,7 @@
     struct { unsigned long long *d_stats = nullptr; int max_len = 0, kmax = 0; bool armed = false, done = false; } fuse;
     DevBuf<uint4> tasks;
     DevBuf<uint4> tasks2, tasks3;
+    DevBuf<uint2> stat_ents;
     unsigned long long *d_task_count = nullptr;
     DevBuf<cg_match_rec> pass_tmp;
     DevBuf<int32_t> view_base, view_back;
@@ -308,7 +309,7 @@
         l.h_seq.release(); l.h_qual.release(); l.h_offs.release(); l.h_out.release(); l.h_qtrim.release();
         if (l.stream) cudaStreamDestroy(l.stream);
     }
-    c->scratch_p.release(); c->scratch_w.release(); c->tasks.release(); c->tasks2.release(); c->tasks3.release();
+    c->scratch_p.release(); c->scratch_w.release(); c->tasks.release(); c->tasks2.release(); c->tasks3.release(); c->stat_ents.release();
     c->pass_tmp.release(); c->view_base.release(); c->view_back.release();
     for (FastqSlot &f : c->fq) {
         f.d_in.release(); f.d_out.release(); f.d_seq.release(); f.d_qual.release(); f.d_tiles.release(); f.d_nl.release();
@@ -564,8 +565,8 @@
             if (scan_smem <= c->smem_optin && list_smem <= c->smem_optin) {
                 if (plane_w) CU(cg_pscan_occupancy(want_q, plane_w, false, scan_smem, &scan_occ));
                 else CU(cg_scan_occupancy(want_q, scan_smem, &scan_occ));
-                CU(cg_list_occupancy(true, s->host.max_m, list_smem, &plan_occ));
-                CU(cg_list_occupancy(false, s->host.max_m, list_smem, &run_occ));
+                CU(cg_list_occupancy(true, s->host.max_m, false, list_smem, &plan_occ));
+                CU(cg_list_occupancy(false, s->host.max_m, false, list_smem, &run_occ));
                 split = scan_occ >= 1 && plan_occ >= 1 && run_occ >= 1;
             }
         }
@@ -586,12 +587,16 @@
         }
     }
     bool fuse_stats = split && plane_w && c->fuse.armed && !d_view && s->host.n_adapters == 1 && times == 1 &&
-                      s->host.slots == 1 && !want_q && !getenv("CUTADAPT_B200_TWO_LISTS") && c->fuse.max_len <= 4096;
+                      s->host.slots == 1 && !want_q && !getenv("CUTADAPT_B200_TWO_LISTS") && c->fuse.max_len <= 4096 &&
+                      cg_stats_entries_smem_bytes(c->fuse.max_len, c->fuse.kmax) <= 48 * 1024;
     if (fuse_stats) {
         const size_t fsmem = cg_pscan_smem_bytes(a.blob_bytes, a.mini_cap, want_q, c->fuse.max_len);
         int focc = 0;
         if (fsmem <= c->smem_optin) CU(cg_pscan_occupancy(want_q, plane_w, true, fsmem, &focc));
-        fuse_stats = focc >= 1 && focc >= scan_occ;
+        int pocc = 0, rocc = 0;
+        CU(cg_list_occupancy(true, s->host.max_m, true, list_smem, &pocc));
+        CU(cg_list_occupancy(false, s->host.max_m, true, list_smem, &rocc));
+        fuse_stats = focc >= 1 && focc >= scan_occ && pocc >= plan_occ && rocc >= run_occ;
         if (fuse_stats) {
             a.stats = c->fuse.d_stats; a.stats_max_len = c->fuse.max_len; a.stats_kmax = c->fuse.kmax;
             scan_smem = fsmem; scan_occ = focc;
@@ -655,6 +660,7 @@
         int rc = c->tasks.ensure((size_t)cap * plane_rec);
         if (rc == CG_OK) rc = c->tasks2.ensure((size_t)cap * 4);
         if (rc == CG_OK) rc = c->tasks3.ensure((size_t)cap * 4);
+        if (rc == CG_OK && fuse_stats) rc = c->stat_ents.ensure((size_t)cap);
         if (rc != CG_OK) return rc;
         unsigned long long *cnt = c->d_task_count;
         for (long long r0 = 0; r0 < n_reads; r0 += SUB) {
@@ -685,6 +691,7 @@
             else if (plane_w) CU(cg_launch_pscan(b, want_q, plane_w, grid_for(scan_occ), scan_smem, st));
             else CU(cg_launch_scan(b, want_q, grid_for(scan_occ), scan_smem, st));
             if (sev[0]) CU(cudaEventRecord(sev[1], st));
+            b.stat_ents = c->stat_ents.p; b.stat_count = cnt + 6;
             b.tasks2 = c->tasks2.p; b.task2_count = cnt + 1;
             b.tasks3 = c->tasks3.p; b.task3_count = cnt + 2;
             b.task2_count_b = (CG_RUN_BAND && plane_w && !getenv("CUTADAPT_B200_NO_BAND_LISTS")) ? cnt + 5 : nullptr;
@@ -713,8 +720,7 @@
             }
             if (sev[0]) { CU(cudaEventRecord(sev[3], st)); c->stage_events.push_back(sev); }
             if (fuse_stats) {
-                CU(cg_launch_stats(b.seq, b.offsets, n_sub, want_q && b.qtrim, 1, 1, b.out, b.qtrim, 1, a.stats_max_len,
-                                   a.stats_kmax, a.stats, st, c->tasks.p, plane_rec, cnt));
+                CU(cg_launch_stats_entries(c->stat_ents.p, cnt + 6, n_sub, a.stats_max_len, a.stats_kmax, a.stats, st));
                 c->launches += 1;
             }
         }
@@ -2594,7 +2600,7 @@
     CU(cudaMemsetAsync(f.d_fqstats.p, 0, total * sizeof(unsigned long long), st));
     if (g.d_matches && a.n_adapters > 0) {
         CU(cg_launch_stats(f.d_seq.p, f.d_offs.p, g.n, g.d_qtrim != nullptr, g.times, g.slots, g.d_matches, g.d_qtrim,
-                           a.n_adapters, a.max_len, a.kmax, f.d_fqstats.p, st, nullptr, 0, nullptr, 0,
+                           a.n_adapters, a.max_len, a.kmax, f.d_fqstats.p, st, 0,
                            g.action == CG_FQ_ACTION_LOWERCASE ? 1 : 0));
         c->launches += 1;
     }
diff --git a/cutadapt_b200/csrc/cg_args.h b/cutadapt_b200/csrc/cg_args.h
--- a/cutadapt_b200/csrc/cg_args.h
+++ b/cutadapt_b200/csrc/cg_args.h
@@ -37,6 +37,8 @@
     int no_band;
     unsigned long long *stats;
     int stats_max_len, stats_kmax;
+    uint2 *stat_ents;
+    unsigned long long *stat_count;
     uint32_t *scratch_p;
     int *scratch_w;
     long long scratch_stride;
diff --git a/cutadapt_b200/csrc/cg_kernels.cu b/cutadapt_b200/csrc/cg_kernels.cu
--- a/cutadapt_b200/csrc/cg_kernels.cu
+++ b/cutadapt_b200/csrc/cg_kernels.cu
@@ -686,6 +686,53 @@
 }
 size_t cg_dp_smem_bytes(uint32_t blob_bytes, int slot_bytes) { return dp_smem_layout(blob_bytes, slot_bytes).total; }
 
+template <bool PLAN>
+__device__ __forceinline__ void list_stats_append(const CgKernelArgs &a, const CgAdapter &A, bool fin, const CgHit &hit,
+                                                  const uint4 &ta, const uint4 &tc, const uint4 &td, const uint8_t *slot)
+{
+    uint32_t ex = 0, ey = 0;
+    if (fin) {
+        const int n = (int)ta.w;
+        int len = n;
+        if (hit.adapter >= 0) {
+            const bool after = hit.remove == CGK_REMOVE_AFTER;
+            int removed = after ? n - hit.rstart : hit.rstop;
+            removed = removed < 0 ? 0 : removed;
+            const int E = hit.errors < 0 ? 0 : (hit.errors > 2047 ? 2047 : hit.errors);
+            int k = 4;
+            if (after) {
+                if (hit.rstart > 0 && hit.rstart <= n) {
+                    int first = 0, count = 0;
+                    if (!PLAN) {
+                        const int ri = (int)tc.z;
+                        const uint32_t pk = ri == 0 ? td.x : (ri == 1 ? td.y : (ri == 2 ? td.z : td.w));
+                        const int lo = (int)(pk & 0xffffu), hi = (int)(pk >> 16);
+                        count = hi > lo ? hi - lo : 0;
+                        first = A.reverse ? n - hi : lo;
+                    }
+                    const uintptr_t w0 = (uintptr_t)a.seq + (((uintptr_t)ta.y << 32) | ta.z);
+                    const uintptr_t s0 = (w0 + first) & ~(uintptr_t)15, s1 = (w0 + first + count + 15) & ~(uintptr_t)15;
+                    const uintptr_t at = w0 + (hit.rstart - 1);
+                    const uint8_t c = (count > 0 && at >= s0 && at < s1) ? slot[at - s0] : *(const uint8_t *)at;
+                    k = c == 'A' ? 0 : (c == 'C' ? 1 : (c == 'G' ? 2 : (c == 'T' ? 3 : 4)));
+                }
+                len = hit.rstart < 0 ? 0 : (hit.rstart > n ? n : hit.rstart);
+            } else {
+                len = n - (hit.rstop < 0 ? 0 : (hit.rstop > n ? n : hit.rstop));
+            }
+            ey = 1u | (after ? 2u : 0u) | ((uint32_t)k << 2) | ((uint32_t)E << 5) | ((uint32_t)removed << 16);
+        }
+        ex = (uint32_t)n | ((uint32_t)len << 16);
+    }
+    const uint32_t ballot = __ballot_sync(0xffffffffu, fin);
+    if (!ballot) return;
+    const int lane = threadIdx.x & 31;
+    unsigned long long base = 0;
+    if (lane == 0) base = atomicAdd(a.stat_count, (unsigned long long)__popc(ballot));
+    base = __shfl_sync(0xffffffffu, base, 0);
+    if (fin) a.stat_ents[base + __popc(ballot & ((1u << lane) - 1u))] = make_uint2(ex, ey);
+}
+
 #ifndef CG_PLAN_BLOCKS
 #define CG_PLAN_BLOCKS 6
 #endif
@@ -695,7 +742,7 @@
 #ifndef CG_RUN48_BLOCKS
 #define CG_RUN48_BLOCKS 3
 #endif
-template <bool PLAN, int MR>
+template <bool PLAN, int MR, bool STATS>
 __global__ void __launch_bounds__(CG_NT, PLAN ? CG_PLAN_BLOCKS : (MR <= 16 ? CG_RUN16_BLOCKS : (MR <= 32 ? 3 : (MR <= 48 ? CG_RUN48_BLOCKS : 2)))) cg_list_kernel(const CgKernelArgs a)
 {
     extern __shared__ __align__(128) uint8_t smem[];
@@ -844,6 +891,7 @@
             }
         }
         if (has_task && !cont && !defer) store_hit(a.out + (size_t)r * a.slots, hit, 0, n);
+        if (STATS) list_stats_append<PLAN>(a, A, has_task && !cont && !defer, hit, ta, tc, td, s_slot + (size_t)lane * slot_bytes);
         if (PLAN) {
             const uint32_t dballot = __ballot_sync(0xffffffffu, defer);
             if (dballot) {
@@ -882,24 +930,29 @@
 }
 
 typedef void (*list_kernel_t)(const CgKernelArgs);
-static list_kernel_t pick_list(bool plan, int mr)
-{
-    if (plan) return cg_list_kernel<true, 16>;
-    if (mr <= 16) return cg_list_kernel<false, 16>;
-    if (mr <= 32) return cg_list_kernel<false, 32>;
-    if (mr <= 40) return cg_list_kernel<false, 40>;
-    return mr <= 48 ? cg_list_kernel<false, 48> : cg_list_kernel<false, 64>;
-}
-cudaError_t cg_list_occupancy(bool plan, int mr, size_t smem, int *blocks_per_sm)
-{
-    list_kernel_t k = pick_list(plan, mr);
+template <bool STATS>
+static list_kernel_t pick_list_v(bool plan, int mr)
+{
+    if (plan) return cg_list_kernel<true, 16, STATS>;
+    if (mr <= 16) return cg_list_kernel<false, 16, STATS>;
+    if (mr <= 32) return cg_list_kernel<false, 32, STATS>;
+    if (mr <= 40) return cg_list_kernel<false, 40, STATS>;
+    return mr <= 48 ? cg_list_kernel<false, 48, STATS> : cg_list_kernel<false, 64, STATS>;
+}
+static list_kernel_t pick_list(bool plan, int mr, bool stats)
+{
+    return stats ? pick_list_v<true>(plan, mr) : pick_list_v<false>(plan, mr);
+}
+cudaError_t cg_list_occupancy(bool plan, int mr, bool stats, size_t smem, int *blocks_per_sm)
+{
+    list_kernel_t k = pick_list(plan, mr, stats);
     cudaError_t e = cudaFuncSetAttribute(k, cudaFuncAttributeMaxDynamicSharedMemorySize, (int)smem);
     if (e != cudaSuccess) return e;
     return cudaOccupancyMaxActiveBlocksPerMultiprocessor(blocks_per_sm, k, CG_NT, smem);
 }
 cudaError_t cg_launch_list(const CgKernelArgs &a, bool plan, int mr, int grid, size_t smem, cudaStream_t st)
 {
-    pick_list(plan, mr)<<<grid, CG_NT, smem, st>>>(a);
+    pick_list(plan, mr, a.stats != nullptr)<<<grid, CG_NT, smem, st>>>(a);
     return cudaGetLastError();
 }
 
@@ -1354,9 +1407,8 @@
 template <bool SMEM_HIST>
 __global__ void cg_stats_kernel(const uint8_t *seq, const int64_t *offsets, long long n_reads, int quality_trim, int times,
                                 int slots, const cg_match_rec *matches, const int32_t *qtrim,
-                                int n_adapters, int max_len, int kmax, unsigned long long *stats,
-                                const uint4 *task_list, int task_rec, const unsigned long long *task_count,
-                                int count_lengths, int upper)
+                                int n_adapters, int max_len, int kmax, unsigned long long *stats, int count_lengths,
+                                int upper)
 {
     extern __shared__ unsigned int s_hist[];
     const long long nbins = cg_stats_total(n_adapters, max_len, kmax) - CG_STATS_SCALARS;
@@ -1367,17 +1419,7 @@
     unsigned long long n = 0;
     StatsScalars sc; sc.bp = sc.with_adapters = sc.qtrim_bp = sc.adapter_bp = 0;
     unsigned long long *hist = stats + CG_STATS_SCALARS;
-    long long n_items = n_reads;
-    if (task_list) {
-        const unsigned long long t = *task_count;
-        n_items = t < (unsigned long long)n_reads ? (long long)t : n_reads;
-    }
-    for (long long i = (long long)blockIdx.x * blockDim.x + threadIdx.x; i < n_items; i += nthreads) {
-        long long r = i;
-        if (task_list) {
-            const uint4 t = task_list[(size_t)task_rec * i];
-            r = (long long)t.x;
-        }
+    for (long long r = (long long)blockIdx.x * blockDim.x + threadIdx.x; r < n_reads; r += nthreads) {
         const long long o0 = offsets[r];
         const int len = (int)(offsets[r + 1] - o0);
         n += 1;
@@ -1412,8 +1454,7 @@
 cudaError_t cg_launch_stats(const uint8_t *d_seq, const int64_t *d_offsets, long long n_reads, int quality_trim, int times,
                             int slots, const cg_match_rec *d_matches, const int32_t *d_qtrim,
                             int n_adapters, int max_len, int kmax, unsigned long long *d_stats,
-                            cudaStream_t st, const uint4 *d_task_list, int task_rec, const unsigned long long *d_task_count,
-                            int count_lengths, int upper)
+                            cudaStream_t st, int count_lengths, int upper)
 {
     const int block = 256;
     long long grid = (n_reads + block - 1) / block;
@@ -1425,12 +1466,58 @@
     if (hist_bytes <= 48 * 1024 && n_reads / grid < (1LL << 31))
         cg_stats_kernel<true><<<(int)grid, block, hist_bytes, st>>>(d_seq, d_offsets, n_reads, quality_trim, times, slots,
                                                                      d_matches, d_qtrim, n_adapters, max_len, kmax, d_stats,
-                                                                     d_task_list, task_rec, d_task_count, count_lengths,
-                                                                     upper);
+                                                                     count_lengths, upper);
     else
         cg_stats_kernel<false><<<(int)grid, block, len_bytes, st>>>(d_seq, d_offsets, n_reads, quality_trim, times, slots,
                                                                      d_matches, d_qtrim, n_adapters, max_len, kmax, d_stats,
-                                                                     d_task_list, task_rec, d_task_count, count_lengths,
-                                                                     upper);
-    return cudaGetLastError();
-}
+                                                                     count_lengths, upper);
+    return cudaGetLastError();
+}
+
+__global__ void __launch_bounds__(CG_NT) cg_stats_entries_kernel(const uint2 *ents, const unsigned long long *count,
+                                                                 int max_len, int kmax, unsigned long long *stats)
+{
+    extern __shared__ __align__(16) uint8_t s_ent_hist[];
+    const StatsSmem H = stats_smem_view(s_ent_hist, max_len, kmax + 1);
+    stats_smem_zero(H, max_len, kmax + 1);
+    __syncthreads();
+    const long long n = (long long)*count;
+    const int lane = threadIdx.x & 31;
+    for (long long w = (long long)blockIdx.x * CG_NT + (threadIdx.x & ~31); w < n; w += (long long)gridDim.x * CG_NT) {
+        const long long i = w + lane;
+        int bin = -1;
+        uint32_t p1 = 0, p2 = 0, p3 = 0;
+        if (i < n) {
+            const uint2 e = ents[i];
+            const int len = (int)(e.x >> 16);
+            p1 = e.x & 0xffffu;
+            p2 = 1u << 16;
+            if (e.y & 1u) {
+                const bool after = (e.y & 2u) != 0;
+                const int removed = (int)(e.y >> 16), E = (int)((e.y >> 5) & 2047u);
+                p2 |= (uint32_t)removed | (1u << 22);
+                atomicAdd(&H.hrem[((after ? max_len + 1 : 0) + (removed > max_len ? max_len : removed)) * (kmax + 1) +
+                                  (E > kmax ? kmax : E)], 1u);
+                if (after) p3 = 1u << (6 * ((e.y >> 2) & 7u));
+            }
+            bin = len > max_len ? max_len : len;
+        }
+        stats_warp_add(H, bin, p1, p2, p3);
+    }
+    __syncthreads();
+    stats_cta_flush(H, max_len, kmax, kmax + 1, stats);
+}
+
+size_t cg_stats_entries_smem_bytes(int max_len, int kmax) { return stats_smem_bytes(max_len, kmax + 1); }
+
+cudaError_t cg_launch_stats_entries(const uint2 *d_ents, const unsigned long long *d_count, long long cap, int max_len,
+                                    int kmax, unsigned long long *d_stats, cudaStream_t st)
+{
+    const size_t smem = stats_smem_bytes(max_len, kmax + 1);
+    if (smem > 48 * 1024) return cudaErrorInvalidValue;
+    long long grid = (cap + CG_NT - 1) / CG_NT;
+    grid = cg_grid_cap(grid, 2);
+    if (grid < 1) grid = 1;
+    cg_stats_entries_kernel<<<(int)grid, CG_NT, smem, st>>>(d_ents, d_count, max_len, kmax, d_stats);
+    return cudaGetLastError();
+}
diff --git a/cutadapt_b200/csrc/cg_kernels.cuh b/cutadapt_b200/csrc/cg_kernels.cuh
--- a/cutadapt_b200/csrc/cg_kernels.cuh
+++ b/cutadapt_b200/csrc/cg_kernels.cuh
@@ -41,7 +41,7 @@
 cudaError_t cg_pscan_occupancy(bool has_qual, int w, bool stats, size_t smem, int *blocks_per_sm);
 cudaError_t cg_launch_pscan(const CgKernelArgs &a, bool has_qual, int w, int grid, size_t smem, cudaStream_t st);
 size_t cg_dp_smem_bytes(uint32_t blob_bytes, int slot_bytes);
-cudaError_t cg_list_occupancy(bool plan, int mr, size_t smem, int *blocks_per_sm);
+cudaError_t cg_list_occupancy(bool plan, int mr, bool stats, size_t smem, int *blocks_per_sm);
 cudaError_t cg_launch_list(const CgKernelArgs &a, bool plan, int mr, int grid, size_t smem, cudaStream_t st);
 cudaError_t cg_launch_generic(const CgKernelArgs &a, int grid, int block, cudaStream_t st);
 cudaError_t cg_launch_locate_debug(const uint8_t *d_blob, const uint8_t *d_enc, const uint8_t *d_query, int n,
@@ -56,10 +56,12 @@
 cudaError_t cg_launch_stats(const uint8_t *d_seq, const int64_t *d_offsets, long long n_reads, int quality_trim, int times,
                             int slots, const cg_match_rec *d_matches, const int32_t *d_qtrim,
                             int n_adapters, int max_len, int kmax, unsigned long long *d_stats,
-                            cudaStream_t st, const uint4 *d_task_list = nullptr, int task_rec = 0,
-                            const unsigned long long *d_task_count = nullptr,
+                            cudaStream_t st,
                             int count_lengths = 1,
                             int upper = 0);
+size_t cg_stats_entries_smem_bytes(int max_len, int kmax);
+cudaError_t cg_launch_stats_entries(const uint2 *d_ents, const unsigned long long *d_count, long long cap, int max_len,
+                                    int kmax, unsigned long long *d_stats, cudaStream_t st);
 cudaError_t cg_launch_nextseq_trim(const uint8_t *d_seq, const uint8_t *d_qual, const int64_t *d_offsets,
                                    long long n_reads, int cutoff, int base, int32_t *d_out, cudaStream_t st);
 cudaError_t cg_launch_poly_a_trim(const uint8_t *d_seq, const int64_t *d_offsets, long long n_reads, int revcomp,
diff --git a/cutadapt_b200/csrc/cg_pscan.cuh b/cutadapt_b200/csrc/cg_pscan.cuh
--- a/cutadapt_b200/csrc/cg_pscan.cuh
+++ b/cutadapt_b200/csrc/cg_pscan.cuh
@@ -12,6 +12,72 @@
 #define CG_TASK_RESCAN 0x100u
 #define CG_TASK_BYTES 0x400u
 #define CG_TASK_PLANES 0x200u
+struct StatsSmem { uint32_t *hlen, *hrem, *hadj; unsigned long long *scal; };
+__host__ __device__ inline size_t stats_smem_bytes(int max_len, int cols)
+{
+    return cg_align_up((size_t)((1 + 2 * cols) * (max_len + 1) + 8) * sizeof(uint32_t), 8) + 8 * sizeof(unsigned long long);
+}
+__device__ __forceinline__ StatsSmem stats_smem_view(uint8_t *base, int max_len, int cols)
+{
+    StatsSmem H;
+    H.hlen = (uint32_t *)base;
+    H.hrem = H.hlen + (max_len + 1);
+    H.hadj = H.hrem + 2 * cols * (max_len + 1);
+    H.scal = (unsigned long long *)(base + stats_smem_bytes(max_len, cols) - 8 * sizeof(unsigned long long));
+    return H;
+}
+__device__ __forceinline__ void stats_smem_zero(const StatsSmem &H, int max_len, int cols)
+{
+    for (int i = threadIdx.x; i < (1 + 2 * cols) * (max_len + 1) + 8; i += CG_NT) H.hlen[i] = 0;
+    if (threadIdx.x < 8) H.scal[threadIdx.x] = 0;
+}
+__device__ __forceinline__ void stats_warp_add(const StatsSmem &H, int fin, uint32_t p1, uint32_t p2, uint32_t p3)
+{
+    const int lane = threadIdx.x & 31;
+    const uint32_t counted = __ballot_sync(0xffffffffu, fin >= 0);
+    if (!counted) return;
+    const int leader = __ffs(counted) - 1;
+    const int common = __shfl_sync(0xffffffffu, fin, leader);
+    const uint32_t same = __ballot_sync(0xffffffffu, fin == common);
+    if (lane == leader) atomicAdd(&H.hlen[common], (uint32_t)__popc(same));
+    else if (fin >= 0 && fin != common) atomicAdd(&H.hlen[fin], 1u);
+    const uint32_t s1 = __reduce_add_sync(0xffffffffu, p1);
+    const uint32_t s2 = __reduce_add_sync(0xffffffffu, p2);
+    const uint32_t s3 = __reduce_add_sync(0xffffffffu, p3);
+    uint32_t mine_add = 0;
+    switch (lane) {
+    case 0: mine_add = (s2 >> 16) & 63u; break;
+    case 1: mine_add = s2 >> 22; break;
+    case 2: mine_add = s1 & 0xffffu; break;
+    case 3: mine_add = s1 >> 16; break;
+    case 4: mine_add = s2 & 0xffffu; break;
+    default: if (lane < 10) mine_add = (s3 >> (6 * (lane - 5))) & 63u; break;
+    }
+    if (mine_add) {
+        if (lane < 5) atomicAdd(&H.scal[lane], (unsigned long long)mine_add);
+        else atomicAdd(&H.hadj[lane - 5], mine_add);
+    }
+}
+__device__ __forceinline__ void stats_cta_flush(const StatsSmem &H, int max_len, int kmax, int cols, unsigned long long *stats)
+{
+    if (threadIdx.x < 5 && H.scal[threadIdx.x])
+        atomicAdd(&stats[threadIdx.x == 1 ? 2 : (threadIdx.x == 2 ? 1 : threadIdx.x)], H.scal[threadIdx.x]);
+    unsigned long long *hist = stats + CG_STATS_SCALARS;
+    const long long end_size = cg_stats_end_size(max_len, kmax);
+    for (int i = threadIdx.x; i <= max_len; i += CG_NT) {
+        const uint32_t v = H.hlen[i];
+        if (v) atomicAdd(&hist[i], (unsigned long long)v);
+    }
+    for (int i = threadIdx.x; i < 2 * cols * (max_len + 1); i += CG_NT) {
+        const uint32_t w = H.hrem[i];
+        const int kind = i / (cols * (max_len + 1)), j = i - kind * cols * (max_len + 1);
+        if (w) atomicAdd(&hist[(max_len + 1) + kind * end_size + CG_STATS_ADJ + (long long)(j / cols) * (kmax + 1) + j % cols],
+                         (unsigned long long)w);
+    }
+    if (threadIdx.x < 8 && H.hadj[threadIdx.x])
+        atomicAdd(&hist[(max_len + 1) + end_size + threadIdx.x], (unsigned long long)H.hadj[threadIdx.x]);
+}
+
 __host__ __device__ inline ScanSmem pscan_smem_layout(uint32_t blob_bytes, int mini_cap, bool has_qual, int stats_max_len = -1)
 {
     ScanSmem L;
@@ -19,7 +85,7 @@
     L.blob_off = o; o += cg_align_up(blob_bytes, 16);
     L.enc_off = o; o += 768;
     L.stats_off = o;
-    if (stats_max_len >= 0) o += cg_align_up((size_t)(3 * (stats_max_len + 1) + 8) * sizeof(uint32_t), 8) + 8 * sizeof(unsigned long long);
+    if (stats_max_len >= 0) o += stats_smem_bytes(stats_max_len, 1);
     o = cg_align_up(o, 128);
     L.warp_off = o;
     size_t w = 0;
@@ -111,15 +177,10 @@
     uint8_t *s_qual = wbase + L.qual_rel;
 #define CG_PSCAN_STATS_VIEW                                                                                              \
     const int st_len = a.stats_max_len;                                                                                  \
-    uint32_t *s_hlen = (uint32_t *)(smem + pscan_smem_layout(a.blob_bytes, a.mini_cap, HAS_QUAL, st_len).stats_off);     \
-    uint32_t *s_hrem = s_hlen + (st_len + 1);              \
-    uint32_t *s_hadj = s_hrem + 2 * (st_len + 1);                                                                        \
-    unsigned long long *s_scal = (unsigned long long *)((uint8_t *)s_hlen + cg_align_up((size_t)(3 * (st_len + 1) + 8) * sizeof(uint32_t), 8));
+    const StatsSmem H = stats_smem_view(smem + pscan_smem_layout(a.blob_bytes, a.mini_cap, HAS_QUAL, st_len).stats_off, st_len, 1);
     if (STATS && a.stats) {
         CG_PSCAN_STATS_VIEW
-        (void)s_hrem; (void)s_hadj;
-        for (int i = threadIdx.x; i < 3 * (st_len + 1) + 8; i += CG_NT) s_hlen[i] = 0;
-        if (threadIdx.x < 8) s_scal[threadIdx.x] = 0;
+        stats_smem_zero(H, st_len, 1);
     }
     for (uint32_t i = tid; i < a.blob_bytes / 16; i += CG_NT) ((uint4 *)s_blob)[i] = ((const uint4 *)a.blob)[i];
     for (uint32_t i = tid; i < 768 / 16; i += CG_NT) ((uint4 *)s_enc)[i] = ((const uint4 *)a.enc)[i];
@@ -219,7 +280,6 @@
                 store_hit(a.out + (size_t)r * a.slots, hit, 0, nn);
                 if (STATS && a.stats) {
                     CG_PSCAN_STATS_VIEW
-                    (void)s_hlen; (void)s_scal; (void)s_hadj;
                     st_p1 = (uint32_t)n | ((a.quality_trim && a.qtrim) ? (uint32_t)(n - nn) << 16 : 0u);
                     st_p2 = 1u << 16;
                     int fin = nn;
@@ -229,7 +289,7 @@
                         int removed = after ? nn - hit.rstart : hit.rstop;
                         removed = removed < 0 ? 0 : removed;
                         st_p2 |= (uint32_t)removed | (1u << 22);
-                        atomicAdd(&s_hrem[(after ? st_len + 1 : 0) + (removed > st_len ? st_len : removed)], 1u);
+                        atomicAdd(&H.hrem[(after ? st_len + 1 : 0) + (removed > st_len ? st_len : removed)], 1u);
                         if (after) {
                             int k = 4;
                             if (hit.rstart > 0) {
@@ -248,31 +308,7 @@
         }
         if (STATS && a.stats) {
             CG_PSCAN_STATS_VIEW
-            (void)s_hrem;
-            const uint32_t counted = __ballot_sync(0xffffffffu, st_fin >= 0);
-            if (counted) {
-                const int leader = __ffs(counted) - 1;
-                const int common = __shfl_sync(0xffffffffu, st_fin, leader);
-                const uint32_t same = __ballot_sync(0xffffffffu, st_fin == common);
-                if (lane == leader) atomicAdd(&s_hlen[common], (uint32_t)__popc(same));
-                else if (st_fin >= 0 && st_fin != common) atomicAdd(&s_hlen[st_fin], 1u);
-                const uint32_t s1 = __reduce_add_sync(0xffffffffu, st_p1);
-                const uint32_t s2 = __reduce_add_sync(0xffffffffu, st_p2);
-                const uint32_t s3 = __reduce_add_sync(0xffffffffu, st_p3);
-                uint32_t mine_add = 0;
-                switch (lane) {
-                case 0: mine_add = (s2 >> 16) & 63u; break;
-                case 1: mine_add = s2 >> 22; break;
-                case 2: mine_add = s1 & 0xffffu; break;
-                case 3: mine_add = s1 >> 16; break;
-                case 4: mine_add = s2 & 0xffffu; break;
-                default: if (lane < 10) mine_add = (s3 >> (6 * (lane - 5))) & 63u; break;
-                }
-                if (mine_add) {
-                    if (lane < 5) atomicAdd(&s_scal[lane], (unsigned long long)mine_add);
-                    else atomicAdd(&s_hadj[lane - 5], mine_add);
-                }
-            }
+            stats_warp_add(H, st_fin, st_p1, st_p2, st_p3);
         }
         const bool slow = mine && cls == CG_PLANE_SLOW;
         const bool kind_b = slow && a.task_count_b != nullptr && (t_flags & CG_TASK_PLANES) && !(t_flags & (1u << 20)) &&
@@ -318,20 +354,6 @@
     if (STATS && a.stats) {
         CG_PSCAN_STATS_VIEW
         __syncthreads();
-        if (threadIdx.x < 5 && s_scal[threadIdx.x])
-            atomicAdd(&a.stats[threadIdx.x == 1 ? 2 : (threadIdx.x == 2 ? 1 : threadIdx.x)], s_scal[threadIdx.x]);
-        unsigned long long *hist = a.stats + CG_STATS_SCALARS;
-        const long long end_size = cg_stats_end_size(st_len, a.stats_kmax);
-        for (int i = threadIdx.x; i <= st_len; i += CG_NT) {
-            const uint32_t v = s_hlen[i];
-            if (v) atomicAdd(&hist[i], (unsigned long long)v);
-            for (int kind = 0; kind < 2; ++kind) {
-                const uint32_t w = s_hrem[kind * (st_len + 1) + i];
-                if (w) atomicAdd(&hist[(st_len + 1) + kind * end_size + CG_STATS_ADJ + (long long)i * (a.stats_kmax + 1)],
-                                 (unsigned long long)w);
-            }
-        }
-        if (threadIdx.x < 8 && s_hadj[threadIdx.x])
-            atomicAdd(&hist[(st_len + 1) + end_size + threadIdx.x], (unsigned long long)s_hadj[threadIdx.x]);
-    }
-}
+        stats_cta_flush(H, st_len, a.stats_kmax, 1, a.stats);
+    }
+}
```

After: 7.750 billion, median of 6. 3.9% higher.
